# akashsengupta1997/STRAPS-3DHumanShapePose

Measured on AMD Instinct MI355X. Metric: bodies/sec, higher is better.
Workload: dtype fp32 (encoder convolutions as exact bf16x3 operand splits (six bf16 products per term); in-step SMPL blend contraction and skinning as 3-product fp16 splits (fp16x3_lbs: 22-bit operands); fp32 accumulate throughout)

## Files before the change

### include/straps_hip.h

```cpp
#ifndef STRAPS_HIP_H
#define STRAPS_HIP_H

#include <stddef.h>
#include <stdint.h>

#ifdef __cplusplus
extern "C" {
#endif

#define STRAPS_ABI_VERSION 12

#define STRAPS_OK 0
#define STRAPS_EINVAL 1
#define STRAPS_EHIP 2
#define STRAPS_EUNSUPPORTED 3

int straps_abi_version(void);
int straps_selftest_mfma_peak(const float* seed512, float* out, int blocks, int iters, void* stream);
int straps_selftest_mfma_bf16(float* out, unsigned long long* clk2, int blocks, int iters, void* stream);
int straps_selftest_mfma_bf16_dense(float* out, unsigned long long* clk2, int blocks, int iters, int data, void* stream);
const char* straps_last_error(void);
int straps_device_count(void);
int straps_wall_clock_khz(void);
int straps_set_clock_accumulator(unsigned long long* acc2);
// ... 129 lines not shown
#define STRAPS_SMPL_SPLIT_F16_LBS_P16 4

size_t straps_smpl_workspace_bytes(const straps_smpl_model_t* model, long long batch);
int straps_smpl_fwd(const straps_smpl_model_t* model, const float* betas, const float* rotmats,
                    float* verts, float* joints, void* workspace, long long batch, int chunks, int mode,
                    void* stream);

size_t straps_smpl_bwd_workspace_bytes(long long batch, int chunks);
int straps_smpl_bwd(const straps_smpl_model_t* model, const float* betas, const float* rotmats,
                    const float* dverts, const float* djoints, float* dbetas, float* drotmats,
                    void* workspace, long long batch, int chunks, void* stream);
int straps_smpl_bwd_aa(const straps_smpl_model_t* model, const float* betas, const float* rotmats,
                       const float* full_pose_aa, const float* dverts, const float* djoints, float* dbetas,
                       float* dfull_pose_aa, float* drotmats, void* workspace, long long batch, int chunks,
                       void* stream);

int straps_conv_dgrad(const float* dy_nhwc, const float* w_crsk, const float* addend,
                      float* dx_nhwc, int batch, int h, int w, int cin, int cout, int kh, int kw,
                      int stride, int pad, int tile_cfg, void* stream);

int straps_split3_bf16(const float* x, unsigned short* planes, long long n, long long plane_stride,
                       void* stream);
int straps_split3_bf16_cm(const float* x, unsigned short* planes, long long rows, int c,
                          long long plane_stride, void* stream);
int straps_conv_x3_stat_blocks(int batch, int h, int w, int cin, int cout, int kh, int kw, int stride,
                               int pad, int tile_cfg);

int straps_conv_x3f_supported(int cin, int cout, int kh, int kw, int stride, int pad);
int straps_conv_fwd_x3f(const float* x, const float* a_scale, const float* a_shift, int a_relu, const unsigned short* w3,
                        long long w_plane_stride, const float* scale, const float* shift, const float* residual, int relu,
                        float* y, float* stats_partial, int batch, int h, int w, int cin, int cout, int kh, int kw, int stride,
                        int pad, int tile_cfg, void* stream);
int straps_conv_x3f_stat_blocks(int batch, int h, int w, int cin, int cout, int kh, int kw, int stride, int pad, int tile_cfg);
int straps_conv_dgrad_x3f(const float* dy, const unsigned short* w3_crsk, long long w_plane_stride, const float* addend,
                          const unsigned* addend_bits, float* dx, int batch, int h, int w, int cin, int cout, int kh, int kw,
                          int stride, int pad, int tile_cfg, const float* bn_raw, const unsigned* bn_out_bits,
                          const float* bn_mask_scale, const float* bn_mask_shift, const float* bn_mean, const float* bn_invstd,
                          double* bn_partials, void* stream);
int straps_conv_dgrad_x3f_bn_blocks(int batch, int h, int w, int cin, int cout, int kh, int kw, int stride, int pad, int tile_cfg);
size_t straps_conv_wgrad_x3f_workspace_bytes(int batch, int h, int w, int cin, int cout, int kh, int kw, int stride, int pad);
int straps_conv_wgrad_x3f(const float* x, const float* a_scale, const float* a_shift, int a_relu, const float* dy, float* dw_oihw,
                          void* workspace, int batch, int h, int w, int cin, int cout, int kh, int kw, int stride, int pad,
                          int accumulate, void* stream);
int straps_conv_fwd_x3(const unsigned short* x3, long long x_plane_stride,
                       const unsigned short* w3_krsc, long long w_plane_stride, const float* scale,
                       const float* shift, const float* residual, int relu, float* y_nhwc,
                       float* stats_partial, int batch, int h, int w, int cin, int cout, int kh,
                       int kw, int stride, int pad, int tile_cfg, void* stream);
int straps_conv_fwd_x3p(const unsigned short* x3, long long x_plane_stride,
                        const unsigned short* w3_krsc, long long w_plane_stride, const float* scale,
                        const float* shift, const float* residual, int relu, float* y_nhwc,
                        unsigned short* y_planes, long long y_plane_stride, int batch, int h, int w,
                        int cin, int cout, int kh, int kw, int stride, int pad, int tile_cfg, void* stream);
int straps_split_bf16_cm(const float* x, unsigned short* plane, long long rows, int c, void* stream);
int straps_pack_conv_weight_bf16(const float* w_oihw, unsigned short* w_plane, int cout, int cin, int kh, int kw, void* stream);
int straps_conv_bf16_tile_choice(int batch, int h, int w, int cin, int cout, int kh, int kw, int stride, int pad);
int straps_conv_fwd_bf16(const unsigned short* x1, const unsigned short* w1_krsc, const float* scale, const float* shift,
                         const float* residual, int relu, float* y_nhwc, unsigned short* y_plane, int batch, int h, int w,
                         int cin, int cout, int kh, int kw, int stride, int pad, int tile_cfg, void* stream);
int straps_conv_dgrad_x3(const unsigned short* dy3, long long dy_plane_stride,
                         const unsigned short* w3_crsk, long long w_plane_stride,
                         const float* addend, float* dx_nhwc, int batch, int h, int w, int cin,
                         int cout, int kh, int kw, int stride, int pad, int tile_cfg, void* stream);
int straps_bn_apply_x3(const float* raw, const float* scale, const float* shift, const float* residual,
                       int relu, float* y, unsigned short* y_planes, long long plane_stride,
                       long long rows, int c, void* stream);
int straps_bn_relu_maxpool_fwd_x3(const float* raw, const float* scale, const float* shift,
                                  float* y_pool, uint8_t* idx, unsigned short* y_planes,
                                  long long plane_stride, int batch, int h, int w, int c, void* stream);
int straps_bn_bwd_x3(const float* dy, const float* yact, const float* raw, const float* save_mean,
                     const float* save_invstd, const float* gamma, const float* mask_scale,
                     const float* mask_shift, float* dgamma, float* dbeta, float* draw, float* dz_out,
                     unsigned short* draw_planes, long long plane_stride, void* workspace,
                     long long rows, int c, int accumulate, void* stream);
int straps_conv_dgrad_x3_bn_blocks(int batch, int h, int w, int cin, int cout, int kh, int kw, int stride,
                                   int pad, int tile_cfg);
int straps_conv_dgrad_x3_bn(const unsigned short* dy3, long long dy_plane_stride,
                            const unsigned short* w3_crsk, long long w_plane_stride, const float* addend,
                            float* dx_nhwc, int batch, int h, int w, int cin, int cout, int kh, int kw,
                            int stride, int pad, int tile_cfg, const float* bn_raw, const float* bn_out,
                            const float* bn_mask_scale, const float* bn_mask_shift, const float* bn_mean,
                            const float* bn_invstd, double* bn_partials, void* stream);
int straps_bn_bwd_finish_x3(const float* dy, const float* yact, const float* raw, const float* save_mean,
                            const float* save_invstd, const float* gamma, const float* mask_scale,
                            const float* mask_shift, float* dgamma, float* dbeta, float* draw, float* dz_out,
                            unsigned short* draw_planes, long long plane_stride, const double* partials,
                            int nblk, void* workspace, long long rows, int c, int accumulate, void* stream);
int straps_bn_apply_bits_x3(const float* raw, const float* scale, const float* shift, const float* residual, float* y,
                            unsigned short* y_planes, long long plane_stride, unsigned* relu_bits, long long rows,
                            int c, void* stream);
int straps_bn_bwd_bits_x3(const float* dy, const unsigned* relu_bits, const float* raw, const float* save_mean,
                          const float* save_invstd, const float* gamma, float* dgamma, float* dbeta, float* draw,
                          unsigned short* draw_planes, long long plane_stride, void* workspace, long long rows, int c,
                          int accumulate, void* stream);
int straps_bn_bwd_finish_bits_x3(const float* dy, const unsigned* relu_bits, const float* raw, const float* save_mean,
                                 const float* save_invstd, const float* gamma, float* dgamma, float* dbeta, float* draw,
                                 unsigned short* draw_planes, long long plane_stride, const double* partials, int nblk,
                                 void* workspace, long long rows, int c, int accumulate, void* stream);
int straps_conv_dgrad_x3_bits(const unsigned short* dy3, long long dy_plane_stride, const unsigned short* w3_crsk,
                              long long w_plane_stride, const float* addend, float* dx_nhwc, int batch, int h, int w,
                              int cin, int cout, int kh, int kw, int stride, int pad, int tile_cfg,
                              const unsigned* addend_bits, void* stream);
int straps_conv_dgrad_x3_bn_bits(const unsigned short* dy3, long long dy_plane_stride,
                                 const unsigned short* w3_crsk, long long w_plane_stride, const float* addend,
                                 float* dx_nhwc, int batch, int h, int w, int cin, int cout, int kh, int kw,
                                 int stride, int pad, int tile_cfg, const float* bn_raw, const float* bn_out,
                                 const float* bn_mask_scale, const float* bn_mask_shift, const float* bn_mean,
                                 const float* bn_invstd, double* bn_partials, const unsigned* addend_bits,
                                 const unsigned* bn_out_bits, void* stream);
int straps_conv_wgrad_x3_on_planes(int batch, int h, int w, int cin, int cout, int kh, int kw,
                                   int stride, int pad);
int straps_conv_wgrad_x3(const float* x_nhwc, const float* dy_nhwc, const unsigned short* x3,
                         long long x_plane_stride, const unsigned short* dy3, long long dy_plane_stride,
                         float* dw_oihw, void* workspace, int batch, int h, int w, int cin, int cout,
                         int kh, int kw, int stride, int pad, int accumulate, void* stream);


size_t straps_conv_wgrad_workspace_bytes(int batch, int h, int w, int cin, int cout, int kh,
                                         int kw, int stride, int pad);
int straps_conv_wgrad(const float* x_nhwc, const float* dy_nhwc, float* dw_oihw, void* workspace,
                      int batch, int h, int w, int cin, int cout, int kh, int kw, int stride,
                      int pad, int accumulate, void* stream);
size_t straps_stem_wgrad_workspace_bytes(int batch, int cin, int h, int w);
int straps_stem_wgrad(const float* x_nchw, const float* dy_nhwc, float* dw_oihw, void* workspace,
                      const uint32_t* nzmask , int batch, int cin,
                      int h, int w, int accumulate, void* stream);
#define STRAPS_STEM_DGRAD_MAX_CIN 64
size_t straps_stem_dgrad_weight_floats(int cin);
int straps_pack_stem_dgrad_weight(const float* w_oihw, float* w_pk, int cin, void* stream);
int straps_stem_dgrad(const float* dy_nhwc, const float* w_pk, float* dx_nchw, int batch, int cin, int h, int w,
                      int accumulate, void* stream);
int straps_bn_bwd_blocks(long long rows, int c);
size_t straps_bn_bwd_workspace_bytes(long long rows, int c);
int straps_bn_bwd(const float* dy, const float* yact, const float* raw, const float* save_mean,
                  const float* save_invstd, const float* gamma, const float* mask_scale,
                  const float* mask_shift, float* dgamma, float* dbeta, float* draw, float* dz_out,
                  void* workspace, long long rows, int c, int accumulate, void* stream);
int straps_bn_relu_maxpool_fwd(const float* raw_nhwc, const float* scale, const float* shift,
                               float* y_pool_nhwc, uint8_t* idx, int batch, int h, int w, int c,
                               void* stream);
int straps_bn_bwd_pooled(const float* dy_pool_nhwc, const uint8_t* idx, const float* raw,
                         const float* save_mean, const float* save_invstd, const float* gamma,
                         const float* mask_scale, const float* mask_shift, float* dgamma, float* dbeta,
                         float* draw, void* workspace, int batch, int h, int w, int c, int accumulate,
                         void* stream);
size_t straps_stem_tiles(int batch, int in_h, int in_w);
int straps_stem_tile_activity(const uint32_t* nzmask, uint8_t* tile_active, int batch, int cin, int in_h,
                              int in_w, void* stream);
int straps_bn_bwd_pooled_sparse(const float* dy_pool_nhwc, const uint8_t* idx, const float* raw,
                                const float* save_mean, const float* save_invstd, const float* gamma,
                                const float* mask_scale, const float* mask_shift, float* dgamma,
                                float* dbeta, float* draw, void* workspace, int batch, int h, int w, int c,
                                int accumulate, const uint8_t* tile_active, void* stream);
int straps_maxpool_fwd_idx(const float* x_nhwc, float* y_nhwc, uint8_t* idx, int batch, int h,
                           int w, int c, void* stream);
int straps_maxpool_bwd(const float* dy_nhwc, const uint8_t* idx, float* dx_nhwc, int batch, int h,
                       int w, int c, void* stream);
int straps_gap_bwd(const float* dfeat, float* dx_nhwc, int batch, int hw, int c, void* stream);
int straps_masked_copy(const float* x, int ldx, const float* mask, int ldmask, float* y, int ldy,
                       int m, int n, int accumulate, void* stream);
int straps_rot6d_bwd(const float* x6, long long ld, int per_row, const float* drot, float* dx6,
                     long long ldd, long long rows, void* stream);

int straps_build_proxy_input(const float* seg, const float* joints2d, float* out_nchw, int batch,
                             int nj, int wh, void* stream);
int straps_build_proxy_input_std(const float* seg, const float* joints2d, float* out_nchw, int batch,
                                 int nj, int wh, int std, void* stream);
int straps_build_proxy_input_nz(const float* seg, const float* joints2d, float* out_nchw, uint32_t* nzmask,
                                int batch, int nj, int wh, int std, void* stream);
size_t straps_loss_workspace_bytes(long long batch);
int straps_loss_fwd_bwd(const float* pred_verts, const float* pred_joints, const float* est,
                        int ld_est, const float* pred_rot, const float* tgt_verts,
                        const float* tgt_joints2d, const float* tgt_joints3d,
                        const float* tgt_shape, const float* tgt_rot, const float* log_vars,
                        float* loss_out, float* dverts, float* djoints, float* dest, float* drot,
                        float* dlogvar, void* workspace, long long batch, int img_wh, void* stream);
int straps_loss_fwd_bwd_gm(const float* pred_verts, const float* pred_joints, const float* est, int ld_est,
                           const float* pred_rot, const float* tgt_verts, const float* tgt_joints2d,
                           const float* tgt_joints3d, const float* tgt_shape, const float* tgt_rot,
                           const float* log_vars, float* loss_out, float* dverts, float* djoints, float* dest,
                           float* drot, float* dlogvar, void* workspace, long long batch, int img_wh,
                           const float* j2d_count_global, float count_scale, void* stream);
int straps_count_visible(const float* tgt_joints2d, float* out_count, long long batch, int nj, int img_wh,
                         void* stream);
int straps_mse_fwd(const float* pred, const float* tgt, const uint8_t* row_mask, long long rows,
                   int cols, float tgt_scale, float tgt_shift, float* out3, void* workspace,
                   void* stream);
int straps_mse_bwd(const float* pred, const float* tgt, const uint8_t* row_mask, long long rows,
                   int cols, float tgt_scale, float tgt_shift, const float* coef, float* grad,
                   void* stream);
int straps_augment_seg(const float* seg, const float* uniforms, const float* remove_prob,
                       float occlude_prob, int box_dim, float* out, int batch, int wh, void* stream);
int straps_philox_fill(unsigned long long seed, const long long* step_dev, long long step_host,
                       unsigned substream, float* out, long long n, int kind, void* stream);
int straps_counter_add(long long* counters, int n, long long delta, void* stream);
int straps_gather_f32(const float* src, const int* index, float* dst, int n, void* stream);
int straps_memset_zero(void* ptr, size_t bytes, void* stream);
int straps_augment_smpl(const float* pose_rows, long long n_rows, const float* u_index,
                        const float* orig_shape, const float* mean_shape, const float* shape_draws,
                        int shape_mode, const float* std_vector, double range_lo, double range_hi,
                        float* out_shape, float* out_rotmats, float* out_pose, long long batch,
                        void* stream);
int straps_augment_cam_t(const float* mean_cam_t, const float* normals_xy, const float* uniform_z,
                         double xy_std, double z_lo, double z_hi, float* out_cam_t, long long batch,
                         void* stream);
int straps_deviate_joints2d(const float* joints2d, const float* uniforms, double lo, double hi,
                            double hip_lo, double hip_hi, float* out, long long batch, void* stream);
int straps_deviate_verts2d(const float* verts, const float* uniforms, double lo, double hi, float* out,
                           long long nverts_total, void* stream);
int straps_project_targets(const float* joints, const float* cam_t, float fx, float fy, float cx,
                           float cy, float* joints2d, float* joints3d, long long batch, void* stream);
size_t straps_rasterize_workspace_bytes(long long batch, int nverts, int wh);
int straps_rasterize_parts(const float* verts, const int32_t* faces, const uint8_t* face_parts,
                           const float* cam_K, const float* cam_R, const float* cam_t, float* parts,
                           float* depth, void* workspace, long long batch, int nverts, int nfaces, int wh,
                           int cam_per_body, float near, float far, const float* vert_noise_u, double noise_lo,
                           double noise_hi, void* stream);
int straps_crop_resize(const float* seg, const float* joints2d, const float* uniforms,
                       double orig_scale_factor, double delta_scale_lo, double delta_scale_hi,
                       double delta_centre_lo, double delta_centre_hi, float* out_seg,
                       float* out_joints2d, int* boxes, int batch, int wh, int out_wh, int nj,
                       void* stream);
int straps_point_metrics(const float* pred, const float* target, float* out3, long long batch,
                         int npoints, void* stream);
int straps_adam_step(float* params, const float* grads, float* exp_avg, float* exp_avg_sq,
                     long long n, int step, float lr, float beta1, float beta2, float eps,
                     float grad_scale, const long long* step_dev, void* stream);

typedef struct {
    int layers;
    int in_channels;
    int ief_iters;
    int precision;
} straps_regressor_desc_t;
size_t straps_regressor_param_floats(const straps_regressor_desc_t* desc);
size_t straps_regressor_prepared_bytes(const straps_regressor_desc_t* desc);
int straps_regressor_prepare(const straps_regressor_desc_t* desc, const float* params, void* prepared, void* stream);
size_t straps_regressor_workspace_bytes(const straps_regressor_desc_t* desc, int batch, int h, int w);
int straps_regressor_fwd_infer(const straps_regressor_desc_t* desc, const void* prepared, const float* x, int batch, int h, int w,
                               float* est, int ld_est, float* rotmats, void* workspace, size_t workspace_bytes, void* stream);

size_t straps_regressor_train_param_floats(const straps_regressor_desc_t* desc);
size_t straps_regressor_bn_state_floats(const straps_regressor_desc_t* desc);
size_t straps_regressor_train_workspace_bytes(const straps_regressor_desc_t* desc, int batch, int h, int w);
int straps_regressor_fwd_train(const straps_regressor_desc_t* desc, const float* params, float* bn_state, const float* init_est,
                               const float* x, int batch, int h, int w, float* est, int ld_est,
                               void* workspace, size_t workspace_bytes, void* stream);
int straps_regressor_bwd(const straps_regressor_desc_t* desc, const float* params, const float* x, int batch, int h, int w,
                         const float* dest, int ld_dest, float* grads, float* dx,
                         void* workspace, size_t workspace_bytes, void* stream);
int straps_regressor_export_infer_params(const straps_regressor_desc_t* desc, const float* params, const float* bn_state,
                                         const float* init_est, float* infer_params, void* stream);

#define STRAPS_COMM_ID_BYTES 128
int straps_comm_unique_id(void* id128);
int straps_comm_init_rank(const void* id128, int nranks, int rank, void** comm);
int straps_comm_destroy(void* comm);
int straps_comm_size(void* comm);
const char* straps_comm_library(void);
int straps_allreduce_grads(float* flat_g, long long n, void* comm, void* stream);

#ifdef __cplusplus
}
#endif
#endif
```

### straps-3dhumanshapepose_amd/autograd_ops.py

```python
import ctypes as C

import torch

from . import hipabi
from .encoder_exec import encoder_forward
from .ief_module import EST_LD


def _empty_like(t):
    return torch.empty_like(t, memory_format=torch.contiguous_format)


class GradSink(dict):

    def __init__(self, views=None):
        super().__init__()
        self.views = views

    def buf(self, p, zero=False):
        if self.views is not None and p in self.views:
            return self.views[p]
        return torch.zeros_like(p) if zero else torch.empty_like(p)


class _SideStream:

    def __init__(self, stream):
        self.s, self.keep = stream, []

    def run(self, fn, *tensors):
        if self.s is None:
            return fn()
        self.keep.extend(tensors)
        self.s.wait_stream(torch.cuda.current_stream())
        with torch.cuda.stream(self.s):
            return fn()

    def join(self):
        if self.s is not None:
            torch.cuda.current_stream().wait_stream(self.s)
            self.keep.clear()


_FUSE_BN_SUMS = True
_SPARSE_STEM_TAIL = True


def _packed_dgrad_weight(net, conv):
    w = conv.weight

    def make():
        wd = w.detach().contiguous()
        out = torch.empty(wd.numel(), device=wd.device, dtype=torch.float32)
        hipabi.check(hipabi.lib().straps_pack_conv_weight_dgrad(hipabi.ptr(wd), hipabi.ptr(out), wd.shape[0], wd.shape[1], wd.shape[2],
                                                                wd.shape[3], hipabi.stream_ptr()), 'straps_pack_conv_weight_dgrad')
        return out
    return net._cached(('wd', id(conv)), [w], make)


def _bn_bwd(L, rec, dy, masked, want_dz, grads, planes_sink=None, keep_fp32=True, mask_bits=None):
    bn = rec['bn']
    raw, ss = rec['raw'], rec['stats']
    rows, Cc = raw.numel() // raw.shape[-1], raw.shape[-1]
    ws = torch.empty(L.straps_bn_bwd_workspace_bytes(rows, Cc) // 4, device=raw.device, dtype=torch.float32)
    dgamma, dbeta = grads.buf(bn.weight), grads.buf(bn.bias)
    keep_fp32 = keep_fp32 or planes_sink is None
    draw = _empty_like(raw) if keep_fp32 else raw.new_empty(0)
    dz = _empty_like(raw) if want_dz else None
    from_raw = masked and rec.get('residual') is None
    bits = mask_bits if mask_bits is not None else (rec.get('bits') if masked and not from_raw else None)
    if bits is not None and want_dz:
        raise RuntimeError('BatchNorm backward on ReLU bits writes no masked gradient (dz)')
    planes, ps = None, 0
    if planes_sink is not None:
        ps = (raw.numel() + 7) // 8 * 8
        planes = torch.empty(3, ps, device=raw.device, dtype=torch.int16)
        planes_sink[id(draw)] = (draw, planes, ps)
    flags = 2 if rec.get('frozen') else 0
    fused = rec.pop('bwd_partials', None)
    if bits is not None:
        args = (hipabi.ptr(dy), hipabi.ptr(bits), hipabi.ptr(raw), hipabi.ptr(ss[2]), hipabi.ptr(ss[3]), hipabi.ptr(bn.weight), hipabi.ptr(dgamma),
                hipabi.ptr(dbeta), hipabi.ptr(draw if keep_fp32 else None), hipabi.ptr(planes), ps)
        if fused is not None and fused[2] is dy and masked:
            hipabi.check(L.straps_bn_bwd_finish_bits_x3(*args, hipabi.ptr(fused[0]), fused[1], hipabi.ptr(ws), rows, Cc, flags, hipabi.stream_ptr()),
                         'straps_bn_bwd_finish_bits_x3')
        else:
            hipabi.check(L.straps_bn_bwd_bits_x3(*args, hipabi.ptr(ws), rows, Cc, flags, hipabi.stream_ptr()), 'straps_bn_bwd_bits_x3')
    elif fused is not None and fused[2] is dy and masked:
        hipabi.check(L.straps_bn_bwd_finish_x3(hipabi.ptr(dy), hipabi.ptr(rec['out'] if not from_raw else None), hipabi.ptr(raw), hipabi.ptr(ss[2]),
                                               hipabi.ptr(ss[3]), hipabi.ptr(bn.weight), hipabi.ptr(ss[0] if from_raw else None),
                                               hipabi.ptr(ss[1] if from_raw else None), hipabi.ptr(dgamma), hipabi.ptr(dbeta),
                                               hipabi.ptr(draw if keep_fp32 else None), hipabi.ptr(dz), hipabi.ptr(planes), ps, hipabi.ptr(fused[0]),
                                               fused[1], hipabi.ptr(ws), rows, Cc, flags, hipabi.stream_ptr()), 'straps_bn_bwd_finish_x3')
    else:
        hipabi.check(L.straps_bn_bwd_x3(hipabi.ptr(dy), hipabi.ptr(rec['out'] if masked and not from_raw else None), hipabi.ptr(raw), hipabi.ptr(ss[2]),
                                        hipabi.ptr(ss[3]), hipabi.ptr(bn.weight), hipabi.ptr(ss[0] if from_raw else None),
                                        hipabi.ptr(ss[1] if from_raw else None), hipabi.ptr(dgamma), hipabi.ptr(dbeta), hipabi.ptr(draw if keep_fp32 else None),
                                        hipabi.ptr(dz), hipabi.ptr(planes), ps, hipabi.ptr(ws), rows, Cc, flags, hipabi.stream_ptr()), 'straps_bn_bwd')
    grads[bn.weight] = dgamma
    grads[bn.bias] = dbeta
    return draw, dz


def _conv_wgrad(L, rec, draw, grads, planes_sink=None):
    conv = rec['conv']
    B, H, W, Cin, Cout, k, stride, pad, Ho, Wo = rec['geom']
    dw = grads.buf(conv.weight)
    if rec.get('fmode'):
        a_bn = rec.get('a_bn')
        wsf = torch.empty(max(L.straps_conv_wgrad_x3f_workspace_bytes(B, H, W, Cin, Cout, k, k, stride, pad) // 4, 1), device=draw.device, dtype=torch.float32)
        hipabi.check(L.straps_conv_wgrad_x3f(hipabi.ptr(rec['x']), hipabi.ptr(a_bn[0] if a_bn is not None else None), hipabi.ptr(a_bn[1] if a_bn is not None else None),
                                             int(a_bn is not None), hipabi.ptr(draw), hipabi.ptr(dw), hipabi.ptr(wsf), B, H, W, Cin, Cout, k, k, stride, pad, 0,
                                             hipabi.stream_ptr()), 'straps_conv_wgrad_x3f')
        grads[conv.weight] = dw
        return
    ws = torch.empty(L.straps_conv_wgrad_workspace_bytes(B, H, W, Cin, Cout, k, k, stride, pad) // 4, device=draw.device, dtype=torch.float32)
    fp = lambda t: hipabi.ptr(t if t is not None and t.numel() else None)
    xh = rec.get('x3')
    gh = planes_sink.get(id(draw)) if planes_sink is not None else None
    if xh is not None and gh is not None and xh[0] is rec['x'] and gh[0] is draw:
        hipabi.check(L.straps_conv_wgrad_x3(fp(rec['x']), fp(draw), hipabi.ptr(xh[1]), xh[2], hipabi.ptr(gh[1]), gh[2], hipabi.ptr(dw),
                                            hipabi.ptr(ws), B, H, W, Cin, Cout, k, k, stride, pad, 0, hipabi.stream_ptr()), 'straps_conv_wgrad_x3')
    else:
        hipabi.check(L.straps_conv_wgrad(hipabi.ptr(rec['x']), hipabi.ptr(draw), hipabi.ptr(dw), hipabi.ptr(ws), B, H, W, Cin, Cout, k, k, stride,
                                         pad, 0, hipabi.stream_ptr()), 'straps_conv_wgrad')
    grads[conv.weight] = dw


def _conv_dgrad(L, net, rec, draw, addend, planes_sink=None, bn_next=None, addend_bits=None):
    conv = rec['conv']
    B, H, W, Cin, Cout, k, stride, pad, Ho, Wo = rec['geom']
    dx = torch.empty(B, H, W, Cin, device=draw.device, dtype=torch.float32)
    if rec.get('fmode'):
        if not draw.numel():
            raise RuntimeError('fp32-operand data gradient: the fp32 gradient was not materialised')
        w3, wps = net._packed_weight_x3(conv, dgrad=True)
        raw = nbits = msc = msh = mean = invstd = part = None
        if bn_next is not None and _FUSE_BN_SUMS:
            ssn = bn_next['stats']
            from_raw = bn_next.get('residual') is None
            nbits = None if from_raw else bn_next.get('bits')
            if from_raw or nbits is not None:
                nblk = L.straps_conv_dgrad_x3f_bn_blocks(B, H, W, Cin, Cout, k, k, stride, pad, 0)
                part = torch.empty(nblk, Cin, 2, device=dx.device, dtype=torch.float64)
                raw, mean, invstd = bn_next['raw'], ssn[2], ssn[3]
                if from_raw:
                    msc, msh = ssn[0], ssn[1]
        if bn_next is None or not _FUSE_BN_SUMS or part is not None:
            hipabi.check(L.straps_conv_dgrad_x3f(hipabi.ptr(draw), hipabi.ptr(w3), wps, hipabi.ptr(addend), hipabi.ptr(addend_bits), hipabi.ptr(dx), B, H, W, Cin, Cout,
                                                 k, k, stride, pad, 0, hipabi.ptr(raw), hipabi.ptr(nbits), hipabi.ptr(msc), hipabi.ptr(msh), hipabi.ptr(mean),
                                                 hipabi.ptr(invstd), hipabi.ptr(part), hipabi.stream_ptr()), 'straps_conv_dgrad_x3f')
            if part is not None:
                bn_next['bwd_partials'] = (part, nblk, dx)
            return dx
    if getattr(net, 'conv_precision', 'fp32') == 'bf16x3':
        if not draw.numel() and (planes_sink is None or planes_sink.get(id(draw)) is None):
            raise RuntimeError('data gradient: neither the fp32 gradient nor its planes exist')
        hit = planes_sink.get(id(draw)) if planes_sink is not None else None
        if hit is not None and hit[0] is draw:
            g3, gps = hit[1], hit[2]
        else:
            from .encoder_exec import split3
            g3, gps = split3(L, draw)
        w3, wps = net._packed_weight_x3(conv, dgrad=True)
        if bn_next is not None and _FUSE_BN_SUMS:
            ssn = bn_next['stats']
            from_raw = bn_next.get('residual') is None
            nblk = L.straps_conv_dgrad_x3_bn_blocks(B, H, W, Cin, Cout, k, k, stride, pad, 0)
            part = torch.empty(nblk, Cin, 2, device=dx.device, dtype=torch.float64)
            nbits = None if from_raw else bn_next.get('bits')
            if addend_bits is not None or nbits is not None:
                hipabi.check(L.straps_conv_dgrad_x3_bn_bits(hipabi.ptr(g3), gps, hipabi.ptr(w3), wps, hipabi.ptr(addend), hipabi.ptr(dx), B, H, W, Cin,
                                                            Cout, k, k, stride, pad, 0, hipabi.ptr(bn_next['raw']),
                                                            hipabi.ptr(None if from_raw or nbits is not None else bn_next['out']),
                                                            hipabi.ptr(ssn[0] if from_raw else None), hipabi.ptr(ssn[1] if from_raw else None),
                                                            hipabi.ptr(ssn[2]), hipabi.ptr(ssn[3]), hipabi.ptr(part), hipabi.ptr(addend_bits),
                                                            hipabi.ptr(nbits), hipabi.stream_ptr()), 'straps_conv_dgrad_x3_bn_bits')
                bn_next['bwd_partials'] = (part, nblk, dx)
                return dx
            hipabi.check(L.straps_conv_dgrad_x3_bn(hipabi.ptr(g3), gps, hipabi.ptr(w3), wps, hipabi.ptr(addend), hipabi.ptr(dx), B, H, W, Cin, Cout,
                                                   k, k, stride, pad, 0, hipabi.ptr(bn_next['raw']), hipabi.ptr(None if from_raw else bn_next['out']),
                                                   hipabi.ptr(ssn[0] if from_raw else None), hipabi.ptr(ssn[1] if from_raw else None),
                                                   hipabi.ptr(ssn[2]), hipabi.ptr(ssn[3]), hipabi.ptr(part), hipabi.stream_ptr()),
                         'straps_conv_dgrad_x3_bn')
            bn_next['bwd_partials'] = (part, nblk, dx)
            return dx
        if addend_bits is not None:
            hipabi.check(L.straps_conv_dgrad_x3_bits(hipabi.ptr(g3), gps, hipabi.ptr(w3), wps, hipabi.ptr(addend), hipabi.ptr(dx), B, H, W, Cin, Cout,
                                                     k, k, stride, pad, 0, hipabi.ptr(addend_bits), hipabi.stream_ptr()), 'straps_conv_dgrad_x3_bits')
            return dx
        hipabi.check(L.straps_conv_dgrad_x3(hipabi.ptr(g3), gps, hipabi.ptr(w3), wps, hipabi.ptr(addend), hipabi.ptr(dx), B, H, W, Cin, Cout,
                                            k, k, stride, pad, 0, hipabi.stream_ptr()), 'straps_conv_dgrad_x3')
        return dx
    if addend_bits is not None:
        raise RuntimeError('ReLU bits exist only on the bf16x3 route')
    hipabi.check(L.straps_conv_dgrad(hipabi.ptr(draw), hipabi.ptr(_packed_dgrad_weight(net, conv)), hipabi.ptr(addend), hipabi.ptr(dx), B, H, W,
                                     Cin, Cout, k, k, stride, pad, 0, hipabi.stream_ptr()), 'straps_conv_dgrad')
    return dx


def encoder_backward(net, tape, dfeat, views=None, side_stream=None, after_layer3=None, want_dx=False, param_grads=True):
    L = hipabi.lib()
    grads = GradSink(views)
    side = _SideStream(side_stream)
    sink = {} if getattr(net, 'conv_precision', 'fp32') == 'bf16x3' else None

    def sink_of(rec):
        return None if rec.get('fmode') else sink

    def keep(rec):
        if sink is None or rec.get('x3') is None:
            return True
        B, H, W, Cin, Cout, k, stride, pad, Ho, Wo = rec['geom']
        return not L.straps_conv_wgrad_x3_on_planes(B, H, W, Cin, Cout, k, k, stride, pad)
    rec = tape['gap']
    B, HW, Cf = rec['geom']
    dy = _empty_like(rec['x'])
    hipabi.check(L.straps_gap_bwd(hipabi.ptr(dfeat.contiguous()), hipabi.ptr(dy), B, HW, Cf, hipabi.stream_ptr()), 'straps_gap_bwd')
    units = [u for li in range(1, 5) for u in getattr(net, 'layer%d' % li)]
    for li in range(4, 0, -1):
        for unit in reversed(list(getattr(net, 'layer%d' % li))):
            pairs = unit.conv_bn_pairs()
            ui = units.index(unit)
            prev_last = tape[id(units[ui - 1].conv_bn_pairs()[-1][0])] if ui > 0 else None
            rec = tape[id(pairs[-1][0])]
            ubits = rec.get('bits') if sink is not None else None
            dskip_bits = None
            if ubits is not None:
                draw, _ = _bn_bwd(L, rec, dy, True, False, grads, sink_of(rec), keep(rec))
                dz = dy
            else:
                draw, dz = _bn_bwd(L, rec, dy, True, True, grads, sink_of(rec), keep(rec))
            if param_grads:
                side.run(lambda rec=rec, draw=draw: _conv_wgrad(L, rec, draw, grads, sink), draw)
            if unit.downsample is not None:
                recd = tape[id(unit.downsample[0])]
                drawd, _ = _bn_bwd(L, recd, dz, False, False, grads, sink_of(recd), keep(recd), mask_bits=ubits)
                if param_grads:
                    side.run(lambda recd=recd, drawd=drawd: _conv_wgrad(L, recd, drawd, grads, sink), drawd)
                dskip = _conv_dgrad(L, net, recd, drawd, None, sink)
            else:
                dskip, dskip_bits = dz, ubits
            for ci in range(len(pairs) - 1, 0, -1):
                rec_prev = tape[id(pairs[ci - 1][0])]
                dt = _conv_dgrad(L, net, tape[id(pairs[ci][0])], draw, None, sink, bn_next=rec_prev if sink is not None else None)
                rec = rec_prev
                draw, _ = _bn_bwd(L, rec, dt, True, False, grads, sink_of(rec), keep(rec))
                if param_grads:
                    side.run(lambda rec=rec, draw=draw: _conv_wgrad(L, rec, draw, grads, sink), draw)
            dy = _conv_dgrad(L, net, tape[id(pairs[0][0])], draw, dskip, sink, bn_next=prev_last if sink is not None else None,
                             addend_bits=dskip_bits)
        if li == 3 and after_layer3 is not None:
            side.join()
            after_layer3()
    rec = tape['maxpool']
    B, H, W, Cc, Hp, Wp = rec['geom']
    if rec['kind'] == 'maxpool_fused':
        idx = rec['idx']
        rec = tape['stem']
        bn, raw, ss = rec['bn'], rec['raw'], rec['stats']
        ws = torch.empty(L.straps_bn_bwd_workspace_bytes(B * H * W, Cc) // 4, device=raw.device, dtype=torch.float32)
        dgamma, dbeta = grads.buf(bn.weight), grads.buf(bn.bias)
        draw = _empty_like(raw)
        tact = None
        if rec.get('nzmask') is not None and _SPARSE_STEM_TAIL and not want_dx:
            _, Cin0, Hin, Win = rec['geom'][:4]
            tact = torch.empty(L.straps_stem_tiles(B, Hin, Win), device=raw.device, dtype=torch.uint8)
            hipabi.check(L.straps_stem_tile_activity(hipabi.ptr(rec['nzmask']), hipabi.ptr(tact), B, Cin0, Hin, Win, hipabi.stream_ptr()),
                         'straps_stem_tile_activity')
        hipabi.check(L.straps_bn_bwd_pooled_sparse(hipabi.ptr(dy), hipabi.ptr(idx), hipabi.ptr(raw), hipabi.ptr(ss[2]), hipabi.ptr(ss[3]),
                                                   hipabi.ptr(bn.weight), hipabi.ptr(ss[0]), hipabi.ptr(ss[1]), hipabi.ptr(dgamma), hipabi.ptr(dbeta),
                                                   hipabi.ptr(draw), hipabi.ptr(ws), B, H, W, Cc, 2 if rec.get('frozen') else 0, hipabi.ptr(tact),
                                                   hipabi.stream_ptr()), 'straps_bn_bwd_pooled_sparse')
        grads[bn.weight] = dgamma
        grads[bn.bias] = dbeta
    else:
        dstem = _empty_like(rec['x'])
        hipabi.check(L.straps_maxpool_bwd(hipabi.ptr(dy), hipabi.ptr(rec['idx']), hipabi.ptr(dstem), B, H, W, Cc, hipabi.stream_ptr()),
                     'straps_maxpool_bwd')
        rec = tape['stem']
        draw, _ = _bn_bwd(L, rec, dstem, True, False, grads)
    B, Cin, H, W, Ho, Wo = rec['geom']
    dx = None
    if want_dx:
        dx = torch.empty(B, Cin, H, W, device=draw.device, dtype=torch.float32)
        hipabi.check(L.straps_stem_dgrad(hipabi.ptr(draw), hipabi.ptr(net._packed_stem_dgrad_weight()), hipabi.ptr(dx), B, Cin, H, W, 0,
                                         hipabi.stream_ptr()), 'straps_stem_dgrad')
    if param_grads:
        ws = torch.empty(L.straps_stem_wgrad_workspace_bytes(B, Cin, H, W) // 4, device=draw.device, dtype=torch.float32)
        dw = grads.buf(net.conv1.weight)
        hipabi.check(L.straps_stem_wgrad(hipabi.ptr(rec['x']), hipabi.ptr(draw), hipabi.ptr(dw), hipabi.ptr(ws), hipabi.ptr(rec.get('nzmask')),
                                         B, Cin, H, W, 0, hipabi.stream_ptr()), 'straps_stem_wgrad')
        grads[net.conv1.weight] = dw
    side.join()
    return (grads, dx) if want_dx else grads


def ief_backward(ief, feat, tape, dest, views=None, param_grads=True):
    sink = GradSink(views)
    L, st = hipabi.lib(), hipabi.stream_ptr()
    pk = ief._packed(feat.device)
    B, F = feat.shape
    H1, H2, P = ief.fc1.out_features, ief.fc2.out_features, ief.num_output_params
    dev = feat.device
    T = len(tape)
    e = lambda *s: torch.empty(*s, device=dev, dtype=torch.float32)
    D = hipabi.gemm_desc
    ests, h1s, h2s = tape[0]['stacks']
    assert ests.shape == (T + 1, B, EST_LD) and h1s.shape == (T, B, H1) and h2s.shape == (T, B, H2)
    dW3, db3 = sink.buf(ief.fc3.weight), sink.buf(ief.fc3.bias)
    dW2, db2 = sink.buf(ief.fc2.weight), sink.buf(ief.fc2.bias)
    dW1, db1 = sink.buf(ief.fc1.weight), sink.buf(ief.fc1.bias)
    dests = e(T + 1, B, EST_LD)
    dsrc = dest if dest.stride(-1) == 1 and dest.dim() == 2 else dest.contiguous()
    hipabi.check(L.straps_masked_copy(hipabi.ptr(dsrc), dsrc.stride(0), None, 0, hipabi.ptr(dests[T]), EST_LD, B, EST_LD, 0, st), 'ief dest slot')
    dh2s, dh1s, dc1 = e(T, B, H2), e(T, B, H1), e(B, H1)
    w3, w2 = ief.fc3.weight, ief.fc2.weight
    for it in reversed(range(T)):
        hipabi.gemm_multi([D(dests[it + 1], EST_LD, 1, w3, H2, 1, dh2s[it], H2, B, H2, P, mask=h2s[it], ldmask=H2)])
        hipabi.gemm_multi([D(dh2s[it], H2, 1, w2, H1, 1, dh1s[it], H1, B, H1, H2, mask=h1s[it], ldmask=H1,
                             c2=dc1, ldc2=H1, accumulate2=int(it != T - 1))])
        hipabi.gemm_multi([D(dh1s[it], H1, 1, pk['w1e'], EST_LD, 1, dests[it], EST_LD, B, P, H1, addend=dests[it + 1], ldadd=EST_LD)])
    one = pk['one']
    dfeat = e(B, F)
    if not param_grads:
        hipabi.gemm_multi([D(dc1, H1, 1, pk['w1f'], F, 1, dfeat, F, B, F, H1)])
        return dfeat, {}
    KB = T * B
    hipabi.gemm_multi([
        D(dh2s, 1, H2, h1s, H1, 1, dW2, H1, H2, H1, KB),
        D(dc1, 1, H1, feat, F, 1, dW1, F + P, H1, F, B),
        D(dh1s, 1, H1, ests, EST_LD, 1, dW1.data_ptr() + 4 * F, F + P, H1, P, KB),
        D(dests[1], 1, EST_LD, h2s, H2, 1, dW3, H2, P, H2, KB),
        D(dc1, H1, 1, pk['w1f'], F, 1, dfeat, F, B, F, H1),
        D(one, 0, 0, dh2s, H2, 1, db2, H2, 1, H2, KB),
        D(one, 0, 0, dests[1], EST_LD, 1, db3, P, 1, P, KB),
        D(one, 0, 0, dc1, H1, 1, db1, H1, 1, H1, B)])
    grads = {ief.fc1.weight: dW1, ief.fc1.bias: db1, ief.fc2.weight: dW2, ief.fc2.bias: db2, ief.fc3.weight: dW3, ief.fc3.bias: db3}
    return dfeat, grads


class _RegressorFn(torch.autograd.Function):

    @staticmethod
    def forward(ctx, reg, x, *params):
        enc_tape, ief_tape = {}, []
        with torch.no_grad():
            feat = encoder_forward(reg.image_encoder, x, enc_tape)
            est = reg.ief_module.forward_estimate(feat, ief_tape)
        ctx.reg, ctx.feat, ctx.enc_tape, ctx.ief_tape, ctx.params = reg, feat, enc_tape, ief_tape, params
        return est

    @staticmethod
    def backward(ctx, dest):
        reg = ctx.reg
        want_dx, pg = ctx.needs_input_grad[1], any(ctx.needs_input_grad[2:])
        dfeat, g_ief = ief_backward(reg.ief_module, ctx.feat, ctx.ief_tape, dest, param_grads=pg)
        g_enc = encoder_backward(reg.image_encoder, ctx.enc_tape, dfeat, want_dx=want_dx, param_grads=pg)
        g_enc, dx = g_enc if want_dx else (g_enc, None)
        g_enc.update(g_ief)
        out = [g_enc.get(p) if need else None for p, need in zip(ctx.params, ctx.needs_input_grad[2:])]
        ctx.enc_tape = ctx.ief_tape = None
        return (None, dx) + tuple(out)


def regressor_autograd(reg, x):
    hipabi.require_gpu_tensor(x, 'regressor input', torch.float32)
    params = list(reg.parameters())
    est = _RegressorFn.apply(reg, x, *params)
    P = reg.ief_module.num_output_params
    return est[:, :3], est[:, 3:3 + 24 * 6], est[:, 3 + 24 * 6:P]


class _EncoderFn(torch.autograd.Function):

    @staticmethod
    def forward(ctx, net, x, *params):
        tape = {}
        with torch.no_grad():
            feat = encoder_forward(net, x, tape)
        ctx.net, ctx.tape, ctx.params = net, tape, params
        return feat

    @staticmethod
    def backward(ctx, dfeat):
        want_dx = ctx.needs_input_grad[1]
        g = encoder_backward(ctx.net, ctx.tape, dfeat, want_dx=want_dx, param_grads=any(ctx.needs_input_grad[2:]))
        g, dx = g if want_dx else (g, None)
        ctx.tape = None
        return (None, dx) + tuple(g.get(p) if need else None for p, need in zip(ctx.params, ctx.needs_input_grad[2:]))


def encoder_autograd(net, x):
    hipabi.require_gpu_tensor(x, 'encoder input', torch.float32)
    return _EncoderFn.apply(net, x, *list(net.parameters()))


class _IefFn(torch.autograd.Function):
    @staticmethod
    def forward(ctx, ief, feat, *params):
        tape = []
        with torch.no_grad():
            est = ief.forward_estimate(feat, tape)
        ctx.ief, ctx.feat, ctx.tape, ctx.params = ief, feat.detach().contiguous(), tape, params
        return est

    @staticmethod
    def backward(ctx, dest):
        dfeat, g = ief_backward(ctx.ief, ctx.feat, ctx.tape, dest, param_grads=any(ctx.needs_input_grad[2:]))
        return (None, dfeat) + tuple(g.get(p) if need else None for p, need in zip(ctx.params, ctx.needs_input_grad[2:]))


def ief_autograd(ief, feat):
    return _IefFn.apply(ief, feat, *list(ief.parameters()))


class _Rot6dFn(torch.autograd.Function):
    @staticmethod
    def forward(ctx, x):
        from .rigid_transform_utils import _rot6d_fwd
        ctx.save_for_backward(x)
        return _rot6d_fwd(x.detach())

    @staticmethod
    def backward(ctx, dR):
        (x,) = ctx.saved_tensors
        xd = x.detach()
        if xd.dim() == 2 and xd.stride(1) == 1 and xd.shape[1] % 6 == 0 and xd.stride(0) >= xd.shape[1]:
            rows, per_row, ld = xd.shape[0], xd.shape[1] // 6, xd.stride(0)
            dx = torch.empty(rows, xd.shape[1], device=xd.device, dtype=torch.float32)
        else:
            xd = xd.contiguous().view(-1, 6)
            rows, per_row, ld = xd.shape[0], 1, 6
            dx = torch.empty(rows, 6, device=xd.device, dtype=torch.float32)
        hipabi.check(hipabi.lib().straps_rot6d_bwd(hipabi.ptr(xd), ld, per_row, hipabi.ptr(dR.contiguous()), hipabi.ptr(dx), dx.stride(0), rows,
                                                   hipabi.stream_ptr()), 'straps_rot6d_bwd')
        return dx.view(x.shape)


def rot6d_autograd(x):
    return _Rot6dFn.apply(x)


class _RodriguesFn(torch.autograd.Function):
    @staticmethod
# ... 78 lines not shown
```

### straps-3dhumanshapepose_amd/csrc/backward.hip

```cpp
#include "common.h"
#include <stdlib.h>

namespace {

struct WgradP {
    const float* x;
    const float* dy;
    float* part;
    int B, H, W, Cin, Cout, R, S, stride, pad, Ho, Wo;
    int M, rows_per_split, ct, it;
};

__device__ __attribute__((aligned(16))) float k_zero16w[4] = {0.f, 0.f, 0.f, 0.f};

template <int BCO, int BCI>
__global__ __launch_bounds__(256) void conv_wgrad_kernel(WgradP p) {
    constexpr int STG = 32 * (BCO + BCI);
    constexpr int LPD = BCO / 4, PWD = 64 / LPD, RDD = 8 / PWD;
    constexpr int LPX = BCI / 4, PWX = 64 / LPX, RDX = 8 / PWX;
    constexpr int MI = BCO / 64, NI = BCI / 64;
    extern __shared__ __attribute__((aligned(16))) float smem[];
    const int tid = threadIdx.x, lane = tid & 63, wave = tid >> 6;
    const int wave_u = __builtin_amdgcn_readfirstlane(wave);
    const int wm = wave >> 1, wn = wave & 1;
// ... 510 lines not shown
#pragma unroll
        for (int q = 0; q < DR; ++q) {
            if (NG > 1 && (q & 1) != grp) continue;
#pragma unroll
            for (int pl = 0; pl < 3; ++pl)
                __builtin_amdgcn_global_load_lds((const __attribute__((address_space(1))) void*)(dbase + d_off[q] + pl * p.dps),
                                                 (__attribute__((address_space(3))) void*)(D + (pl * DPX + 32 * q + 8 * wave_u) * 64), 16, 0, 0);
        }
#pragma unroll
        for (int q = 0; q < XR; ++q) {
            if (q * 32 + 8 * wave_u >= npatch || q * 32 + 8 * wave_u >= XPX) break;
            if (NG > 1 && ((q + DR) & 1) != grp) continue;
            const int hi = ho0 + x_pr[q], wi = wo0 + x_pc[q];
            const bool ok = (unsigned)hi < (unsigned)p.H && (unsigned)wi < (unsigned)p.W;
            const u16* src = ok ? xsrc + (x_pr[q] * p.W + x_pc[q]) * 32 + x_g[q] : zsrc;
            const long long ps = ok ? p.xps : 0;
#pragma unroll
            for (int pl = 0; pl < 3; ++pl)
                __builtin_amdgcn_global_load_lds((const __attribute__((address_space(1))) void*)(src + pl * ps),
                                                 (__attribute__((address_space(3))) void*)(X + (pl * XPX + 32 * q + 8 * wave_u) * 64), 16, 0, 0);
        }
    };

    const int t = lane & 15, ch16 = (lane >> 4) & 1, kh = lane >> 5;
    auto row_off = [&](int slot_px, int c4) {
        const int g = (c4 >> 3) ^ (((slot_px >> 1) & 1) << 2);
        return slot_px * 64 + g * 8 + (c4 & 4);
    };
    int d_fo[KSG][2], x_fo[KSG][2];
#pragma unroll
    for (int ks = 0; ks < KSG; ++ks)
#pragma unroll
        for (int r = 0; r < 2; ++r) {
            const int px = (grp + NG * ks) * 16 + kh * 8 + r * 4 + (t >> 2);
            d_fo[ks][r] = row_off(px, wm * 32 + ch16 * 16 + (t & 3) * 4);
            x_fo[ks][r] = (px >> p.cw_log2) * pw + (px & (p.cw - 1));
        }
    const int x_c4 = wn * 32 + ch16 * 16 + (t & 3) * 4;

    f32x16 acc[9];
#pragma unroll
    for (int tp = 0; tp < 9; ++tp)
#pragma unroll
        for (int q = 0; q < 16; ++q) acc[tp][q] = 0.f;
    if (cbeg < cend) dma_chunk(cbeg, 0);
    constexpr int TA[6] = {1, 0, 2, 0, 1, 0};
    constexpr int TB[6] = {1, 2, 0, 1, 0, 0};
    for (int c = cbeg; c < cend; ++c) {
        const int stage = (c - cbeg) & 1;
        asm volatile("s_waitcnt vmcnt(0)" ::: "memory");
        __builtin_amdgcn_s_barrier();
        asm volatile("" ::: "memory");
        if (c + 1 < cend && !(ABL & 1)) dma_chunk(c + 1, stage ^ 1);
        const u16* D = smem + ((ABL & 1) ? 0 : stage) * STAGE;
        const u16* X = D + 3 * DPX * 64;
        __builtin_amdgcn_s_setprio(1);
#pragma unroll
        for (int ks = 0; ks < KSG; ++ks) {
            bf16x8w a[3];
#pragma unroll
            for (int pl = 0; pl < 3; ++pl) a[pl] = tr_frag(D + pl * DPX * 64 + d_fo[ks][0], D + pl * DPX * 64 + d_fo[ks][1]);
#pragma unroll
            for (int tp0 = 0; tp0 < 9; tp0 += W3X_TG) {
                bf16x8w b[W3X_TG][3];
#pragma unroll
                for (int u = 0; u < W3X_TG; ++u) {
                    const int tp = tp0 + u;
                    if (tp >= 9) break;
                    const int sh = (ABL & 4) ? 0 : (tp / 3) * pw + (tp % 3);
                    const int o0 = row_off(x_fo[ks][0] + sh, x_c4), o1 = row_off(x_fo[ks][1] + sh, x_c4);
#pragma unroll
                    for (int pl = 0; pl < 3; ++pl) b[u][pl] = tr_frag(X + pl * XPX * 64 + o0, X + pl * XPX * 64 + o1);
                }
                if (ABL & 2) {
#pragma unroll
                    for (int u = 0; u < W3X_TG; ++u)
                        if (tp0 + u < 9)
#pragma unroll
                            for (int pl = 0; pl < 3; ++pl) acc[0][pl] += (float)b[u][pl][0] + (float)a[pl][1];
                    continue;
                }
#pragma unroll
                for (int e = 0; e < 6; ++e)
#pragma unroll
                    for (int u = 0; u < W3X_TG; ++u)
                        if (tp0 + u < 9) acc[tp0 + u] = __builtin_amdgcn_mfma_f32_32x32x16_bf16(a[TA[e]], b[u][TB[e]], acc[tp0 + u], 0, 0, 0);
            }
        }
        __builtin_amdgcn_s_setprio(0);
    }
    if constexpr (NG > 1) {
        float* R = smem_f + ((wave * 3) * 16) * 64 + lane;
#pragma unroll
        for (int rd = 0; rd < 3; ++rd) {
            __syncthreads();
            if (grp == 1) {
#pragma unroll
                for (int tp = 0; tp < 3; ++tp)
#pragma unroll
                    for (int q = 0; q < 16; ++q) R[(tp * 16 + q) * 64] = acc[rd * 3 + tp][q];
            }
            __syncthreads();
            if (grp == 0) {
#pragma unroll
                for (int tp = 0; tp < 3; ++tp)
#pragma unroll
                    for (int q = 0; q < 16; ++q) acc[rd * 3 + tp][q] += R[(tp * 16 + q) * 64];
            }
        }
        if (grp != 0) return;
    }
    const int i = lane & 31;
    float* o = p.part + (long long)blockIdx.y * p.Cout * 9 * p.Cin;
#pragma unroll
    for (int tp = 0; tp < 9; ++tp)
#pragma unroll
        for (int q = 0; q < 16; ++q) {
            const int co = co0 + wm * 32 + mfma_row(q, lane);
            o[((long long)co * 9 + tp) * p.Cin + ci0 + wn * 32 + i] = acc[tp][q];
        }
}

__global__ __launch_bounds__(256) void wgrad_reduce_kernel(const float* __restrict__ part, float* __restrict__ dw, int splits,
                                                           int Cout, int Cin, int RS, int accumulate) {
    __shared__ f32x4 red[4][64];
    const long long n = (long long)Cout * RS * Cin;
    const int lane = threadIdx.x & 63, sg = threadIdx.x >> 6;
    const long long idx = ((long long)blockIdx.x * 64 + lane) * 4;
    f32x4 s = {0.f, 0.f, 0.f, 0.f};
    int k = sg;
    for (; k + 12 < splits; k += 16) {
        const f32x4 v0 = *reinterpret_cast<const f32x4*>(part + (long long)k * n + idx);
        const f32x4 v1 = *reinterpret_cast<const f32x4*>(part + (long long)(k + 4) * n + idx);
        const f32x4 v2 = *reinterpret_cast<const f32x4*>(part + (long long)(k + 8) * n + idx);
        const f32x4 v3 = *reinterpret_cast<const f32x4*>(part + (long long)(k + 12) * n + idx);
        s += (v0 + v1) + (v2 + v3);
    }
    for (; k < splits; k += 4) s += *reinterpret_cast<const f32x4*>(part + (long long)k * n + idx);
    red[sg][lane] = s;
    __syncthreads();
    if (sg != 0) return;
    s = (red[0][lane] + red[1][lane]) + (red[2][lane] + red[3][lane]);
    const int ci = (int)(idx % Cin);
    long long t = idx / Cin;
    const int tap = (int)(t % RS);
    const int co = (int)(t / RS);
#pragma unroll
    for (int e = 0; e < 4; ++e) {
        const long long o = ((long long)co * Cin + ci + e) * RS + tap;
        dw[o] = accumulate ? dw[o] + s[e] : s[e];
    }
}

constexpr int TY = 2, TX = 32, PH = 2 * TY + 5, PW = 72, TPIX = TY * TX;
constexpr int CG = 4, GK = CG * 49, GNB = (GK + 31) / 32, GUNITS = 2 * GNB, UPW = (GUNITS + 3) / 4;

__global__ __launch_bounds__(256) void stem_tileact_kernel(const unsigned* __restrict__ nzmask, uint8_t* __restrict__ tact, int C, int H, int W,
                                                           int tiles_x, int tiles_y, int ntiles, int groups) {
    const int idx = blockIdx.x * 256 + threadIdx.x;
    if (idx >= ntiles * groups) return;
    const int grp = idx / ntiles, tile = idx - grp * ntiles;
    int bid = tile;
    const int b = bid / (tiles_x * tiles_y);
    bid -= b * tiles_x * tiles_y;
    const int ty = bid / tiles_x, tx = bid - ty * tiles_x;
    const int hi0 = 2 * (ty * TY) - 3, wi0 = 2 * (tx * TX) - 3;
    const int HC = (H + 3) >> 2, WW = (W + 255) >> 8;
    const int rc0 = max(hi0, 0) >> 2, rc1 = min(hi0 + PH - 1, H - 1) >> 2;
    const int wa = max(wi0 - 1, 0), wb = min(wi0 - 2 + PW, W - 1);
    const int c0 = grp * CG, nc = min(CG, C - c0);
    unsigned chact = 0;
    for (int cl = 0; cl < nc; ++cl) {
        unsigned any = 0;
        for (int rcell = rc0; rcell <= rc1; ++rcell)
            for (int word = wa >> 8; word <= (wb >> 8); ++word) {
                const int lo = max(wa, word << 8), hi = min(wb, (word << 8) + 255);
                const int b0 = (lo >> 3) & 31, b1 = (hi >> 3) & 31;
                const unsigned bits = (b1 == 31 ? 0xffffffffu : ((1u << (b1 + 1)) - 1u)) & ~((1u << b0) - 1u);
                any |= nzmask[(((long long)b * C + c0 + cl) * HC + rcell) * WW + word] & bits;
            }
        if (any) chact |= 1u << cl;
    }
    tact[idx] = (uint8_t)chact;
}

__global__ __launch_bounds__(256) void stem_tileany_kernel(const unsigned* __restrict__ nzmask, uint8_t* __restrict__ tany, int C, int H, int W,
                                                           int tiles_x, int tiles_y, int ntiles) {
    const int lane = threadIdx.x & 63, sub = lane & 31;
    const int tile = (blockIdx.x * 256 + threadIdx.x) >> 5;
    unsigned any = 0;
    if (tile < ntiles) {
        int bid = tile;
        const int b = bid / (tiles_x * tiles_y);
        bid -= b * tiles_x * tiles_y;
        const int ty = bid / tiles_x, tx = bid - ty * tiles_x;
        const int hi0 = 2 * (ty * TY) - 3, wi0 = 2 * (tx * TX) - 3;
        const int HC = (H + 3) >> 2, WW = (W + 255) >> 8;
        const int rc0 = max(hi0, 0) >> 2, rc1 = min(hi0 + PH - 1, H - 1) >> 2;
        const int wa = max(wi0 - 1, 0), wb = min(wi0 - 2 + PW, W - 1);
        for (int c = sub; c < C; c += 32)
            for (int rcell = rc0; rcell <= rc1; ++rcell)
                for (int word = wa >> 8; word <= (wb >> 8); ++word) {
                    const int lo = max(wa, word << 8), hi = min(wb, (word << 8) + 255);
                    const int b0 = (lo >> 3) & 31, b1 = (hi >> 3) & 31;
                    const unsigned bits = (b1 == 31 ? 0xffffffffu : ((1u << (b1 + 1)) - 1u)) & ~((1u << b0) - 1u);
                    any |= nzmask[(((long long)b * C + c) * HC + rcell) * WW + word] & bits;
                }
    }
    const unsigned long long bal = __ballot(any != 0u);
    const unsigned mine = (unsigned)(bal >> (lane & 32));
    if (sub == 0 && tile < ntiles) tany[tile] = mine ? 1 : 0;
}

__global__ __launch_bounds__(256) void stem_wgrad_kernel(const float* __restrict__ x, const float* __restrict__ dy,
                                                         float* __restrict__ part, const uint8_t* __restrict__ tact, int B, int C, int H,
                                                         int W, int Ho, int Wo,
                                                         int tiles_x, int tiles_y, int Kp, int ntiles, int rot) {
    __shared__ __attribute__((aligned(16))) float patch[2 * CG * PH * PW];
    __shared__ __attribute__((aligned(16))) float dys[2 * TPIX * 68];
    const int tid = threadIdx.x, lane = tid & 63;
    const int wave = __builtin_amdgcn_readfirstlane(tid >> 6);
    const int i = lane & 31, h = lane >> 5;
    const int c0 = blockIdx.y * CG;
    const int nc = min(CG, C - c0);
    const int gk = nc * 49;

    int u_a[UPW], u_nb[UPW], u_ko[UPW];
    unsigned u_span[UPW];
#pragma unroll
    for (int j = 0; j < UPW; ++j) {
        const int u = wave + 4 * j;
        u_a[j] = u & 1;
        u_nb[j] = u >> 1;
        const int k = u_nb[j] * 32 + i;
        int o = 0;
        if (u < GUNITS && k < gk) {
            const int cl = k / 49, rs = k - cl * 49;
            const int r = rs / 7, s_ = rs - r * 7;
            o = (cl * PH + r) * PW + s_ + 1;
        }
        u_ko[j] = o;
        const int k0 = u_nb[j] * 32;
        u_span[j] = 0;
        if (u < GUNITS && k0 < gk) {
            const int cl0 = k0 / 49, cl1 = min(k0 + 31, gk - 1) / 49;
            u_span[j] = (1u << cl0) | (1u << cl1);
        }
    }
    f32x16 acc[UPW];
#pragma unroll
    for (int j = 0; j < UPW; ++j)
#pragma unroll
        for (int q = 0; q < 16; ++q) acc[j][q] = 0.f;

    constexpr int PIT = (CG * PH * (PW / 4) + 255) / 256;
    constexpr int DIT = TPIX * 16 / 256;
    const bool vec = (W & 3) == 0;
    f32x4 pv[PIT], dv[DIT];
    auto tile_origin = [&](int tile, int& b, int& y0, int& x0) {
        b = tile / (tiles_x * tiles_y);
        const int bid = tile - b * tiles_x * tiles_y;
        const int ty = bid / tiles_x;
        y0 = ty * TY;
        x0 = (bid - ty * tiles_x) * TX;
    };
    auto issue_loads = [&](int tile, unsigned chact) {
        int b, y0, x0;
        tile_origin(tile, b, y0, x0);
        const int hi0 = 2 * y0 - 3, wi0 = 2 * x0 - 3;
#pragma unroll
        for (int it = 0; it < PIT; ++it) {
            const int idx = tid + it * 256;
            const int q = idx % (PW / 4);
            const int rc = idx / (PW / 4);
            const int row = rc % PH, cl = rc / PH;
            const int hi = hi0 + row, wi = wi0 - 1 + 4 * q;
            pv[it] = f32x4{0.f, 0.f, 0.f, 0.f};
            if (vec && cl < nc && ((chact >> cl) & 1u) && (unsigned)hi < (unsigned)H && wi >= 0 && wi < W)
                pv[it] = *reinterpret_cast<const f32x4*>(x + (((long long)b * C + c0 + cl) * H + hi) * W + wi);
        }
#pragma unroll
        for (int it = 0; it < DIT; ++it) {
            const int idx = tid + it * 256;
            const int pix = idx >> 4, c4 = idx & 15;
            const int yo = y0 + (pix >> 5), xo = x0 + (pix & 31);
            dv[it] = f32x4{0.f, 0.f, 0.f, 0.f};
            if (yo < Ho && xo < Wo) dv[it] = *reinterpret_cast<const f32x4*>(dy + (((long long)b * Ho + yo) * Wo + xo) * 64 + c4 * 4);
        }
    };
    auto store_tile = [&](int tile, unsigned chact, float* pb, float* db) {
        if (vec) {
#pragma unroll
            for (int it = 0; it < PIT; ++it) {
                const int idx = tid + it * 256;
                if (idx < nc * PH * (PW / 4)) *reinterpret_cast<f32x4*>(pb + (idx / (PW / 4)) * PW + 4 * (idx % (PW / 4))) = pv[it];
            }
        } else {
            int b, y0, x0;
            tile_origin(tile, b, y0, x0);
            const int hi0 = 2 * y0 - 3, wi0 = 2 * x0 - 3;
            for (int idx = tid; idx < nc * PH * PW; idx += 256) {
                const int col = idx % PW;
                const int rc = idx / PW;
                const int row = rc % PH, cl = rc / PH;
                const int hi = hi0 + row, wi = wi0 - 1 + col;
                float v = 0.f;
                if (((chact >> cl) & 1u) && (unsigned)hi < (unsigned)H && (unsigned)wi < (unsigned)W) v = x[(((long long)b * C + c0 + cl) * H + hi) * W + wi];
                pb[idx] = v;
            }
        }
#pragma unroll
        for (int it = 0; it < DIT; ++it) {
            const int idx = tid + it * 256;
            *reinterpret_cast<f32x4*>(db + (idx >> 4) * 68 + (idx & 15) * 4) = dv[it];
        }
    };

    const uint8_t* myact = tact + (long long)blockIdx.y * ntiles;
    int buf = 0;
    const int G = gridDim.x;
    for (int m0 = 0; (long long)m0 * G < ntiles; m0 += 64) {
        const int m = m0 + lane;
        const long long mine_l = (long long)m * G + (blockIdx.x + (long long)rot * m) % G;
        const int mine = mine_l < ntiles ? (int)mine_l : -1;
        const unsigned act = mine >= 0 ? myact[mine] : 0u;
        unsigned long long todo = __ballot(act != 0u);
        if (todo) {
            const int l0 = __ffsll((long long)todo) - 1;
            issue_loads(__shfl(mine, l0, 64), (unsigned)__shfl((int)act, l0, 64));
        }
        while (todo) {
            const int l = __ffsll((long long)todo) - 1;
            todo &= todo - 1;
            const int tile = __shfl(mine, l, 64);
            const unsigned chact = (unsigned)__shfl((int)act, l, 64);
            float* pb = patch + buf * (CG * PH * PW);
            float* db = dys + buf * (TPIX * 68);
            store_tile(tile, chact, pb, db);
            __syncthreads();
            if (todo) {
                const int ln = __ffsll((long long)todo) - 1;
                issue_loads(__shfl(mine, ln, 64), (unsigned)__shfl((int)act, ln, 64));
            }
#pragma unroll
            for (int j = 0; j < UPW; ++j) {
                if (!(u_span[j] & chact)) continue;
                const float* ap = db + (h * 4) * 68 + u_a[j] * 32 + i;
                const float* bp = pb + u_ko[j] + 8 * h;
                float av[32], bv[32];
#pragma unroll
                for (int g = 0; g < TPIX / 8; ++g)
#pragma unroll
                    for (int e = 0; e < 4; ++e) {
                        av[g * 4 + e] = ap[(g * 8 + e) * 68];
                        bv[g * 4 + e] = bp[(g >> 2) * 2 * PW + (g & 3) * 16 + 2 * e];
                    }
                __builtin_amdgcn_sched_barrier(0);
                f32x16 c = acc[j];
#pragma unroll
                for (int t = 0; t < 32; ++t) c = mfma32(av[t], bv[t], c);
                acc[j] = c;
                __builtin_amdgcn_sched_barrier(0);
            }
            buf ^= 1;
        }
        __syncthreads();
    }
    float* o = part + (long long)blockIdx.x * 64 * Kp + c0 * 49;
#pragma unroll
    for (int j = 0; j < UPW; ++j) {
        const int kcol = u_nb[j] * 32 + i;
        if (wave + 4 * j < GUNITS && kcol < gk) {
#pragma unroll
            for (int q = 0; q < 16; ++q) o[(long long)(u_a[j] * 32 + mfma_row(q, lane)) * Kp + kcol] = acc[j][q];
        }
    }
}

__global__ __launch_bounds__(256) void stem_wgrad_reduce_kernel(const float* __restrict__ part, float* __restrict__ dw, int nblocks,
                                                                int K, int Kp, int accumulate) {
    __shared__ float red[4][64];
    const int o = threadIdx.x & 63, g = threadIdx.x >> 6;
    const int idx = blockIdx.x * 64 + o;
    const bool live = idx < 64 * K;
    const int co = live ? idx / K : 0, k = live ? idx - co * K : 0;
    const float* src = part + (long long)co * Kp + k;
    const long long bstride = (long long)64 * Kp;
    float s = 0.f;
    if (live) {
#pragma unroll 8
        for (int b = g; b < nblocks; b += 4) s += src[b * bstride];
    }
    red[g][o] = s;
    __syncthreads();
    if (g == 0 && live) {
        const float t = ((red[0][o] + red[1][o]) + red[2][o]) + red[3][o];
        dw[idx] = accumulate ? dw[idx] + t : t;
    }
}

struct PoolSrc {
    const float* dyp;
    const uint8_t* idx;
    int H, W, Ho, Wo;
    const uint8_t* tany;
    int tiles_x, tiles_y;
};

__device__ __forceinline__ f32x4 pool_grad(const PoolSrc& ps, long long row, int c4, int C) {
    const int wi = (int)(row % ps.W);
    const long long t = row / ps.W;
    const int hi = (int)(t % ps.H);
    const long long b = t / ps.H;
    f32x4 g = {0.f, 0.f, 0.f, 0.f};
    const int ho_lo = hi >> 1, ho_hi = (hi + 1) >> 1;
    const int wo_lo = wi >> 1, wo_hi = (wi + 1) >> 1;
    for (int ho = ho_lo; ho <= ho_hi; ++ho) {
        if (ho >= ps.Ho) continue;
        const int r = hi - (2 * ho - 1);
        for (int wo = wo_lo; wo <= wo_hi; ++wo) {
            if (wo >= ps.Wo) continue;
            const int want = r * 3 + wi - (2 * wo - 1);
            const long long o = ((b * ps.Ho + ho) * ps.Wo + wo) * C + c4 * 4;
            const uchar4 k = *reinterpret_cast<const uchar4*>(ps.idx + o);
            const f32x4 d = *reinterpret_cast<const f32x4*>(ps.dyp + o);
            if (k.x == want) g[0] += d[0];
            if (k.y == want) g[1] += d[1];
            if (k.z == want) g[2] += d[2];
            if (k.w == want) g[3] += d[3];
        }
    }
    return g;
}

template <bool POOL>
__global__ __launch_bounds__(256) void bn_bwd_reduce_kernel(const float* __restrict__ dy, const float* __restrict__ yact,
                                                            const float* __restrict__ raw, const float* __restrict__ mean,
                                                            const float* __restrict__ invstd, const float* __restrict__ msc,
                                                            const float* __restrict__ msh, double* __restrict__ part, long long rows,
                                                            int C, int rows_per_block, PoolSrc ps, const unsigned* __restrict__ bits) {
    __shared__ double red[256][8];
    constexpr int TR = 16;
    const int tc = threadIdx.x & 15, tr = threadIdx.x >> 4;
    const int c4 = blockIdx.y * 16 + tc;
    const bool active = c4 * 4 < C;
    const long long r0 = (long long)blockIdx.x * rows_per_block;
    const long long r1 = r0 + rows_per_block < rows ? r0 + rows_per_block : rows;
    double s1[4] = {0.0, 0.0, 0.0, 0.0}, s2[4] = {0.0, 0.0, 0.0, 0.0};
    f32x4 is = {0.f, 0.f, 0.f, 0.f};
    if (active) {
        const f32x4 mu = *reinterpret_cast<const f32x4*>(mean + c4 * 4);
        is = *reinterpret_cast<const f32x4*>(invstd + c4 * 4);
        f32x4 ksc = {0.f, 0.f, 0.f, 0.f}, ksh = ksc;
        if (msc) { ksc = *reinterpret_cast<const f32x4*>(msc + c4 * 4); ksh = *reinterpret_cast<const f32x4*>(msh + c4 * 4); }
        long long r = r0 + tr;
        for (; r + 3 * TR < r1; r += 4 * TR) {
            f32x4 g[4], ya[4], xr[4];
#pragma unroll
            for (int u = 0; u < 4; ++u) {
                const long long o = (r + (long long)u * TR) * C + c4 * 4;
                if constexpr (POOL) g[u] = pool_grad(ps, r + (long long)u * TR, c4, C);
                else g[u] = *reinterpret_cast<const f32x4*>(dy + o);
                xr[u] = *reinterpret_cast<const f32x4*>(raw + o);
                if (bits) ya[u][0] = __uint_as_float(bits[(r + (long long)u * TR) * (C >> 5) + (c4 >> 3)]);
                else if (yact) ya[u] = *reinterpret_cast<const f32x4*>(yact + o);
            }
#pragma unroll
            for (int u = 0; u < 4; ++u) {
                if (bits) {
                    const unsigned nib = __float_as_uint(ya[u][0]) >> ((c4 & 7) * 4);
#pragma unroll
                    for (int e = 0; e < 4; ++e) g[u][e] = ((nib >> e) & 1u) ? g[u][e] : 0.f;
                } else if (yact) {
#pragma unroll
                    for (int e = 0; e < 4; ++e) g[u][e] = ya[u][e] > 0.f ? g[u][e] : 0.f;
                } else if (msc) {
#pragma unroll
                    for (int e = 0; e < 4; ++e) g[u][e] = fmaf(xr[u][e], ksc[e], ksh[e]) > 0.f ? g[u][e] : 0.f;
                }
#pragma unroll
                for (int e = 0; e < 4; ++e) {
                    s1[e] += (double)g[u][e];
                    s2[e] += (double)g[u][e] * ((double)xr[u][e] - (double)mu[e]);
                }
            }
        }
        for (; r < r1; r += TR) {
            const long long o = r * C + c4 * 4;
            f32x4 g;
            if constexpr (POOL) g = pool_grad(ps, r, c4, C);
            else g = *reinterpret_cast<const f32x4*>(dy + o);
            const f32x4 xr = *reinterpret_cast<const f32x4*>(raw + o);
            if (bits) {
                const unsigned nib = bits[r * (C >> 5) + (c4 >> 3)] >> ((c4 & 7) * 4);
#pragma unroll
                for (int e = 0; e < 4; ++e) g[e] = ((nib >> e) & 1u) ? g[e] : 0.f;
            } else if (yact) {
                const f32x4 ya = *reinterpret_cast<const f32x4*>(yact + o);
#pragma unroll
                for (int e = 0; e < 4; ++e) g[e] = ya[e] > 0.f ? g[e] : 0.f;
            } else if (msc) {
#pragma unroll
                for (int e = 0; e < 4; ++e) g[e] = fmaf(xr[e], ksc[e], ksh[e]) > 0.f ? g[e] : 0.f;
            }
#pragma unroll
            for (int e = 0; e < 4; ++e) {
                s1[e] += (double)g[e];
                s2[e] += (double)g[e] * ((double)xr[e] - (double)mu[e]);
            }
        }
    }
#pragma unroll
    for (int e = 0; e < 4; ++e) { red[threadIdx.x][e] = s1[e]; red[threadIdx.x][4 + e] = s2[e] * (double)is[e]; }
    __syncthreads();
    if (tr == 0 && active) {
        double t[8];
#pragma unroll
        for (int e = 0; e < 8; ++e) t[e] = red[tc][e];
        for (int q = 1; q < TR; ++q)
#pragma unroll
            for (int e = 0; e < 8; ++e) t[e] += red[q * 16 + tc][e];
        double* o = part + ((long long)blockIdx.x * C + c4 * 4) * 2;
#pragma unroll
        for (int e = 0; e < 4; ++e) { o[e * 2 + 0] = t[e]; o[e * 2 + 1] = t[4 + e]; }
    }
}

__global__ __launch_bounds__(256) void bn_bwd_reduce_pooled_kernel(const float* __restrict__ raw, const float* __restrict__ mean,
                                                                   const float* __restrict__ invstd, const float* __restrict__ msc,
                                                                   const float* __restrict__ msh, double* __restrict__ part, long long prows,
                                                                   int C, int rows_per_block, PoolSrc ps) {
    __shared__ double red[256][8];
    constexpr int TR = 16;
    const int tc = threadIdx.x & 15, tr = threadIdx.x >> 4;
    const int c4 = blockIdx.y * 16 + tc;
    const bool active = c4 * 4 < C;
    const long long r0 = (long long)blockIdx.x * rows_per_block;
    const long long r1 = r0 + rows_per_block < prows ? r0 + rows_per_block : prows;
    double s1[4] = {0.0, 0.0, 0.0, 0.0}, s2[4] = {0.0, 0.0, 0.0, 0.0};
    f32x4 is = {0.f, 0.f, 0.f, 0.f};
    if (active) {
        const f32x4 mu = *reinterpret_cast<const f32x4*>(mean + c4 * 4);
        is = *reinterpret_cast<const f32x4*>(invstd + c4 * 4);
        const f32x4 ksc = *reinterpret_cast<const f32x4*>(msc + c4 * 4), ksh = *reinterpret_cast<const f32x4*>(msh + c4 * 4);
        for (long long r = r0 + tr; r < r1; r += TR) {
            const int wo = (int)(r % ps.Wo);
            const long long t = r / ps.Wo;
            const int ho = (int)(t % ps.Ho);
            const long long b = t / ps.Ho;
            const long long o = r * C + c4 * 4;
            const f32x4 d = *reinterpret_cast<const f32x4*>(ps.dyp + o);
            const uchar4 k4 = *reinterpret_cast<const uchar4*>(ps.idx + o);
            const int k[4] = {k4.x, k4.y, k4.z, k4.w};
            float xr[4];
#pragma unroll
            for (int e = 0; e < 4; ++e) {
                const int hi = 2 * ho - 1 + k[e] / 3, wi = 2 * wo - 1 + k[e] % 3;
                xr[e] = raw[((b * ps.H + hi) * ps.W + wi) * C + c4 * 4 + e];
            }
#pragma unroll
            for (int e = 0; e < 4; ++e) {
                const float g = fmaf(xr[e], ksc[e], ksh[e]) > 0.f ? d[e] : 0.f;
                s1[e] += (double)g;
                s2[e] += (double)g * ((double)xr[e] - (double)mu[e]);
            }
        }
    }
#pragma unroll
    for (int e = 0; e < 4; ++e) { red[threadIdx.x][e] = s1[e]; red[threadIdx.x][4 + e] = s2[e] * (double)is[e]; }
    __syncthreads();
    if (tr == 0 && active) {
        double t[8];
#pragma unroll
        for (int e = 0; e < 8; ++e) t[e] = red[tc][e];
        for (int q = 1; q < TR; ++q)
#pragma unroll
            for (int e = 0; e < 8; ++e) t[e] += red[q * 16 + tc][e];
        double* o = part + ((long long)blockIdx.x * C + c4 * 4) * 2;
#pragma unroll
        for (int e = 0; e < 4; ++e) { o[e * 2 + 0] = t[e]; o[e * 2 + 1] = t[4 + e]; }
    }
}

__global__ __launch_bounds__(256) void bn_bwd_finalize_kernel(const double* __restrict__ part, int nblocks, int C, double count,
                                                             const float* __restrict__ gamma, const float* __restrict__ invstd,
                                                             float* __restrict__ dgamma, float* __restrict__ dbeta,
                                                             double* __restrict__ coefd, float* __restrict__ k1, int accumulate) {
    int c;
    double s1, s2;
    if (bn_partials_sum4(part, nblocks, C, s1, s2, c)) {
        dbeta[c] = accumulate ? dbeta[c] + (float)s1 : (float)s1;
        dgamma[c] = accumulate ? dgamma[c] + (float)s2 : (float)s2;
        k1[c] = gamma[c] * invstd[c];
        coefd[c] = s1 / count;
        coefd[C + c] = s2 / count;
    }
}

constexpr int POOL_CHUNK = 1024;
template <bool POOL>
__global__ __launch_bounds__(256) void bn_bwd_apply_kernel(const float* __restrict__ dy, const float* __restrict__ yact,
                                                           const float* __restrict__ raw, const float* __restrict__ mean,
                                                           const float* __restrict__ invstd, const double* __restrict__ coefd,
                                                           const float* __restrict__ k1p, const float* __restrict__ msc,
                                                           const float* __restrict__ msh, float* __restrict__ draw, float* dz_out,
                                                           u16* __restrict__ planes, long long pstride, long long n4, int C, PoolSrc ps,
                                                           const unsigned* __restrict__ bits, int tiled) {
    const int C4 = C >> 2;
    const long long first = POOL ? (long long)blockIdx.x * POOL_CHUNK + threadIdx.x : (long long)blockIdx.x * 256 + threadIdx.x;
    const long long last = POOL ? (n4 < ((long long)blockIdx.x + 1) * POOL_CHUNK ? n4 : ((long long)blockIdx.x + 1) * POOL_CHUNK) : n4;
    const long long step = POOL ? 256 : (long long)gridDim.x * 256;
    const long long rows = n4 / C4;
    struct Consts { f32x4 ksc, ksh, mu, is, k1; double m1[4], m2[4]; };
    auto load_consts = [&](int c4) {
        Consts k;
        if (!yact && !bits && msc) { k.ksc = *reinterpret_cast<const f32x4*>(msc + c4 * 4); k.ksh = *reinterpret_cast<const f32x4*>(msh + c4 * 4); }
        k.mu = *reinterpret_cast<const f32x4*>(mean + c4 * 4);
        k.is = *reinterpret_cast<const f32x4*>(invstd + c4 * 4);
        k.k1 = *reinterpret_cast<const f32x4*>(k1p + c4 * 4);
#pragma unroll
        for (int e = 0; e < 4; ++e) { k.m1[e] = coefd[c4 * 4 + e]; k.m2[e] = coefd[C + c4 * 4 + e]; }
        return k;
    };
    auto body = [&](long long idx, long long row, int c4, const Consts& k) {
        f32x4 g;
        if constexpr (POOL) {
            if (ps.tany) {
                const int wi = (int)(row % ps.W);
                const long long t = row / ps.W;
                const int hi = (int)(t % ps.H);
                const long long b = t / ps.H;
                if (!ps.tany[(b * ps.tiles_y + (hi >> 1)) * ps.tiles_x + (wi >> 5)]) return;
            }
            g = pool_grad(ps, row, c4, C);
        } else {
            g = *reinterpret_cast<const f32x4*>(dy + idx * 4);
        }
        const f32x4 xr = *reinterpret_cast<const f32x4*>(raw + idx * 4);
        if (bits) {
            const unsigned nib = bits[row * (C >> 5) + (c4 >> 3)] >> ((c4 & 7) * 4);
#pragma unroll
            for (int e = 0; e < 4; ++e) g[e] = ((nib >> e) & 1u) ? g[e] : 0.f;
        } else if (yact) {
            const f32x4 ya = *reinterpret_cast<const f32x4*>(yact + idx * 4);
#pragma unroll
            for (int e = 0; e < 4; ++e) g[e] = ya[e] > 0.f ? g[e] : 0.f;
        } else if (msc) {
#pragma unroll
            for (int e = 0; e < 4; ++e) g[e] = fmaf(xr[e], k.ksc[e], k.ksh[e]) > 0.f ? g[e] : 0.f;
        }
        f32x4 o;
#pragma unroll
        for (int e = 0; e < 4; ++e) {
            const double xh = ((double)xr[e] - (double)k.mu[e]) * (double)k.is[e];
            o[e] = (float)((double)k.k1[e] * (((double)g[e] - k.m1[e]) - xh * k.m2[e]));
        }
        if (dz_out) *reinterpret_cast<f32x4*>(dz_out + idx * 4) = g;
        if (draw) *reinterpret_cast<f32x4*>(draw + idx * 4) = o;
        if (planes) store_planes4_cm(planes, pstride, row, c4 * 4, rows, o);
    };
    if (!POOL && tiled) {
        const int l = threadIdx.x & 63, w = threadIdx.x >> 6, wcg = tiled, ncb = (C4 >> 4) / wcg, trows = 16 / wcg;
        const int c4 = ((int)(blockIdx.x % ncb) * wcg + w % wcg) * 16 + (l >> 5) * 8 + (l & 7);
        const Consts k = load_consts(c4);
        const long long rstep = (long long)(gridDim.x / ncb) * trows;
        for (long long row = (long long)(blockIdx.x / ncb) * trows + (w / wcg) * 4 + ((l >> 3) & 3); row < rows; row += rstep) body(row * C4 + c4, row, c4, k);
    } else if (step % C4 == 0) {
        if (first >= last) return;
        const int c4 = (int)(first % C4);
        const Consts k = load_consts(c4);
        const long long rstep = step / C4;
        long long row = first / C4;
        for (long long idx = first; idx < last; idx += step, row += rstep) body(idx, row, c4, k);
    } else {
        for (long long idx = first; idx < last; idx += step) {
            const int c4 = (int)(idx % C4);
            body(idx, idx / C4, c4, load_consts(c4));
        }
    }
}

__global__ __launch_bounds__(256) void maxpool_idx_kernel(const float* __restrict__ x, float* __restrict__ y, uint8_t* __restrict__ idx,
                                                          int B, int H, int W, int C, int Ho, int Wo) {
    const int C4 = C >> 2;
    const long long n = (long long)B * Ho * Wo * C4;
    for (long long i = (long long)blockIdx.x * 256 + threadIdx.x; i < n; i += (long long)gridDim.x * 256) {
        const int c4 = (int)(i % C4);
        long long t = i / C4;
        const int wo = (int)(t % Wo); t /= Wo;
        const int ho = (int)(t % Ho);
        const int b = (int)(t / Ho);
        f32x4 m = {-INFINITY, -INFINITY, -INFINITY, -INFINITY};
        int am[4] = {0, 0, 0, 0};
        bool first = true;
#pragma unroll
        for (int r = 0; r < 3; ++r) {
            const int hi = 2 * ho - 1 + r;
            if ((unsigned)hi >= (unsigned)H) continue;
#pragma unroll
            for (int s = 0; s < 3; ++s) {
                const int wi = 2 * wo - 1 + s;
                if ((unsigned)wi >= (unsigned)W) continue;
                const f32x4 v = *reinterpret_cast<const f32x4*>(x + (((long long)b * H + hi) * W + wi) * C + c4 * 4);
#pragma unroll
                for (int e = 0; e < 4; ++e)
                    if (first || v[e] > m[e] || v[e] != v[e]) { m[e] = v[e]; am[e] = r * 3 + s; }
                first = false;
            }
        }
        *reinterpret_cast<f32x4*>(y + i * 4) = m;
        *reinterpret_cast<uchar4*>(idx + i * 4) = make_uchar4((unsigned char)am[0], (unsigned char)am[1], (unsigned char)am[2], (unsigned char)am[3]);
    }
}

__global__ __launch_bounds__(256) void bn_relu_maxpool_kernel(const float* __restrict__ raw, const float* __restrict__ scale,
                                                              const float* __restrict__ shift, float* __restrict__ y, uint8_t* __restrict__ idx,
                                                              u16* __restrict__ planes, long long pstride, int B, int H, int W, int C, int Ho, int Wo) {
    const int C4 = C >> 2;
    const long long n = (long long)B * Ho * Wo * C4;
    for (long long i = (long long)blockIdx.x * 256 + threadIdx.x; i < n; i += (long long)gridDim.x * 256) {
        const int c4 = (int)(i % C4);
        long long t = i / C4;
        const int wo = (int)(t % Wo); t /= Wo;
        const int ho = (int)(t % Ho);
        const int b = (int)(t / Ho);
        const f32x4 sc = *reinterpret_cast<const f32x4*>(scale + c4 * 4);
        const f32x4 sh = *reinterpret_cast<const f32x4*>(shift + c4 * 4);
        f32x4 m = {-INFINITY, -INFINITY, -INFINITY, -INFINITY};
        int am[4] = {0, 0, 0, 0};
        bool first = true;
#pragma unroll
        for (int r = 0; r < 3; ++r) {
            const int hi = 2 * ho - 1 + r;
            if ((unsigned)hi >= (unsigned)H) continue;
#pragma unroll
            for (int s = 0; s < 3; ++s) {
                const int wi = 2 * wo - 1 + s;
                if ((unsigned)wi >= (unsigned)W) continue;
                f32x4 v = *reinterpret_cast<const f32x4*>(raw + (((long long)b * H + hi) * W + wi) * C + c4 * 4);
#pragma unroll
                for (int e = 0; e < 4; ++e) {
                    v[e] = fmaxf(fmaf(v[e], sc[e], sh[e]), 0.f);
                    if (first || v[e] > m[e] || v[e] != v[e]) { m[e] = v[e]; am[e] = r * 3 + s; }
                }
                first = false;
            }
        }
        *reinterpret_cast<f32x4*>(y + i * 4) = m;
        *reinterpret_cast<uchar4*>(idx + i * 4) = make_uchar4((unsigned char)am[0], (unsigned char)am[1], (unsigned char)am[2], (unsigned char)am[3]);
        if (planes) store_planes4_cm(planes, pstride, i / C4, c4 * 4, (long long)B * Ho * Wo, m);
    }
}

__global__ __launch_bounds__(256) void maxpool_bwd_kernel(const float* __restrict__ dy, const uint8_t* __restrict__ idx,
                                                          float* __restrict__ dx, int B, int H, int W, int C, int Ho, int Wo) {
    const int C4 = C >> 2;
    const long long n = (long long)B * H * W * C4;
    for (long long i = (long long)blockIdx.x * 256 + threadIdx.x; i < n; i += (long long)gridDim.x * 256) {
        const int c4 = (int)(i % C4);
        long long t = i / C4;
        const int wi = (int)(t % W); t /= W;
        const int hi = (int)(t % H);
        const int b = (int)(t / H);
        f32x4 g = {0.f, 0.f, 0.f, 0.f};
        const int ho_lo = hi >> 1, ho_hi = (hi + 1) >> 1;
        const int wo_lo = wi >> 1, wo_hi = (wi + 1) >> 1;
        for (int ho = ho_lo; ho <= ho_hi; ++ho) {
            if (ho >= Ho) continue;
            const int r = hi - (2 * ho - 1);
            for (int wo = wo_lo; wo <= wo_hi; ++wo) {
                if (wo >= Wo) continue;
                const int s = wi - (2 * wo - 1);
                const long long o = (((long long)b * Ho + ho) * Wo + wo) * C + c4 * 4;
                const uchar4 k = *reinterpret_cast<const uchar4*>(idx + o);
                const f32x4 d = *reinterpret_cast<const f32x4*>(dy + o);
                const int want = r * 3 + s;
                if (k.x == want) g[0] += d[0];
                if (k.y == want) g[1] += d[1];
                if (k.z == want) g[2] += d[2];
                if (k.w == want) g[3] += d[3];
            }
        }
        *reinterpret_cast<f32x4*>(dx + i * 4) = g;
    }
}

__global__ __launch_bounds__(256) void gap_bwd_kernel(const float* __restrict__ dfeat, float* __restrict__ dx, int B, int HW, int C) {
    const long long n = (long long)B * HW * C;
    const float inv = 1.0f / (float)HW;
    for (long long i = (long long)blockIdx.x * 256 + threadIdx.x; i < n; i += (long long)gridDim.x * 256) {
        const int c = (int)(i % C);
        const long long b = i / ((long long)HW * C);
        dx[i] = dfeat[b * C + c] * inv;
    }
}

__global__ __launch_bounds__(256) void masked_copy_kernel(const float* __restrict__ x, int ldx, const float* __restrict__ mask, int ldm,
                                                          float* y, int ldy, int M, int N, int accumulate) {
    const long long i = (long long)blockIdx.x * 256 + threadIdx.x;
    if (i >= (long long)M * N) return;
    const int m = (int)(i / N), n = (int)(i - (long long)m * N);
    float v = x[(long long)m * ldx + n];
    if (mask) v = mask[(long long)m * ldm + n] > 0.f ? v : 0.f;
    float* o = y + (long long)m * ldy + n;
    *o = accumulate ? *o + v : v;
}

__global__ __launch_bounds__(256) void rot6d_bwd_kernel(const float* __restrict__ x6, long long ld, int per_row,
                                                        const float* __restrict__ dR, float* __restrict__ dx6, long long ldd,
// ... 176 lines not shown
static void wgrad_x3_block(long long M, int cin, int cout, int taps, bool big, int stride, int* bco, int* bci) {
    const int v = STRAPS_TOOL_ENV_INT("STRAPS_WGRAD_TILE", 0);
    if (v) {
        const int o = v / 1000, i = v % 1000;
        const bool known = (o == 256 && i == 64) || (o == 64 && i == 256) || (o == 256 && i == 128) || (o == 128 && i == 256) || (o == 128 && i == 64) ||
                           (o == 64 && i == 128) || (o == 128 && i == 128) || (o == 64 && i == 64);
        if (known && cout % o == 0 && cin % i == 0 && !(o == 128 && i == 128 && !big)) { *bco = o; *bci = i; }
        return;
    }
    if (taps == 1) {
        if (M >= 32768 && cout % 256 == 0 && cin % 128 == 0) { *bco = 256; *bci = 128; }
        else if (M <= 8192 && cout % 128 == 0 && cin % 128 == 0) {
            if (stride == 1 && cout > cin) { *bco = 64; *bci = 128; }
            else { *bco = 128; *bci = 64; }
        }
    } else if (cout % 256 == 0 && cin % 128 == 0) { *bco = 256; *bci = 128; }
    else if (cout % 128 == 0 && cin % 64 == 0) { *bco = 128; *bci = 64; }
}

extern "C" int straps_conv_wgrad_x3_on_planes(int batch, int h, int w, int cin, int cout, int kh, int kw, int stride, int pad) {
    return wgrad_x3_route(batch, h, w, cin, cout, kh, kw, stride, pad) != 0;
}

extern "C" int straps_conv_wgrad_x3(const float* x, const float* dy, const unsigned short* x3, long long x_plane_stride, const unsigned short* dy3,
                                    long long dy_plane_stride, float* dw_oihw, void* workspace, int batch, int h, int w, int cin, int cout, int kh,
                                    int kw, int stride, int pad, int accumulate, void* stream) {
    STRAPS_REQUIRE(dw_oihw && workspace, "straps_conv_wgrad_x3: null pointer");
    const int route = (x3 && dy3) ? wgrad_x3_route(batch, h, w, cin, cout, kh, kw, stride, pad) : 0;
    STRAPS_REQUIRE(route != 0 || (x && dy), "straps_conv_wgrad_x3: this shape runs on the fp32 tensors, which are NULL (see straps_conv_wgrad_x3_on_planes)");
    STRAPS_REQUIRE(cin % 64 == 0 && cout % 64 == 0, "straps_conv_wgrad_x3: need cin%%64==0 and cout%%64==0 (cin=%d cout=%d)", cin, cout);
    Wgrad3P p3;
    int splits3;
    if (route == 1 && wgrad3_plan(batch, h, w, cin, cout, kh, kw, stride, pad, &p3, &splits3)) {
        STRAPS_REQUIRE(x_plane_stride % 8 == 0 && dy_plane_stride % 8 == 0, "straps_conv_wgrad_x3: plane strides must be multiples of 8 elements");
        Wgrad3XP q;
        q.x3 = x3; q.dy3 = dy3; q.xps = x_plane_stride; q.dps = dy_plane_stride; q.part = (float*)workspace;
        q.H = p3.H; q.W = p3.W; q.Cin = p3.Cin; q.Cout = p3.Cout; q.cw = p3.cw; q.cw_log2 = p3.cw_log2; q.rpc = p3.rpc;
        q.chunks_per_row = p3.chunks_per_row; q.chunk_rows_per_img = p3.chunk_rows_per_img; q.nchunks = p3.nchunks;
        q.chunks_per_split = p3.chunks_per_split; q.it = p3.it;
        q.rows = (long long)batch * h * w;
        constexpr int W3X_NG = 2;
        hipStream_t st3 = (hipStream_t)stream;
        Wgrad3P p64;
        int splits64;
        const bool c64 = wgrad3_plan(batch, h, w, cin, cout, kh, kw, stride, pad, &p64, &splits64, 64) && splits64 <= splits3;
        if (c64) {
            q.rpc = p64.rpc; q.chunks_per_row = p64.chunks_per_row; q.chunk_rows_per_img = p64.chunk_rows_per_img; q.nchunks = p64.nchunks;
            q.chunks_per_split = p64.chunks_per_split;
            splits3 = splits64;
            const size_t lds = (size_t)2 * 3 * (64 + 136) * 64 * sizeof(u16);
            const dim3 grid3((cout / 64) * (cin / 64), splits3);
#ifdef STRAPS_TOOLS
            static const int abl = STRAPS_TOOL_ENV_INT("STRAPS_WGRAD3_ABL", 0);
            if (abl) {
                auto kern = abl == 1 ? conv_wgrad3x3_x3_kernel<W3X_NG, 64, 1> : abl == 2 ? conv_wgrad3x3_x3_kernel<W3X_NG, 64, 2>
                          : abl == 3 ? conv_wgrad3x3_x3_kernel<W3X_NG, 64, 3> : abl == 4 ? conv_wgrad3x3_x3_kernel<W3X_NG, 64, 4> : conv_wgrad3x3_x3_kernel<W3X_NG, 64, 5>;
                hipFuncSetAttribute((const void*)kern, hipFuncAttributeMaxDynamicSharedMemorySize, (int)lds);
                hipLaunchKernelGGL(kern, grid3, dim3(256 * W3X_NG), lds, st3, q);
                STRAPS_CHECK_LAUNCH("conv_wgrad3x3_x3_kernel (ablation)");
                return STRAPS_OK;
            }
#endif
            STRAPS_RAISE_LDS((conv_wgrad3x3_x3_kernel<W3X_NG, 64>), lds, "conv_wgrad3x3_x3_kernel");
            hipLaunchKernelGGL((conv_wgrad3x3_x3_kernel<W3X_NG, 64>), grid3, dim3(256 * W3X_NG), lds, st3, q);
        } else {
            const size_t lds = (size_t)2 * 3 * (32 + 128) * 64 * sizeof(u16);
            STRAPS_RAISE_LDS((conv_wgrad3x3_x3_kernel<W3X_NG, 32>), lds, "conv_wgrad3x3_x3_kernel");
            hipLaunchKernelGGL((conv_wgrad3x3_x3_kernel<W3X_NG, 32>), dim3((cout / 64) * (cin / 64), splits3), dim3(256 * W3X_NG), lds, st3, q);
        }
        STRAPS_CHECK_LAUNCH("conv_wgrad3x3_x3_kernel");
        const long long n3 = (long long)cout * 9 * cin;
        hipLaunchKernelGGL(wgrad_reduce_kernel, dim3((unsigned)(n3 / 256)), dim3(256), 0, st3, q.part, dw_oihw, splits3, cout, cin, 9, accumulate);
        STRAPS_CHECK_LAUNCH("wgrad_reduce_kernel");
        return STRAPS_OK;
    }
    if (route == 2) {
        STRAPS_REQUIRE(x_plane_stride % 8 == 0 && dy_plane_stride % 8 == 0, "straps_conv_wgrad_x3: plane strides must be multiples of 8 elements");
        WgradXP q;
        q.x3 = x3; q.dy3 = dy3; q.xps = x_plane_stride; q.dps = dy_plane_stride; q.part = (float*)workspace;
        q.B = batch; q.H = h; q.W = w; q.Cin = cin; q.Cout = cout; q.R = kh; q.S = kw; q.stride = stride; q.pad = pad;
        q.Ho = (h + 2 * pad - kh) / stride + 1;
        q.Wo = (w + 2 * pad - kw) / stride + 1;
        const long long M = (long long)batch * q.Ho * q.Wo;
        STRAPS_REQUIRE(M < (1LL << 31), "straps_conv_wgrad_x3: problem too large");
        q.M = (int)M;
        const bool big = wgrad_big_tile(M, cin, cout, kh * kw);
        int bco = big ? 128 : 64, bci = bco;
        wgrad_x3_block(M, cin, cout, kh * kw, big, stride, &bco, &bci);
        q.ct = cout / bco; q.it = cin / bci;
        const int tiles = kh * kw * q.ct * q.it;
        const size_t lds = (size_t)2 * 3 * 32 * (bco + bci) * sizeof(u16);
        int splits;
        if (bco == bci) splits = wgrad_splits(M, tiles, bco == 128, true);
        else {
            const int per_cu = (int)((160 * 1024) / lds) < 1 ? 1 : (int)((160 * 1024) / lds);
            splits = (256 * per_cu + tiles - 1) / tiles;
            const long long max_s = (M + 127) / 128;
            if (splits > max_s) splits = (int)max_s;
            const int cap = wgrad_splits(M, kh * kw * (cout / (big ? 128 : 64)) * (cin / (big ? 128 : 64)), big);
            if (splits > cap) splits = cap;
            if (splits < 1) splits = 1;
        }
        q.rows_per_split = (int)(((M + splits - 1) / splits + 31) / 32 * 32);
        hipStream_t st = (hipStream_t)stream;
        static const int nst_env = STRAPS_TOOL_ENV_INT("STRAPS_WGRAD_TAP_NST", 2);
        constexpr int SB = 3 * 32 * 256 * 2, SS = 3 * 32 * 128 * 2;
#define STRAPS_WGRAD_X3_LAUNCH(BCO_, BCI_)                                                                              \
        do {                                                                                                            \
            STRAPS_RAISE_LDS((conv_wgrad_x3_kernel<BCO_, BCI_, 2>), lds, "conv_wgrad_x3_kernel");                       \
            hipLaunchKernelGGL((conv_wgrad_x3_kernel<BCO_, BCI_, 2>), dim3(tiles, splits), dim3(256), lds, st, q);      \
        } while (0)
        if (bco == 256 && bci == 64) STRAPS_WGRAD_X3_LAUNCH(256, 64);
        else if (bco == 64 && bci == 256) STRAPS_WGRAD_X3_LAUNCH(64, 256);
        else if (bco == 256 && bci == 128) STRAPS_WGRAD_X3_LAUNCH(256, 128);
        else if (bco == 128 && bci == 256) STRAPS_WGRAD_X3_LAUNCH(128, 256);
        else if (bco == 128 && bci == 64) STRAPS_WGRAD_X3_LAUNCH(128, 64);
        else if (bco == 64 && bci == 128) STRAPS_WGRAD_X3_LAUNCH(64, 128);
        else if (bco == 128) {
            if (nst_env == 3) {
                STRAPS_RAISE_LDS((conv_wgrad_x3_kernel<128, 128, 3>), 3 * SB, "conv_wgrad_x3_kernel");
                hipLaunchKernelGGL((conv_wgrad_x3_kernel<128, 128, 3>), dim3(tiles, splits), dim3(256), 3 * SB, st, q);
            } else {
                STRAPS_RAISE_LDS((conv_wgrad_x3_kernel<128, 128, 2>), 2 * SB, "conv_wgrad_x3_kernel");
                hipLaunchKernelGGL((conv_wgrad_x3_kernel<128, 128, 2>), dim3(tiles, splits), dim3(256), 2 * SB, st, q);
            }
        } else if (nst_env == 3) {
            STRAPS_RAISE_LDS((conv_wgrad_x3_kernel<64, 64, 3>), 3 * SS, "conv_wgrad_x3_kernel");
            hipLaunchKernelGGL((conv_wgrad_x3_kernel<64, 64, 3>), dim3(tiles, splits), dim3(256), 3 * SS, st, q);
        } else if (nst_env == 4) {
            STRAPS_RAISE_LDS((conv_wgrad_x3_kernel<64, 64, 4>), 4 * SS, "conv_wgrad_x3_kernel");
            hipLaunchKernelGGL((conv_wgrad_x3_kernel<64, 64, 4>), dim3(tiles, splits), dim3(256), 4 * SS, st, q);
        } else {
            hipLaunchKernelGGL((conv_wgrad_x3_kernel<64, 64, 2>), dim3(tiles, splits), dim3(256), 2 * SS, st, q);
        }
#undef STRAPS_WGRAD_X3_LAUNCH
        STRAPS_CHECK_LAUNCH("conv_wgrad_x3_kernel");
        const long long n = (long long)cout * kh * kw * cin;
        hipLaunchKernelGGL(wgrad_reduce_kernel, dim3((unsigned)(n / 256)), dim3(256), 0, st, q.part, dw_oihw, splits, cout, cin, kh * kw, accumulate);
        STRAPS_CHECK_LAUNCH("wgrad_reduce_kernel");
        return STRAPS_OK;
    }
    return straps_conv_wgrad(x, dy, dw_oihw, workspace, batch, h, w, cin, cout, kh, kw, stride, pad, accumulate, stream);
}

extern "C" size_t straps_stem_wgrad_workspace_bytes(int batch, int cin, int h, int w) {
    const int Ho = (h - 1) / 2 + 1, Wo = (w - 1) / 2 + 1;
    const int ntiles = batch * ((Ho + TY - 1) / TY) * ((Wo + TX - 1) / TX);
    const int Kp = (cin * 49 + 31) / 32 * 32;
    const size_t groups = (cin + CG - 1) / CG;
    return (size_t)stem_wgrad_blocks(ntiles) * 64 * Kp * sizeof(float) + straps_stem_nzmask_words(batch, cin, h, w) * sizeof(uint32_t) +
           ((groups * ntiles + 3) & ~(size_t)3);
}

extern "C" int straps_stem_wgrad(const float* x_nchw, const float* dy_nhwc, float* dw_oihw, void* workspace, const uint32_t* nzmask,
                                 int batch, int cin, int h, int w, int accumulate, void* stream) {
    STRAPS_REQUIRE(x_nchw && dy_nhwc && dw_oihw && workspace, "straps_stem_wgrad: null pointer");
    STRAPS_REQUIRE(batch > 0 && cin > 0 && h >= 7 && w >= 7, "straps_stem_wgrad: bad shape B=%d C=%d H=%d W=%d", batch, cin, h, w);
    const int K = cin * 49, Kp = (K + 31) / 32 * 32;
    const int Ho = (h - 1) / 2 + 1, Wo = (w - 1) / 2 + 1;
    const int tiles_x = (Wo + TX - 1) / TX, tiles_y = (Ho + TY - 1) / TY;
    const int ntiles = batch * tiles_x * tiles_y;
    const int nblk = stem_wgrad_blocks(ntiles);
    const int groups = (cin + CG - 1) / CG;
    STRAPS_REQUIRE(groups <= 65535, "straps_stem_wgrad: too many input channels (%d)", cin);
    hipStream_t st = (hipStream_t)stream;
    float* part = (float*)workspace;
    uint32_t* own = (uint32_t*)(part + (size_t)nblk * 64 * Kp);
    uint8_t* tact = (uint8_t*)(own + straps_stem_nzmask_words(batch, cin, h, w));
    if (!nzmask) {
        const int rc = straps_stem_nzmask(x_nchw, own, batch, cin, h, w, stream);
        if (rc != STRAPS_OK) return rc;
        nzmask = own;
    }
    hipLaunchKernelGGL(stem_tileact_kernel, dim3((ntiles * groups + 255) / 256), dim3(256), 0, st, nzmask, tact, cin, h, w, tiles_x, tiles_y, ntiles,
                       groups);
    STRAPS_CHECK_LAUNCH("stem_tileact_kernel");
    static const int rot = STRAPS_TOOL_ENV_INT("STRAPS_STEM_WGRAD_ROT", 97);
    hipLaunchKernelGGL(stem_wgrad_kernel, dim3(nblk, groups), dim3(256), 0, st, x_nchw, dy_nhwc, part, tact, batch, cin, h, w, Ho, Wo,
                       tiles_x, tiles_y, Kp, ntiles, rot);
    STRAPS_CHECK_LAUNCH("stem_wgrad_kernel");
    hipLaunchKernelGGL(stem_wgrad_reduce_kernel, dim3((64 * K + 63) / 64), dim3(256), 0, st, (const float*)workspace, dw_oihw, nblk, K, Kp, accumulate);
    STRAPS_CHECK_LAUNCH("stem_wgrad_reduce_kernel");
    return STRAPS_OK;
}

static double bn_bwd_count(long long rows, int flags) { return (flags & 2) ? (double)INFINITY : (double)rows; }

extern "C" int straps_bn_bwd_blocks(long long rows, int c) {
    const int colblocks = (c + 63) / 64;
    long long b = 2048 / colblocks;
    const long long cap = (rows + 63) / 64;
    if (b > cap) b = cap;
    return (int)(b < 1 ? 1 : b);
}

static int bn_bwd_x3_impl(const float* dy, const float* yact, const unsigned* relu_bits, const float* raw, const float* save_mean, const float* save_invstd,
                          const float* gamma, const float* mask_scale, const float* mask_shift, float* dgamma, float* dbeta, float* draw,
                          float* dz_out, unsigned short* draw_planes, long long plane_stride, void* workspace, long long rows, int c,
                          int accumulate, void* stream) {
    STRAPS_REQUIRE(!relu_bits || (!yact && (c & 31) == 0), "straps_bn_bwd_bits_x3: the bits replace yact (and need c %% 32 == 0; c=%d)", c);
    STRAPS_REQUIRE(!draw_planes || (plane_stride >= rows * c && plane_stride % 8 == 0), "straps_bn_bwd_x3: plane_stride must be >= rows*c and a multiple of 8");
    STRAPS_REQUIRE(!draw_planes || (c & 31) == 0, "straps_bn_bwd_x3: chunk-major planes need c %% 32 == 0 (c=%d)", c);
    STRAPS_REQUIRE(dy && raw && save_mean && save_invstd && gamma && dgamma && dbeta && (draw || draw_planes) && workspace, "straps_bn_bwd: null pointer");
    STRAPS_REQUIRE(rows > 0 && c > 0 && (c & 3) == 0, "straps_bn_bwd: bad shape rows=%lld c=%d", rows, c);
    const int C4 = c >> 2;
    STRAPS_REQUIRE(C4 <= 256 ? (256 % C4 == 0) : (C4 % 256 == 0), "straps_bn_bwd: channel count %d not supported", c);
    hipStream_t st = (hipStream_t)stream;
    const int nblk = straps_bn_bwd_blocks(rows, c);
    const int rpb = (int)((rows + nblk - 1) / nblk);
    double* part = (double*)workspace;
    double* coefd = part + (size_t)nblk * c * 2;
    float* k1 = (float*)(coefd + 2 * (size_t)c);
    hipLaunchKernelGGL(bn_bwd_reduce_kernel<false>, dim3(nblk, (c + 63) / 64), dim3(256), 0, st, dy, yact, raw, save_mean, save_invstd, mask_scale, mask_shift, part, rows, c, rpb, PoolSrc{}, relu_bits);
    STRAPS_CHECK_LAUNCH("bn_bwd_reduce_kernel");
    hipLaunchKernelGGL(bn_bwd_finalize_kernel, dim3((c + 3) / 4), dim3(256), 0, st, part, nblk, c, bn_bwd_count(rows, accumulate), gamma, save_invstd, dgamma, dbeta, coefd, k1, accumulate & 1);
    STRAPS_CHECK_LAUNCH("bn_bwd_finalize_kernel");
    const long long n4 = rows * C4;
    const int tiled = straps_bn_tiled(rows, c >> 2);
    hipLaunchKernelGGL(bn_bwd_apply_kernel<false>, dim3(tiled ? straps_bn_tiled_grid(rows, c >> 2, tiled) : straps_grid256_rows(n4, c >> 2)), dim3(256), 0, st, dy, yact, raw, save_mean, save_invstd, coefd, k1, mask_scale, mask_shift, draw, dz_out, draw_planes, plane_stride, n4, c, PoolSrc{}, relu_bits, tiled);
    STRAPS_CHECK_LAUNCH("bn_bwd_apply_kernel");
    return STRAPS_OK;
}

extern "C" int straps_bn_bwd_x3(const float* dy, const float* yact, const float* raw, const float* save_mean, const float* save_invstd,
                                const float* gamma, const float* mask_scale, const float* mask_shift, float* dgamma, float* dbeta, float* draw,
                                float* dz_out, unsigned short* draw_planes, long long plane_stride, void* workspace, long long rows, int c,
                                int accumulate, void* stream) {
    return bn_bwd_x3_impl(dy, yact, nullptr, raw, save_mean, save_invstd, gamma, mask_scale, mask_shift, dgamma, dbeta, draw, dz_out, draw_planes,
                          plane_stride, workspace, rows, c, accumulate, stream);
}

extern "C" int straps_bn_bwd_bits_x3(const float* dy, const unsigned* relu_bits, const float* raw, const float* save_mean, const float* save_invstd,
                                     const float* gamma, float* dgamma, float* dbeta, float* draw, unsigned short* draw_planes, long long plane_stride,
                                     void* workspace, long long rows, int c, int accumulate, void* stream) {
    STRAPS_REQUIRE(relu_bits, "straps_bn_bwd_bits_x3: null bit mask");
    return bn_bwd_x3_impl(dy, nullptr, relu_bits, raw, save_mean, save_invstd, gamma, nullptr, nullptr, dgamma, dbeta, draw, nullptr, draw_planes,
                          plane_stride, workspace, rows, c, accumulate, stream);
}

static int bn_bwd_finish_x3_impl(const float* dy, const float* yact, const unsigned* relu_bits, const float* raw, const float* save_mean,
                                 const float* save_invstd, const float* gamma, const float* mask_scale, const float* mask_shift, float* dgamma,
                                 float* dbeta, float* draw, float* dz_out, unsigned short* draw_planes, long long plane_stride, const double* partials,
                                 int nblk, void* workspace, long long rows, int c, int accumulate, void* stream) {
    STRAPS_REQUIRE(!relu_bits || (!yact && (c & 31) == 0), "straps_bn_bwd_finish_bits_x3: the bits replace yact (and need c %% 32 == 0; c=%d)", c);
    STRAPS_REQUIRE(!draw_planes || (plane_stride >= rows * c && plane_stride % 8 == 0), "straps_bn_bwd_finish_x3: plane_stride must be >= rows*c and a multiple of 8");
    STRAPS_REQUIRE(!draw_planes || (c & 31) == 0, "straps_bn_bwd_finish_x3: chunk-major planes need c %% 32 == 0 (c=%d)", c);
    STRAPS_REQUIRE(dy && raw && save_mean && save_invstd && gamma && dgamma && dbeta && (draw || draw_planes) && workspace && partials && nblk > 0,
                   "straps_bn_bwd_finish_x3: null pointer");
    STRAPS_REQUIRE(rows > 0 && c > 0 && (c & 3) == 0, "straps_bn_bwd_finish_x3: bad shape rows=%lld c=%d", rows, c);
    const int C4 = c >> 2;
    STRAPS_REQUIRE(C4 <= 256 ? (256 % C4 == 0) : (C4 % 256 == 0), "straps_bn_bwd_finish_x3: channel count %d not supported", c);
    hipStream_t st = (hipStream_t)stream;
    double* coefd = (double*)workspace;
    float* k1 = (float*)(coefd + 2 * (size_t)c);
    hipLaunchKernelGGL(bn_bwd_finalize_kernel, dim3((c + 3) / 4), dim3(256), 0, st, partials, nblk, c, bn_bwd_count(rows, accumulate), gamma, save_invstd, dgamma, dbeta, coefd, k1, accumulate & 1);
    STRAPS_CHECK_LAUNCH("bn_bwd_finalize_kernel");
    const long long n4 = rows * C4;
    const int tiled = straps_bn_tiled(rows, c >> 2);
    hipLaunchKernelGGL(bn_bwd_apply_kernel<false>, dim3(tiled ? straps_bn_tiled_grid(rows, c >> 2, tiled) : straps_grid256_rows(n4, c >> 2)), dim3(256), 0, st, dy, yact, raw, save_mean, save_invstd, coefd, k1, mask_scale, mask_shift, draw, dz_out, draw_planes, plane_stride, n4, c, PoolSrc{}, relu_bits, tiled);
    STRAPS_CHECK_LAUNCH("bn_bwd_apply_kernel");
    return STRAPS_OK;
}

extern "C" int straps_bn_bwd_finish_x3(const float* dy, const float* yact, const float* raw, const float* save_mean, const float* save_invstd,
                                       const float* gamma, const float* mask_scale, const float* mask_shift, float* dgamma, float* dbeta,
                                       float* draw, float* dz_out, unsigned short* draw_planes, long long plane_stride, const double* partials,
                                       int nblk, void* workspace, long long rows, int c, int accumulate, void* stream) {
    return bn_bwd_finish_x3_impl(dy, yact, nullptr, raw, save_mean, save_invstd, gamma, mask_scale, mask_shift, dgamma, dbeta, draw, dz_out, draw_planes,
                                 plane_stride, partials, nblk, workspace, rows, c, accumulate, stream);
}

extern "C" int straps_bn_bwd_finish_bits_x3(const float* dy, const unsigned* relu_bits, const float* raw, const float* save_mean,
                                            const float* save_invstd, const float* gamma, float* dgamma, float* dbeta, float* draw,
                                            unsigned short* draw_planes, long long plane_stride, const double* partials, int nblk, void* workspace,
                                            long long rows, int c, int accumulate, void* stream) {
    STRAPS_REQUIRE(relu_bits, "straps_bn_bwd_finish_bits_x3: null bit mask");
    return bn_bwd_finish_x3_impl(dy, nullptr, relu_bits, raw, save_mean, save_invstd, gamma, nullptr, nullptr, dgamma, dbeta, draw, nullptr, draw_planes,
                                 plane_stride, partials, nblk, workspace, rows, c, accumulate, stream);
}

extern "C" int straps_bn_bwd(const float* dy, const float* yact, const float* raw, const float* save_mean, const float* save_invstd,
                             const float* gamma, const float* mask_scale, const float* mask_shift, float* dgamma, float* dbeta, float* draw,
                             float* dz_out, void* workspace, long long rows, int c, int accumulate, void* stream) {
    return straps_bn_bwd_x3(dy, yact, raw, save_mean, save_invstd, gamma, mask_scale, mask_shift, dgamma, dbeta, draw, dz_out, nullptr, 0, workspace,
                            rows, c, accumulate, stream);
}

extern "C" size_t straps_stem_tiles(int batch, int h, int w) {
    const int Ho = (h - 1) / 2 + 1, Wo = (w - 1) / 2 + 1;
    return (size_t)batch * ((Wo + TX - 1) / TX) * ((Ho + TY - 1) / TY);
}

extern "C" int straps_stem_tile_activity(const uint32_t* nzmask, uint8_t* tile_active, int batch, int cin, int h, int w, void* stream) {
    STRAPS_REQUIRE(nzmask && tile_active, "straps_stem_tile_activity: null pointer");
    STRAPS_REQUIRE(batch > 0 && cin > 0 && h >= 7 && w >= 7, "straps_stem_tile_activity: bad shape B=%d C=%d H=%d W=%d", batch, cin, h, w);
    const int Ho = (h - 1) / 2 + 1, Wo = (w - 1) / 2 + 1;
    const int tiles_x = (Wo + TX - 1) / TX, tiles_y = (Ho + TY - 1) / TY;
    const int ntiles = batch * tiles_x * tiles_y;
    hipLaunchKernelGGL(stem_tileany_kernel, dim3((unsigned)(((long long)ntiles * 32 + 255) / 256)), dim3(256), 0, (hipStream_t)stream, nzmask, tile_active, cin, h, w, tiles_x, tiles_y,
                       ntiles);
    STRAPS_CHECK_LAUNCH("stem_tileany_kernel");
    return STRAPS_OK;
}

extern "C" int straps_bn_bwd_pooled(const float* dy_pool, const uint8_t* idx, const float* raw, const float* save_mean, const float* save_invstd,
                                    const float* gamma, const float* mask_scale, const float* mask_shift, float* dgamma, float* dbeta,
                                    float* draw, void* workspace, int batch, int h, int w, int c, int accumulate, void* stream) {
    return straps_bn_bwd_pooled_sparse(dy_pool, idx, raw, save_mean, save_invstd, gamma, mask_scale, mask_shift, dgamma, dbeta, draw, workspace, batch, h, w,
                                       c, accumulate, nullptr, stream);
}

extern "C" int straps_bn_bwd_pooled_sparse(const float* dy_pool, const uint8_t* idx, const float* raw, const float* save_mean, const float* save_invstd,
                                           const float* gamma, const float* mask_scale, const float* mask_shift, float* dgamma, float* dbeta,
                                           float* draw, void* workspace, int batch, int h, int w, int c, int accumulate,
                                           const uint8_t* tile_active, void* stream) {
    STRAPS_REQUIRE(dy_pool && idx && raw && save_mean && save_invstd && gamma && mask_scale && mask_shift && dgamma && dbeta && draw && workspace,
                   "straps_bn_bwd_pooled: null pointer");
    STRAPS_REQUIRE(batch > 0 && h > 0 && w > 0 && c > 0 && (c & 3) == 0, "straps_bn_bwd_pooled: bad shape %dx%dx%dx%d", batch, h, w, c);
    const int C4 = c >> 2;
    STRAPS_REQUIRE(C4 <= 256 ? (256 % C4 == 0) : (C4 % 256 == 0), "straps_bn_bwd_pooled: channel count %d not supported", c);
    hipStream_t st = (hipStream_t)stream;
    const long long rows = (long long)batch * h * w;
    const int nblk = straps_bn_bwd_blocks(rows, c);
    const int rpb = (int)((rows + nblk - 1) / nblk);
    double* part = (double*)workspace;
    double* coefd = part + (size_t)nblk * c * 2;
    float* k1 = (float*)(coefd + 2 * (size_t)c);
    const PoolSrc ps{dy_pool, idx, h, w, (h - 1) / 2 + 1, (w - 1) / 2 + 1, tile_active, (w + TX - 1) / TX, (h + TY - 1) / TY};
    const long long prows = (long long)batch * ps.Ho * ps.Wo;
    const int prpb = (int)((prows + nblk - 1) / nblk);
    (void)rpb;
    hipLaunchKernelGGL(bn_bwd_reduce_pooled_kernel, dim3(nblk, (c + 63) / 64), dim3(256), 0, st, raw, save_mean, save_invstd, mask_scale, mask_shift, part, prows, c, prpb, ps);
    STRAPS_CHECK_LAUNCH("bn_bwd_reduce_pooled_kernel");
    hipLaunchKernelGGL(bn_bwd_finalize_kernel, dim3((c + 3) / 4), dim3(256), 0, st, part, nblk, c, bn_bwd_count(rows, accumulate), gamma, save_invstd, dgamma, dbeta, coefd, k1, accumulate & 1);
    STRAPS_CHECK_LAUNCH("bn_bwd_finalize_kernel");
    const long long n4 = rows * C4;
    hipLaunchKernelGGL(bn_bwd_apply_kernel<true>, dim3((unsigned)((n4 + POOL_CHUNK - 1) / POOL_CHUNK)), dim3(256), 0, st, nullptr, nullptr, raw, save_mean, save_invstd, coefd, k1, mask_scale, mask_shift, draw, nullptr, (u16*)nullptr, 0LL, n4, c, ps, (const unsigned*)nullptr, 0);
    STRAPS_CHECK_LAUNCH("bn_bwd_apply_kernel<pool>");
    return STRAPS_OK;
}

extern "C" int straps_bn_relu_maxpool_fwd_x3(const float* raw, const float* scale, const float* shift, float* y_pool, uint8_t* idx,
                                             unsigned short* y_planes, long long plane_stride, int batch, int h, int w, int c, void* stream) {
    STRAPS_REQUIRE(raw && scale && shift && y_pool && idx && batch > 0 && h > 0 && w > 0 && c > 0 && (c & 3) == 0, "straps_bn_relu_maxpool_fwd: bad arguments");
    const int Ho = (h - 1) / 2 + 1, Wo = (w - 1) / 2 + 1;
    const long long n = (long long)batch * Ho * Wo * (c >> 2);
    STRAPS_REQUIRE(!y_planes || (plane_stride >= n * 4 && plane_stride % 8 == 0), "straps_bn_relu_maxpool_fwd_x3: plane_stride must be >= the output size and a multiple of 8");
    STRAPS_REQUIRE(!y_planes || (c & 31) == 0, "straps_bn_relu_maxpool_fwd_x3: chunk-major planes need c %% 32 == 0 (c=%d)", c);
    hipLaunchKernelGGL(bn_relu_maxpool_kernel, dim3(capped_grid(n)), dim3(256), 0, (hipStream_t)stream, raw, scale, shift, y_pool, idx, y_planes, plane_stride, batch, h, w, c, Ho, Wo);
    STRAPS_CHECK_LAUNCH("bn_relu_maxpool_kernel");
    return STRAPS_OK;
}

extern "C" int straps_bn_relu_maxpool_fwd(const float* raw, const float* scale, const float* shift, float* y_pool, uint8_t* idx, int batch, int h,
                                          int w, int c, void* stream) {
    return straps_bn_relu_maxpool_fwd_x3(raw, scale, shift, y_pool, idx, nullptr, 0, batch, h, w, c, stream);
}

extern "C" size_t straps_bn_bwd_workspace_bytes(long long rows, int c) {
    return ((size_t)straps_bn_bwd_blocks(rows, c) * c * 2 + 2 * (size_t)c) * sizeof(double) + (size_t)c * sizeof(float);
}

extern "C" int straps_maxpool_fwd_idx(const float* x, float* y, uint8_t* idx, int batch, int h, int w, int c, void* stream) {
    STRAPS_REQUIRE(x && y && idx && batch > 0 && (c & 3) == 0, "straps_maxpool_fwd_idx: bad arguments");
    const int Ho = (h - 1) / 2 + 1, Wo = (w - 1) / 2 + 1;
    const long long n = (long long)batch * Ho * Wo * (c >> 2);
    hipLaunchKernelGGL(maxpool_idx_kernel, dim3(capped_grid(n)), dim3(256), 0, (hipStream_t)stream, x, y, idx, batch, h, w, c, Ho, Wo);
    STRAPS_CHECK_LAUNCH("maxpool_idx_kernel");
    return STRAPS_OK;
}

extern "C" int straps_maxpool_bwd(const float* dy, const uint8_t* idx, float* dx, int batch, int h, int w, int c, void* stream) {
    STRAPS_REQUIRE(dy && idx && dx && batch > 0 && (c & 3) == 0, "straps_maxpool_bwd: bad arguments");
    const int Ho = (h - 1) / 2 + 1, Wo = (w - 1) / 2 + 1;
    const long long n = (long long)batch * h * w * (c >> 2);
    hipLaunchKernelGGL(maxpool_bwd_kernel, dim3(capped_grid(n)), dim3(256), 0, (hipStream_t)stream, dy, idx, dx, batch, h, w, c, Ho, Wo);
    STRAPS_CHECK_LAUNCH("maxpool_bwd_kernel");
    return STRAPS_OK;
}

extern "C" int straps_gap_bwd(const float* dfeat, float* dx, int batch, int hw, int c, void* stream) {
    STRAPS_REQUIRE(dfeat && dx && batch > 0 && hw > 0 && c > 0, "straps_gap_bwd: bad arguments");
    const long long n = (long long)batch * hw * c;
    hipLaunchKernelGGL(gap_bwd_kernel, dim3(capped_grid(n)), dim3(256), 0, (hipStream_t)stream, dfeat, dx, batch, hw, c);
    STRAPS_CHECK_LAUNCH("gap_bwd_kernel");
    return STRAPS_OK;
}

extern "C" int straps_masked_copy(const float* x, int ldx, const float* mask, int ldmask, float* y, int ldy, int m, int n, int accumulate,
                                  void* stream) {
    STRAPS_REQUIRE(x && y && m > 0 && n > 0, "straps_masked_copy: bad arguments");
    const long long t = (long long)m * n;
    hipLaunchKernelGGL(masked_copy_kernel, dim3((unsigned)((t + 255) / 256)), dim3(256), 0, (hipStream_t)stream, x, ldx, mask, ldmask, y, ldy, m, n, accumulate);
    STRAPS_CHECK_LAUNCH("masked_copy_kernel");
    return STRAPS_OK;
}

extern "C" int straps_rot6d_bwd(const float* x6, long long ld, int per_row, const float* drot, float* dx6, long long ldd, long long rows,
                                void* stream) {
    STRAPS_REQUIRE(x6 && drot && dx6 && rows > 0 && per_row > 0, "straps_rot6d_bwd: bad arguments");
    const long long n = rows * per_row;
    hipLaunchKernelGGL(rot6d_bwd_kernel, dim3((unsigned)((n + 255) / 256)), dim3(256), 0, (hipStream_t)stream, x6, ld, per_row, drot, dx6, ldd, n);
    STRAPS_CHECK_LAUNCH("rot6d_bwd_kernel");
    return STRAPS_OK;
}
```

### straps-3dhumanshapepose_amd/csrc/regressor_train.hip

```cpp
#include <algorithm>
#include <cstring>

#include "regressor_net.h"

namespace {

constexpr long long kX3fMinRows = 16384;
constexpr size_t kNone = ~(size_t)0;

struct Layer : Conv, Extent {
    long long rows;
    bool fmode;
    bool keep, planes, defer, bits;
    bool keep_grad;
    int nblk;
    size_t x, x3;
    long long x_ps;
    const Layer* a_bn;
    size_t raw, ss, out, out3, bitsb;
    long long out_ps;
};

struct Plan : Net {
    bool x3;
    int B, stem_nblk;
    Geometry geo;
    Layer lay[kMaxConvs];
    bool pool_planes;
    long long amax;
    size_t wstem, wsd, table, one, krsc, crsk, w1f, w1e, w3;
    size_t nz, stem_raw, stem_ss, pool, pool3, idx;
    long long pool_ps;
    size_t feat, c1, ests, h1s, h2s, fpart;
    size_t g[2], dz, dskip, dt, draw, draw3, drawd, drawd3, part, bnws, wgws, tact, sdraw, swgws, dgb, dests, dh2s, dh1s, dc1, dfeat;
    size_t bytes;
    const Layer& unit_out(int ui) const { return lay[units[ui].c[units[ui].nconv - 1]]; }
};

bool x3f_mode(const Plan& p, const Layer& cv) {
    if (!p.x3 || !straps_conv_x3f_supported(cv.cin, cv.cout, cv.k, cv.k, cv.stride, cv.pad)) return false;
    return (long long)p.B * cv.Ho * cv.Wo >= kX3fMinRows;
}

void needs(const Plan& p, const Layer& cv, bool& f32, bool& planes) {
    if (x3f_mode(p, cv)) { f32 = true; planes = false; return; }
    f32 = !straps_conv_wgrad_x3_on_planes(p.B, cv.H, cv.W, cv.cin, cv.cout, cv.k, cv.k, cv.stride, cv.pad);
    planes = true;
}

bool make_plan(Plan& p, int B, int H, int W) {
    if (!make_geometry(p, B, H, W, p.geo)) return false;
    p.x3 = p.precision == 0;
    p.B = B;
    for (int i = 0; i < p.nconvs; ++i) {
        static_cast<Conv&>(p.lay[i]) = p.convs[i];
        static_cast<Extent&>(p.lay[i]) = p.geo.e[i];
    }
    size_t b = 0;
    auto take = [&](size_t bytes) { const size_t o = b; b = align_up(b + (bytes ? bytes : 1)); return o; };
    auto f32s = [&](long long n) { return take((size_t)n * sizeof(float)); };
    auto planes = [&](long long n) { return take(3 * (size_t)round8(n) * sizeof(unsigned short)); };
    p.wstem = f32s((long long)straps_stem_weight_floats(p.cin));
    p.wsd = p.cin <= STRAPS_STEM_DGRAD_MAX_CIN ? f32s((long long)straps_stem_dgrad_weight_floats(p.cin)) : kNone;
    p.table = take(kMaxConvs * sizeof(straps_pack_desc_t));
    p.one = f32s(1);
    if (p.x3) { p.krsc = take(3 * (size_t)p.ps * sizeof(unsigned short)); p.crsk = take(3 * (size_t)p.ps * sizeof(unsigned short)); }
    else { p.krsc = f32s(p.conv_total); p.crsk = f32s(p.conv_total); }
    p.w1f = f32s((long long)p.H1 * p.F);
    p.w1e = f32s((long long)p.H1 * kEstLd);
    p.w3 = f32s((long long)(kNumParams + 31) / 32 * 32 * p.H2);
    const long long stem_n = (long long)B * p.geo.Hs * p.geo.Ws * 64, pool_n = (long long)B * p.geo.Hp * p.geo.Wp * 64;
    p.nz = take(straps_stem_nzmask_words(B, p.cin, H, W) * sizeof(uint32_t));
    p.stem_raw = f32s(stem_n);
    p.stem_ss = f32s(4 * 64);
    p.pool = f32s(pool_n);
    p.idx = take((size_t)pool_n);
    p.stem_nblk = straps_stem_stat_blocks(B, H, W);
    long long fpart = (long long)p.stem_nblk * 64 * 2;
    p.amax = pool_n;
    {
        const Unit& u0 = p.units[0];
        bool all = x3f_mode(p, p.lay[u0.c[0]]) && (!u0.has_ds || x3f_mode(p, p.lay[u0.ds]));
        p.pool_planes = p.x3 && !all;
        p.pool3 = p.pool_planes ? planes(pool_n) : kNone;
        p.pool_ps = p.pool_planes ? round8(pool_n) : 0;
    }
    long long part_d = 1, bnws = straps_bn_bwd_workspace_bytes(stem_n, 64), wgws = 4;
    size_t in = p.pool, in3 = p.pool3;
    long long in_ps = p.pool_ps;
    auto tape = [&](Layer& cv) -> bool {
        const int ch = cv.H, cw = cv.W;
        cv.rows = (long long)B * cv.Ho * cv.Wo;
        cv.fmode = x3f_mode(p, cv);
        cv.nblk = cv.fmode ? straps_conv_x3f_stat_blocks(B, ch, cw, cv.cin, cv.cout, cv.k, cv.k, cv.stride, cv.pad, 0)
                 : p.x3    ? straps_conv_x3_stat_blocks(B, ch, cw, cv.cin, cv.cout, cv.k, cv.k, cv.stride, cv.pad, 0)
                           : straps_conv_stat_blocks(B, cv.Ho, cv.Wo, cv.cout, cv.k * cv.k * cv.cin, 0);
        if (cv.nblk <= 0) return false;
        fpart = std::max(fpart, (long long)cv.nblk * cv.cout * 2);
        const long long n = cv.rows * cv.cout;
        p.amax = std::max(p.amax, n);
        bnws = std::max(bnws, (long long)straps_bn_bwd_workspace_bytes(cv.rows, cv.cout));
        wgws = std::max(wgws, (long long)(cv.fmode ? straps_conv_wgrad_x3f_workspace_bytes(B, ch, cw, cv.cin, cv.cout, cv.k, cv.k, cv.stride, cv.pad)
                                                   : straps_conv_wgrad_workspace_bytes(B, ch, cw, cv.cin, cv.cout, cv.k, cv.k, cv.stride, cv.pad)));
        if (p.x3) {
            const int nb = cv.fmode ? straps_conv_dgrad_x3f_bn_blocks(B, ch, cw, cv.cin, cv.cout, cv.k, cv.k, cv.stride, cv.pad, 0)
                                    : straps_conv_dgrad_x3_bn_blocks(B, ch, cw, cv.cin, cv.cout, cv.k, cv.k, cv.stride, cv.pad, 0);
            part_d = std::max(part_d, (long long)nb * cv.cin * 2);
        }
        cv.raw = f32s(n);
        cv.ss = f32s(4LL * cv.cout);
        return true;
    };
    for (int ui = 0; ui < p.nunits; ++ui) {
        const Unit& u = p.units[ui];
        if (u.has_ds) {
            Layer& cv = p.lay[u.ds];
            if (!tape(cv)) return false;
            cv.x = in; cv.x3 = in3; cv.x_ps = in_ps; cv.a_bn = nullptr;
            cv.keep = true; cv.planes = false; cv.defer = false; cv.bits = false;
            cv.out = f32s(cv.rows * cv.cout); cv.out3 = kNone; cv.out_ps = 0; cv.bitsb = kNone;
        }
        size_t t = in, t3 = in3;
        long long t_ps = in_ps;
        const Layer* a_bn = nullptr;
        for (int ci = 0; ci < u.nconv; ++ci) {
            Layer& cv = p.lay[u.c[ci]];
            if (!tape(cv)) return false;
            cv.x = t; cv.x3 = t3; cv.x_ps = t_ps; cv.a_bn = a_bn;
            bool keep = true, pl = true, defer = false;
            if (p.x3 && !cv.last) {
                needs(p, p.lay[u.c[ci + 1]], keep, pl);
                defer = keep && !pl;
            } else if (p.x3) {
                pl = false;
                if (ui + 1 < p.nunits) {
                    const Unit& nx = p.units[ui + 1];
                    bool f, q;
                    needs(p, p.lay[nx.c[0]], f, q);
                    pl = q;
                    if (nx.has_ds) { needs(p, p.lay[nx.ds], f, q); pl = pl || q; }
                }
            }
            cv.defer = defer;
            cv.bits = p.x3 && cv.last;
            if (defer) {
                cv.keep = false; cv.planes = false;
                cv.out = kNone; cv.out3 = kNone; cv.out_ps = 0; cv.bitsb = kNone;
                t = cv.raw; t3 = kNone; t_ps = 0; a_bn = &cv;
            } else {
                if (!p.x3) { keep = true; pl = false; }
                else keep = keep || !pl;
                cv.keep = keep; cv.planes = pl;
                cv.out = keep ? f32s(cv.rows * cv.cout) : kNone;
                cv.out3 = pl ? planes(cv.rows * cv.cout) : kNone;
                cv.out_ps = pl ? round8(cv.rows * cv.cout) : 0;
                cv.bitsb = cv.bits ? take((size_t)cv.rows * (cv.cout / 32) * sizeof(uint32_t)) : kNone;
                t = cv.out; t3 = cv.out3; t_ps = cv.out_ps; a_bn = nullptr;
            }
        }
        in = t; in3 = t3; in_ps = t_ps;
    }
    for (int i = 0; i < p.nconvs; ++i) {
        Layer& cv = p.lay[i];
        cv.keep_grad = !p.x3 || cv.fmode || !straps_conv_wgrad_x3_on_planes(B, cv.H, cv.W, cv.cin, cv.cout, cv.k, cv.k, cv.stride, cv.pad);
    }
    p.feat = f32s((long long)B * p.F);
    p.c1 = f32s((long long)B * p.H1);
    p.ests = f32s((long long)(p.iters + 1) * B * kEstLd);
    p.h1s = f32s((long long)p.iters * B * p.H1);
    p.h2s = f32s((long long)p.iters * B * p.H2);
    p.fpart = f32s(fpart);
    for (int i = 0; i < 2; ++i) p.g[i] = f32s(p.amax);
    p.dz = f32s(p.amax);
    p.dskip = f32s(p.amax);
    p.dt = f32s(p.amax);
    p.draw = f32s(p.amax);
    p.drawd = f32s(p.amax);
    p.draw3 = p.x3 ? planes(p.amax) : kNone;
    p.drawd3 = p.x3 ? planes(p.amax) : kNone;
    p.part = take((size_t)part_d * sizeof(double));
    p.bnws = take((size_t)bnws);
    p.wgws = take((size_t)wgws);
    p.tact = take(straps_stem_tiles(B, H, W));
    p.sdraw = f32s(stem_n);
    p.swgws = take(straps_stem_wgrad_workspace_bytes(B, p.cin, H, W));
    p.dgb = f32s(2 * 2048);
    p.dests = f32s((long long)(p.iters + 1) * B * kEstLd);
    p.dh2s = f32s((long long)p.iters * B * p.H2);
    p.dh1s = f32s((long long)p.iters * B * p.H1);
    p.dc1 = f32s((long long)B * p.H1);
    p.dfeat = f32s((long long)B * p.F);
    p.bytes = b;
    return true;
}

struct PackTable {
    straps_pack_desc_t d[kMaxConvs];
};

__global__ __launch_bounds__(64) void write_table_kernel(PackTable t, int n, straps_pack_desc_t* dst, float* one) {
    const int i = threadIdx.x;
    if (i < n) dst[i] = t.d[i];
    if (i == 0) *one = 1.0f;
}

struct Ws {
    char* base;
    float* f(size_t off) const { return off == kNone ? nullptr : (float*)(base + off); }
    unsigned short* h(size_t off) const { return off == kNone ? nullptr : (unsigned short*)(base + off); }
    unsigned* u(size_t off) const { return off == kNone ? nullptr : (unsigned*)(base + off); }
};

int check_common(const char* fn, const straps_regressor_desc_t* d, const float* params, const float* x, int batch, int h, int w,
                 const void* workspace, Plan& p) {
    RG_CALL(check_args(fn, d, true, x, batch, h, w, workspace));
    STRAPS_REQUIRE(params, "%s: null pointer `params`", fn);
    STRAPS_REQUIRE(((uintptr_t)params & 15) == 0, "%s: `params` must be 16-byte aligned", fn);
    make_net(d, p);
    STRAPS_REQUIRE(make_plan(p, batch, h, w), "%s: input %d x %d is too small for resnet%d", fn, h, w, p.layers);
    return STRAPS_OK;
}

int finalize(const float* params, float* bn_state, const float* part, int nblk, int c, long long rows, long long gb, long long rs, float* ss,
             hipStream_t st) {
    return straps_bn_stats_finalize(part, nblk, c, rows, params + gb, params + gb + c, kBnEps, kBnMomentum, bn_state + rs, bn_state + rs + c,
                                    ss, ss + c, ss + 2 * c, ss + 3 * c, st);
}

}

extern "C" size_t straps_regressor_train_param_floats(const straps_regressor_desc_t* d) {
    if (check_desc(d, true)) return 0;
    Net n;
    make_net(d, n);
    return (size_t)n.train_floats;
}

extern "C" size_t straps_regressor_bn_state_floats(const straps_regressor_desc_t* d) {
    if (check_desc(d, true)) return 0;
    Net n;
    make_net(d, n);
    return (size_t)n.bn_floats;
}

extern "C" size_t straps_regressor_train_workspace_bytes(const straps_regressor_desc_t* d, int batch, int h, int w) {
    if (check_desc(d, true)) return 0;
    Plan p;
    make_net(d, p);
    if (!make_plan(p, batch, h, w)) return 0;
    return p.bytes;
}

extern "C" int straps_regressor_fwd_train(const straps_regressor_desc_t* d, const float* params, float* bn_state, const float* init_est,
                                          const float* x, int batch, int h, int w, float* est, int ld_est, void* workspace,
                                          size_t workspace_bytes, void* stream) {
    static const char* fn = "straps_regressor_fwd_train";
    Plan p;
    RG_CALL(check_common(fn, d, params, x, batch, h, w, workspace, p));
    STRAPS_REQUIRE(bn_state, "%s: null pointer `bn_state`", fn);
    STRAPS_REQUIRE(init_est, "%s: null pointer `init_est`", fn);
    STRAPS_REQUIRE(est, "%s: null pointer `est`", fn);
    STRAPS_REQUIRE(ld_est >= kNumParams, "%s: `ld_est` must be >= %d (got %d)", fn, kNumParams, ld_est);
    STRAPS_REQUIRE(((uintptr_t)bn_state & 3) == 0 && ((uintptr_t)init_est & 3) == 0 && ((uintptr_t)est & 3) == 0,
                   "%s: `bn_state`, `init_est` and `est` must be float-aligned", fn);
    STRAPS_REQUIRE(workspace_bytes >= p.bytes, "%s: `workspace_bytes` is %zu, this batch needs %zu (straps_regressor_train_workspace_bytes)", fn,
                   workspace_bytes, p.bytes);
    hipStream_t st = (hipStream_t)stream;
    const Ws ws{(char*)workspace};
    const int B = batch, C = p.cin, F = p.F, H1 = p.H1, H2 = p.H2;
    const bool x3 = p.x3;
    unsigned short* krsc3 = ws.h(p.krsc);
    float* krsc = ws.f(p.krsc);

    RG_CALL(straps_pack_stem_weight(params + p.stem.w_off, ws.f(p.wstem), C, stream));
    PackTable tbl;
    memset(&tbl, 0, sizeof(tbl));
    for (int i = 0; i < p.nconvs; ++i) {
        const Conv& cv = p.convs[i];
        straps_pack_desc_t& e = tbl.d[i];
        e.src = params + cv.w_off;
        e.dst_krsc = x3 ? nullptr : ws.f(p.krsc) + cv.first;
        e.dst_crsk = x3 ? nullptr : ws.f(p.crsk) + cv.first;
        e.o = cv.cout; e.c = cv.cin; e.r = cv.k; e.s = cv.k;
        e.first = cv.first;
    }
    straps_pack_desc_t* table = (straps_pack_desc_t*)(ws.base + p.table);
    hipLaunchKernelGGL(write_table_kernel, dim3(1), dim3(64), 0, st, tbl, p.nconvs, table, ws.f(p.one));
    STRAPS_CHECK_LAUNCH("write_table_kernel");
    if (x3) RG_CALL(straps_pack_conv_weights_batched_x3(table, p.nconvs, p.conv_total, krsc3, ws.h(p.crsk), p.ps, stream));
    else RG_CALL(straps_pack_conv_weights_batched(table, p.nconvs, p.conv_total, stream));
    RG_CALL(straps_ief_pack(params + p.ief.fc1w, params + p.ief.fc3w, ws.f(p.w1f), ws.f(p.w1e), ws.f(p.w3), F, kNumParams, H1, H2, kEstLd, stream));

    uint32_t* nz = (uint32_t*)(ws.base + p.nz);
    float* part = ws.f(p.fpart);
    float* sss = ws.f(p.stem_ss);
    RG_CALL(straps_stem_nzmask(x, nz, B, C, h, w, stream));
    RG_CALL(straps_stem_fwd(x, ws.f(p.wstem), nullptr, nullptr, 0, ws.f(p.stem_raw), part, nz, B, C, h, w, stream));
    RG_CALL(finalize(params, bn_state, part, p.stem_nblk, 64, (long long)B * p.geo.Hs * p.geo.Ws, p.stem.gb_off, p.stem.rs_off, sss, st));
    if (p.pool_planes)
        RG_CALL(straps_bn_relu_maxpool_fwd_x3(ws.f(p.stem_raw), sss, sss + 64, ws.f(p.pool), (uint8_t*)(ws.base + p.idx), ws.h(p.pool3), p.pool_ps,
                                              B, p.geo.Hs, p.geo.Ws, 64, stream));
    else
        RG_CALL(straps_bn_relu_maxpool_fwd(ws.f(p.stem_raw), sss, sss + 64, ws.f(p.pool), (uint8_t*)(ws.base + p.idx), B, p.geo.Hs, p.geo.Ws, 64, stream));

    auto conv_fwd = [&](const Layer& cv) -> int {
        const float* sa = cv.a_bn ? ws.f(cv.a_bn->ss) : nullptr;
        if (cv.fmode)
            return straps_conv_fwd_x3f(ws.f(cv.x), sa, sa ? sa + cv.a_bn->cout : nullptr, cv.a_bn ? 1 : 0, krsc3 + cv.first, p.ps, nullptr, nullptr,
                                       nullptr, 0, ws.f(cv.raw), part, B, cv.H, cv.W, cv.cin, cv.cout, cv.k, cv.k, cv.stride, cv.pad, 0, stream);
        if (x3)
            return straps_conv_fwd_x3(ws.h(cv.x3), cv.x_ps, krsc3 + cv.first, p.ps, nullptr, nullptr, nullptr, 0, ws.f(cv.raw), part,
                                      B, cv.H, cv.W, cv.cin, cv.cout, cv.k, cv.k, cv.stride, cv.pad, 0, stream);
        return straps_conv_fwd(ws.f(cv.x), krsc + cv.first, nullptr, nullptr, nullptr, 0, ws.f(cv.raw), part, B, cv.H, cv.W, cv.cin, cv.cout,
                               cv.k, cv.k, cv.stride, cv.pad, 0, stream);
    };
    auto conv_bn = [&](const Layer& cv, const float* residual) -> int {
        RG_CALL(conv_fwd(cv));
        float* ss = ws.f(cv.ss);
        RG_CALL(finalize(params, bn_state, part, cv.nblk, cv.cout, cv.rows, cv.gb_off, cv.rs_off, ss, st));
        if (cv.defer) return STRAPS_OK;
        if (x3 && cv.relu) {
            if (cv.bits)
                return straps_bn_apply_bits_x3(ws.f(cv.raw), ss, ss + cv.cout, residual, ws.f(cv.out), ws.h(cv.out3), cv.out_ps, ws.u(cv.bitsb),
                                               cv.rows, cv.cout, stream);
            return straps_bn_apply_x3(ws.f(cv.raw), ss, ss + cv.cout, residual, 1, ws.f(cv.out), ws.h(cv.out3), cv.out_ps, cv.rows, cv.cout, stream);
        }
        return straps_bn_apply(ws.f(cv.raw), ss, ss + cv.cout, residual, cv.relu ? 1 : 0, ws.f(cv.out), cv.rows, cv.cout, stream);
    };
    for (int ui = 0; ui < p.nunits; ++ui) {
        const Unit& u = p.units[ui];
        const float* idt = ws.f(p.lay[u.c[0]].x);
        if (u.has_ds) {
            RG_CALL(conv_bn(p.lay[u.ds], nullptr));
            idt = ws.f(p.lay[u.ds].out);
        }
        for (int ci = 0; ci < u.nconv; ++ci) RG_CALL(conv_bn(p.lay[u.c[ci]], p.lay[u.c[ci]].last ? idt : nullptr));
    }
// ... 63 lines not shown
        const int KB = T * B;
        const float* one = ws.f(p.one);
        const straps_gemm_desc_t g[8] = {
            gd(dh2s, 1, H2, h1s, H1, 1, grads + p.ief.fc2w, H1, H2, H1, KB),
            gd(dc1, 1, H1, ws.f(p.feat), F, 1, grads + p.ief.fc1w, F + P, H1, F, B),
            gd(dh1s, 1, H1, ests, kEstLd, 1, grads + p.ief.fc1w + F, F + P, H1, P, KB),
            gd(dests + (size_t)B * kEstLd, 1, kEstLd, h2s, H2, 1, grads + p.ief.fc3w, H2, P, H2, KB),
            gd(dc1, H1, 1, ws.f(p.w1f), F, 1, dfeat, F, B, F, H1),
            gd(one, 0, 0, dh2s, H2, 1, grads + p.ief.fc2b, H2, 1, H2, KB),
            gd(one, 0, 0, dests + (size_t)B * kEstLd, kEstLd, 1, grads + p.ief.fc3b, P, 1, P, KB),
            gd(one, 0, 0, dc1, H1, 1, grads + p.ief.fc1b, H1, 1, H1, B)};
        RG_CALL(straps_gemm_multi(g, 8, stream));
    }

    double* part = (double*)(ws.base + p.part);
    void* bnws = ws.base + p.bnws;
    void* wgws = ws.base + p.wgws;
    const Layer* pending = nullptr;
    int pending_nblk = 0;
    int cur = 0;
    RG_CALL(straps_gap_bwd(dfeat, ws.f(p.g[cur]), B, p.geo.Hf * p.geo.Wf, F, stream));

    auto bn_bwd = [&](const Layer& cv, const float* dy, bool masked, float* dz, const unsigned* mask_bits, size_t out_off, size_t out3_off) -> int {
        const float* ss = ws.f(cv.ss);
        const int c = cv.cout;
        const bool sink = x3 && !cv.fmode;
        float* draw = (cv.keep_grad || !sink) ? ws.f(out_off) : nullptr;
        unsigned short* planes = sink ? ws.h(out3_off) : nullptr;
        const long long ps = sink ? round8(cv.rows * c) : 0;
        const bool from_raw = masked && !cv.last;
        const unsigned* bits = mask_bits ? mask_bits : (masked && !from_raw ? ws.u(cv.bitsb) : nullptr);
        const bool fused = pending == &cv && masked;
        if (pending == &cv) pending = nullptr;
        float* dg = dgamma(cv.gb_off);
        float* db = dbeta(cv.gb_off, c);
        if (bits) {
            if (fused)
                return straps_bn_bwd_finish_bits_x3(dy, bits, ws.f(cv.raw), ss + 2 * c, ss + 3 * c, params + cv.gb_off, dg, db, draw, planes, ps, part,
                                                    pending_nblk, bnws, cv.rows, c, 0, stream);
            return straps_bn_bwd_bits_x3(dy, bits, ws.f(cv.raw), ss + 2 * c, ss + 3 * c, params + cv.gb_off, dg, db, draw, planes, ps, bnws,
                                         cv.rows, c, 0, stream);
        }
        if (fused)
            return straps_bn_bwd_finish_x3(dy, from_raw ? nullptr : ws.f(cv.out), ws.f(cv.raw), ss + 2 * c, ss + 3 * c, params + cv.gb_off,
                                           from_raw ? ss : nullptr, from_raw ? ss + c : nullptr, dg, db, draw, dz, planes, ps, part, pending_nblk, bnws,
                                           cv.rows, c, 0, stream);
        return straps_bn_bwd_x3(dy, masked && !from_raw ? ws.f(cv.out) : nullptr, ws.f(cv.raw), ss + 2 * c, ss + 3 * c, params + cv.gb_off,
                                from_raw ? ss : nullptr, from_raw ? ss + c : nullptr, dg, db, draw, dz, planes, ps, bnws, cv.rows, c, 0, stream);
    };
    auto wgrad = [&](const Layer& cv, size_t draw_off, size_t draw3_off) -> int {
        if (!pg) return STRAPS_OK;
        float* dw = grads + cv.w_off;
        if (cv.fmode) {
            const float* sa = cv.a_bn ? ws.f(cv.a_bn->ss) : nullptr;
            return straps_conv_wgrad_x3f(ws.f(cv.x), sa, sa ? sa + cv.a_bn->cout : nullptr, cv.a_bn ? 1 : 0, ws.f(draw_off), dw, wgws, B, cv.H, cv.W,
                                         cv.cin, cv.cout, cv.k, cv.k, cv.stride, cv.pad, 0, stream);
        }
        if (x3)
            return straps_conv_wgrad_x3(ws.f(cv.x), cv.keep_grad ? ws.f(draw_off) : nullptr, ws.h(cv.x3), cv.x_ps, ws.h(draw3_off), round8(cv.rows * cv.cout),
                                        dw, wgws, B, cv.H, cv.W, cv.cin, cv.cout, cv.k, cv.k, cv.stride, cv.pad, 0, stream);
        return straps_conv_wgrad(ws.f(cv.x), ws.f(draw_off), dw, wgws, B, cv.H, cv.W, cv.cin, cv.cout, cv.k, cv.k, cv.stride, cv.pad, 0, stream);
    };
    auto dgrad = [&](const Layer& cv, size_t draw_off, size_t draw3_off, const float* addend, const unsigned* addend_bits, const Layer* bn_next,
                     float* out) -> int {
        const long long gps = round8(cv.rows * cv.cout);
        if (cv.fmode) {
            const float *raw = nullptr, *msc = nullptr, *msh = nullptr, *mean = nullptr, *invstd = nullptr;
            const unsigned* nbits = nullptr;
            double* prt = nullptr;
            int nblk = 0;
            if (bn_next) {
                const float* ssn = ws.f(bn_next->ss);
                const int cn = bn_next->cout;
                const bool from_raw = !bn_next->last;
                nbits = from_raw ? nullptr : ws.u(bn_next->bitsb);
                if (from_raw || nbits) {
                    nblk = straps_conv_dgrad_x3f_bn_blocks(B, cv.H, cv.W, cv.cin, cv.cout, cv.k, cv.k, cv.stride, cv.pad, 0);
                    prt = part;
                    raw = ws.f(bn_next->raw); mean = ssn + 2 * cn; invstd = ssn + 3 * cn;
                    if (from_raw) { msc = ssn; msh = ssn + cn; }
                }
            }
            RG_CALL(straps_conv_dgrad_x3f(ws.f(draw_off), crsk3 + cv.first, p.ps, addend, addend_bits, out, B, cv.H, cv.W, cv.cin, cv.cout, cv.k, cv.k,
                                          cv.stride, cv.pad, 0, raw, nbits, msc, msh, mean, invstd, prt, stream));
            if (prt) { pending = bn_next; pending_nblk = nblk; }
            return STRAPS_OK;
        }
        if (x3) {
            const unsigned short* g3 = ws.h(draw3_off);
            const unsigned short* w3 = crsk3 + cv.first;
            if (bn_next) {
                const float* ssn = ws.f(bn_next->ss);
                const int cn = bn_next->cout;
                const bool from_raw = !bn_next->last;
                const int nblk = straps_conv_dgrad_x3_bn_blocks(B, cv.H, cv.W, cv.cin, cv.cout, cv.k, cv.k, cv.stride, cv.pad, 0);
                const unsigned* nbits = from_raw ? nullptr : ws.u(bn_next->bitsb);
                if (addend_bits || nbits)
                    RG_CALL(straps_conv_dgrad_x3_bn_bits(g3, gps, w3, p.ps, addend, out, B, cv.H, cv.W, cv.cin, cv.cout, cv.k, cv.k, cv.stride, cv.pad, 0,
                                                         ws.f(bn_next->raw), (from_raw || nbits) ? nullptr : ws.f(bn_next->out),
                                                         from_raw ? ssn : nullptr, from_raw ? ssn + cn : nullptr, ssn + 2 * cn, ssn + 3 * cn, part,
                                                         addend_bits, nbits, stream));
                else
                    RG_CALL(straps_conv_dgrad_x3_bn(g3, gps, w3, p.ps, addend, out, B, cv.H, cv.W, cv.cin, cv.cout, cv.k, cv.k, cv.stride, cv.pad, 0,
                                                    ws.f(bn_next->raw), from_raw ? nullptr : ws.f(bn_next->out), from_raw ? ssn : nullptr,
                                                    from_raw ? ssn + cn : nullptr, ssn + 2 * cn, ssn + 3 * cn, part, stream));
                pending = bn_next;
                pending_nblk = nblk;
                return STRAPS_OK;
            }
            if (addend_bits)
                return straps_conv_dgrad_x3_bits(g3, gps, w3, p.ps, addend, out, B, cv.H, cv.W, cv.cin, cv.cout, cv.k, cv.k, cv.stride, cv.pad, 0,
                                                 addend_bits, stream);
            return straps_conv_dgrad_x3(g3, gps, w3, p.ps, addend, out, B, cv.H, cv.W, cv.cin, cv.cout, cv.k, cv.k, cv.stride, cv.pad, 0, stream);
        }
        return straps_conv_dgrad(ws.f(draw_off), crsk + cv.first, addend, out, B, cv.H, cv.W, cv.cin, cv.cout, cv.k, cv.k, cv.stride, cv.pad, 0, stream);
    };
    for (int ui = p.nunits - 1; ui >= 0; --ui) {
        const Unit& u = p.units[ui];
        const Layer* prev_last = ui > 0 ? &p.unit_out(ui - 1) : nullptr;
        const Layer& lc = p.unit_out(ui);
        const float* dy = ws.f(p.g[cur]);
        const unsigned* ubits = x3 ? ws.u(lc.bitsb) : nullptr;
        const float* dz = dy;
        if (ubits) {
            RG_CALL(bn_bwd(lc, dy, true, nullptr, nullptr, p.draw, p.draw3));
        } else {
            RG_CALL(bn_bwd(lc, dy, true, ws.f(p.dz), nullptr, p.draw, p.draw3));
            dz = ws.f(p.dz);
        }
        RG_CALL(wgrad(lc, p.draw, p.draw3));
        const float* dskip = dz;
        const unsigned* dskip_bits = nullptr;
        if (u.has_ds) {
            const Layer& ds = p.lay[u.ds];
            RG_CALL(bn_bwd(ds, dz, false, nullptr, ubits, p.drawd, p.drawd3));
            RG_CALL(wgrad(ds, p.drawd, p.drawd3));
            RG_CALL(dgrad(ds, p.drawd, p.drawd3, nullptr, nullptr, nullptr, ws.f(p.dskip)));
            dskip = ws.f(p.dskip);
        } else {
            dskip_bits = ubits;
        }
        for (int ci = u.nconv - 1; ci > 0; --ci) {
            const Layer& prev = p.lay[u.c[ci - 1]];
            RG_CALL(dgrad(p.lay[u.c[ci]], p.draw, p.draw3, nullptr, nullptr, x3 ? &prev : nullptr, ws.f(p.dt)));
            RG_CALL(bn_bwd(prev, ws.f(p.dt), true, nullptr, nullptr, p.draw, p.draw3));
            RG_CALL(wgrad(prev, p.draw, p.draw3));
        }
        RG_CALL(dgrad(p.lay[u.c[0]], p.draw, p.draw3, dskip, dskip_bits, x3 ? prev_last : nullptr, ws.f(p.g[cur ^ 1])));
        cur ^= 1;
    }

    const float* sss = ws.f(p.stem_ss);
    const uint32_t* nz = (const uint32_t*)(ws.base + p.nz);
    uint8_t* tact = nullptr;
    if (!dx) {
        tact = (uint8_t*)(ws.base + p.tact);
        RG_CALL(straps_stem_tile_activity(nz, tact, B, C, h, w, stream));
    }
    float* sdraw = ws.f(p.sdraw);
    RG_CALL(straps_bn_bwd_pooled_sparse(ws.f(p.g[cur]), (const uint8_t*)(ws.base + p.idx), ws.f(p.stem_raw), sss + 128, sss + 192, params + p.stem.gb_off,
                                        sss, sss + 64, dgamma(p.stem.gb_off), dbeta(p.stem.gb_off, 64), sdraw, bnws, B, p.geo.Hs, p.geo.Ws, 64, 0, tact, stream));
    if (dx) {
        RG_CALL(straps_pack_stem_dgrad_weight(params + p.stem.w_off, ws.f(p.wsd), C, stream));
        RG_CALL(straps_stem_dgrad(sdraw, ws.f(p.wsd), dx, B, C, h, w, 0, stream));
    }
    if (pg) RG_CALL(straps_stem_wgrad(x, sdraw, grads + p.stem.w_off, ws.base + p.swgws, nz, B, C, h, w, 0, stream));
    return STRAPS_OK;
}

extern "C" int straps_regressor_export_infer_params(const straps_regressor_desc_t* d, const float* params, const float* bn_state,
                                                    const float* init_est, float* infer_params, void* stream) {
    static const char* fn = "straps_regressor_export_infer_params";
    const char* bad = check_desc(d, true);
    STRAPS_REQUIRE(!bad, "%s: %s", fn, bad);
    STRAPS_REQUIRE(params, "%s: null pointer `params`", fn);
    STRAPS_REQUIRE(bn_state, "%s: null pointer `bn_state`", fn);
    STRAPS_REQUIRE(init_est, "%s: null pointer `init_est`", fn);
    STRAPS_REQUIRE(infer_params, "%s: null pointer `infer_params`", fn);
    Net n;
    make_net(d, n);
    hipStream_t st = (hipStream_t)stream;
    auto copy = [&](long long dst, const float* src, long long count) -> int {
        const hipError_t e = hipMemcpyAsync(infer_params + dst, src, (size_t)count * sizeof(float), hipMemcpyDeviceToDevice, st);
        if (e != hipSuccess) {
            straps_set_error("%s: hipMemcpyAsync failed: %s", fn, hipGetErrorString(e));
            return STRAPS_EHIP;
        }
        return STRAPS_OK;
    };
    auto layer = [&](const Conv& cv) -> int {
        RG_CALL(copy(cv.inf_w, params + cv.w_off, cv.weights()));
        RG_CALL(copy(cv.inf_bn, params + cv.gb_off, 2LL * cv.cout));
        return copy(cv.inf_bn + 2LL * cv.cout, bn_state + cv.rs_off, 2LL * cv.cout);
    };
    RG_CALL(layer(n.stem));
    for (int i = 0; i < n.nconvs; ++i) RG_CALL(layer(n.convs[i]));
    RG_CALL(copy(n.ief_inf.fc1w, params + n.ief.fc1w, n.train_floats - n.ief.fc1w));
    RG_CALL(copy(n.inf_init, init_est, kNumParams));
    return STRAPS_OK;
}
```

### straps-3dhumanshapepose_amd/hipabi.py

```python
import ctypes as C
import os
import subprocess

_HERE = os.path.dirname(os.path.abspath(__file__))
CSRC = os.path.join(_HERE, 'csrc')
LIB_PATH = os.path.join(CSRC, 'libstraps_hip.so')
HEADER = os.path.join(os.path.dirname(_HERE), 'include', 'straps_hip.h')
SOURCES = ['abi.hip', 'augment.hip', 'pose.hip', 'ief.hip', 'elementwise.hip', 'conv.hip', 'conv_x3.hip', 'conv_x3_lean.hip', 'conv_bf16.hip', 'conv_x3f.hip', 'conv_wgrad_x3f.hip', 'stem.hip', 'stem_dgrad.hip', 'smpl.hip',
           'smpl_bwd.hip', 'backward.hip', 'train.hip', 'metrics.hip', 'image.hip', 'raster.hip', 'exchange.hip',
           'regressor.hip', 'regressor_train.hip']

_lib = None
LINK_LIBS = ['-ldl']
EXTRA_FLAGS = {'smpl.hip': ['-fno-slp-vectorize']}


def _existing_sources():
    return [os.path.join(CSRC, s) for s in SOURCES if os.path.isfile(os.path.join(CSRC, s))]


TOOLS_LIB_PATH = os.path.join(os.path.dirname(_HERE), 'tools', 'bin', 'libstraps_hip_tools.so')


def build(force=False, verbose=False, tools=False):
# ... 31 lines not shown
            if verbose:
                print(' '.join(cmd))
            jobs.append((cmd, subprocess.Popen(cmd, cwd=CSRC)))
    for cmd, p in jobs:
        if p.wait() != 0:
            raise subprocess.CalledProcessError(p.returncode, cmd)
    objs = [os.path.join(objdir, os.path.basename(s)[:-4] + '.o') for s in srcs]
    cmd = [hipcc, '--offload-arch=gfx950', '-fPIC', '-shared', '-o', lib_path] + objs + LINK_LIBS
    if verbose:
        print(' '.join(cmd))
    subprocess.run(cmd, check=True, cwd=CSRC)
    if not tools:
        _audit(lib_path, 'hipabi.build', fresh=True)
    return lib_path


def _audit(lib_path, what, fresh=False):
    from . import isa_audit
    if not fresh and isa_audit.stamp_ok(lib_path):
        return
    if not isa_audit.enforce(lib_path, what):
        import warnings
        warnings.warn('%s: llvm-objdump not found under %s -- the packed-operand-select audit of %s (DESIGN section 1: wrong results in lanes 48..63 on '
                      'MI355X) did NOT run; set STRAPS_LLVM_BIN or audit the library where it was built (tools/audit_packed_fp32.py)'
                      % (what, isa_audit.LLVM_BIN, lib_path), RuntimeWarning, stacklevel=3)


class SmplModelStruct(C.Structure):
    _fields_ = [('blend_frag', C.c_void_p), ('j_template', C.c_void_p), ('j_shapedirs', C.c_void_p),
                ('parents', C.c_void_p), ('depth', C.c_void_p), ('max_depth', C.c_int32), ('skin_k', C.c_int32),
                ('skin_w', C.c_void_p), ('skin_j', C.c_void_p), ('vj_ptr', C.c_void_p), ('n_tiles', C.c_int32),
                ('reserved0', C.c_int32), ('pick_ids', C.c_void_p), ('blend_frag_t', C.c_void_p), ('children', C.c_void_p),
                ('jrt_ptr', C.c_void_p), ('jrt_code', C.c_void_p), ('jrt_w', C.c_void_p), ('dj_ptr', C.c_void_p), ('dj_code', C.c_void_p),
                ('dj_w', C.c_void_p), ('blend_frag_h', C.c_void_p), ('blend_h_unscale', C.c_float), ('reserved1', C.c_int32), ('skin_frag_p', C.c_void_p)]


class PackDesc(C.Structure):
    _fields_ = [('src', C.c_void_p), ('dst_krsc', C.c_void_p), ('dst_crsk', C.c_void_p), ('o', C.c_int32), ('c', C.c_int32),
                ('r', C.c_int32), ('s', C.c_int32), ('first', C.c_longlong)]


class GemmDesc(C.Structure):
    _fields_ = [('a', C.c_void_p), ('sam', C.c_longlong), ('sak', C.c_longlong), ('b', C.c_void_p), ('sbk', C.c_longlong), ('sbn', C.c_longlong),
                ('c', C.c_void_p), ('ldc', C.c_int32), ('accumulate', C.c_int32), ('addend', C.c_void_p), ('ldadd', C.c_int32), ('reserved0', C.c_int32),
                ('mask', C.c_void_p), ('ldmask', C.c_int32), ('reserved1', C.c_int32), ('c2', C.c_void_p), ('ldc2', C.c_int32), ('accumulate2', C.c_int32),
                ('m', C.c_int32), ('n', C.c_int32), ('k', C.c_int32), ('reserved2', C.c_int32)]


def gemm_desc(a, sam, sak, b, sbk, sbn, c, ldc, m, n, k, accumulate=0, addend=None, ldadd=0, mask=None, ldmask=0, c2=None, ldc2=0, accumulate2=0):
    adr = lambda t: None if t is None else (t if isinstance(t, int) else t.data_ptr())
    return GemmDesc(adr(a), sam, sak, adr(b), sbk, sbn, adr(c), ldc, accumulate, adr(addend), ldadd, 0, adr(mask), ldmask, 0, adr(c2), ldc2, accumulate2,
                    m, n, k, 0)


def gemm_multi(descs):
    arr = (GemmDesc * len(descs))(*descs)
    check(lib().straps_gemm_multi(arr, len(descs), stream_ptr()), 'straps_gemm_multi')


class RegressorDesc(C.Structure):
    _fields_ = [('layers', C.c_int32), ('in_channels', C.c_int32), ('ief_iters', C.c_int32), ('precision', C.c_int32)]


_P, _I, _L, _F, _Z, _D = C.c_void_p, C.c_int, C.c_longlong, C.c_float, C.c_size_t, C.c_double

ABI_VERSION = 12
SIGNATURES = {
    'straps_abi_version': (_I, []),
    'straps_last_error': (C.c_char_p, []),
    'straps_device_count': (_I, []),
    'straps_wall_clock_khz': (_I, []),
    'straps_set_clock_accumulator': (_I, [_P]),
    'straps_selftest_mfma_peak': (_I, [_P, _P, _I, _I, _P]),
    'straps_selftest_mfma_bf16': (_I, [_P, _P, _I, _I, _P]),
    'straps_selftest_mfma_bf16_dense': (_I, [_P, _P, _I, _I, _I, _P]),
    'straps_pack_conv_weight': (_I, [_P, _P, _I, _I, _I, _I, _P]),
    'straps_pack_conv_weight_dgrad': (_I, [_P, _P, _I, _I, _I, _I, _P]),
    'straps_pack_conv_weights_batched': (_I, [_P, _I, _L, _P]),
    'straps_pack_conv_weights_batched_x3': (_I, [_P, _I, _L, _P, _P, _L, _P]),
    'straps_stem_weight_floats': (_Z, [_I]),
    'straps_pack_stem_weight': (_I, [_P, _P, _I, _P]),
    'straps_bn_fold': (_I, [_P, _P, _P, _P, _F, _P, _P, _I, _P]),
    'straps_bn_fold_stats': (_I, [_P, _P, _P, _P, _F, _P, _P, _P, _P, _I, _P]),
    'straps_stem_stat_blocks': (_I, [_I, _I, _I]),
    'straps_stem_nzmask_words': (_Z, [_I, _I, _I, _I]),
    'straps_stem_nzmask': (_I, [_P, _P, _I, _I, _I, _I, _P]),
    'straps_stem_fwd': (_I, [_P, _P, _P, _P, _I, _P, _P, _P, _I, _I, _I, _I, _P]),
    'straps_conv_trace_buffer': (_I, [_P]),
    'straps_split3_bf16': (_I, [_P, _P, _L, _L, _P]),
    'straps_split3_bf16_cm': (_I, [_P, _P, _L, _I, _L, _P]),
    'straps_conv_fwd_x3': (_I, [_P, _L, _P, _L, _P, _P, _P, _I, _P, _P, _I, _I, _I, _I, _I, _I, _I, _I, _I, _I, _P]),
    'straps_conv_fwd_x3p': (_I, [_P, _L, _P, _L, _P, _P, _P, _I, _P, _P, _L, _I, _I, _I, _I, _I, _I, _I, _I, _I, _I, _P]),
    'straps_conv_dgrad_x3': (_I, [_P, _L, _P, _L, _P, _P, _I, _I, _I, _I, _I, _I, _I, _I, _I, _I, _P]),
    'straps_split_bf16_cm': (_I, [_P, _P, _L, _I, _P]),
    'straps_pack_conv_weight_bf16': (_I, [_P, _P, _I, _I, _I, _I, _P]),
    'straps_conv_bf16_tile_choice': (_I, [_I] * 9),
    'straps_conv_fwd_bf16': (_I, [_P, _P, _P, _P, _P, _I, _P, _P] + [_I] * 10 + [_P]),
    'straps_conv_x3_stat_blocks': (_I, [_I] * 10),
    'straps_conv_x3f_supported': (_I, [_I] * 6),
    'straps_conv_fwd_x3f': (_I, [_P, _P, _P, _I, _P, _L, _P, _P, _P, _I, _P, _P] + [_I] * 10 + [_P]),
    'straps_conv_x3f_stat_blocks': (_I, [_I] * 10),
    'straps_conv_dgrad_x3f': (_I, [_P, _P, _L, _P, _P, _P] + [_I] * 10 + [_P] * 8),
    'straps_conv_dgrad_x3f_bn_blocks': (_I, [_I] * 10),
    'straps_conv_wgrad_x3f_workspace_bytes': (_Z, [_I] * 9),
    'straps_conv_wgrad_x3f': (_I, [_P, _P, _P, _I, _P, _P, _P] + [_I] * 10 + [_P]),
    'straps_bn_apply_x3': (_I, [_P, _P, _P, _P, _I, _P, _P, _L, _L, _I, _P]),
    'straps_bn_relu_maxpool_fwd_x3': (_I, [_P, _P, _P, _P, _P, _P, _L, _I, _I, _I, _I, _P]),
    'straps_conv_wgrad_x3_on_planes': (_I, [_I] * 9),
    'straps_conv_dgrad_x3_bn_blocks': (_I, [_I] * 10),
    'straps_conv_dgrad_x3_bn': (_I, [_P, _L, _P, _L, _P, _P, _I, _I, _I, _I, _I, _I, _I, _I, _I, _I, _P, _P, _P, _P, _P, _P, _P, _P]),
    'straps_bn_bwd_finish_x3': (_I, [_P] * 13 + [_L, _P, _I, _P, _L, _I, _I, _P]),
    'straps_conv_wgrad_x3': (_I, [_P, _P, _P, _L, _P, _L, _P, _P, _I, _I, _I, _I, _I, _I, _I, _I, _I, _I, _P]),
    'straps_bn_bwd_x3': (_I, [_P] * 13 + [_L, _P, _L, _I, _I, _P]),
    'straps_bn_apply_bits_x3': (_I, [_P, _P, _P, _P, _P, _P, _L, _P, _L, _I, _P]),
    'straps_bn_bwd_bits_x3': (_I, [_P] * 10 + [_L, _P, _L, _I, _I, _P]),
    'straps_bn_bwd_finish_bits_x3': (_I, [_P] * 10 + [_L, _P, _I, _P, _L, _I, _I, _P]),
    'straps_conv_dgrad_x3_bits': (_I, [_P, _L, _P, _L, _P, _P, _I, _I, _I, _I, _I, _I, _I, _I, _I, _I, _P, _P]),
    'straps_conv_dgrad_x3_bn_bits': (_I, [_P, _L, _P, _L, _P, _P, _I, _I, _I, _I, _I, _I, _I, _I, _I, _I, _P, _P, _P, _P, _P, _P, _P, _P, _P, _P]),
    'straps_conv_stat_blocks': (_I, [_I, _I, _I, _I, _I, _I]),
    'straps_conv_fwd': (_I, [_P, _P, _P, _P, _P, _I, _P, _P, _I, _I, _I, _I, _I, _I, _I, _I, _I, _I, _P]),
    'straps_maxpool_fwd': (_I, [_P, _P, _I, _I, _I, _I, _P]),
    'straps_gap_fwd': (_I, [_P, _P, _I, _I, _I, _P]),
    'straps_bn_stats_finalize': (_I, [_P, _I, _I, _L, _P, _P, _F, _F, _P, _P, _P, _P, _P, _P, _P]),
    'straps_bn_apply': (_I, [_P, _P, _P, _P, _I, _P, _L, _I, _P]),
    'straps_linear_fwd': (_I, [_P, _I, _P, _I, _P, _P, _P, _I, _I, _I, _I, _I, _P]),
    'straps_broadcast_rows': (_I, [_P, _I, _P, _I, _I, _P]),
    'straps_ief_pack': (_I, [_P, _P, _P, _P, _P, _I, _I, _I, _I, _I, _P]),
    'straps_gemm_multi': (_I, [C.POINTER(GemmDesc), _I, _P]),
    'straps_rot6d_fwd': (_I, [_P, _L, _I, _P, _L, _P]),
    'straps_rodrigues_fwd': (_I, [_P, _P, _L, _P]),
    'straps_rodrigues_bwd': (_I, [_P, _P, _P, _L, _P]),
    'straps_orthographic_project': (_I, [_P, _P, _I, _P, _L, _I, _P]),
    'straps_orthographic_project_bwd': (_I, [_P, _P, _I, _P, _P, _P, _L, _I, _P]),
    'straps_perspective_project': (_I, [_P, _P, _P, _P, _I, _P, _L, _I, _P]),
    'straps_smpl_workspace_bytes': (_Z, [C.POINTER(SmplModelStruct), _L]),
    'straps_smpl_fwd': (_I, [C.POINTER(SmplModelStruct), _P, _P, _P, _P, _P, _L, _I, _I, _P]),
    'straps_smpl_bwd_workspace_bytes': (_Z, [_L, _I]),
    'straps_smpl_bwd': (_I, [C.POINTER(SmplModelStruct), _P, _P, _P, _P, _P, _P, _P, _L, _I, _P]),
    'straps_smpl_bwd_aa': (_I, [C.POINTER(SmplModelStruct), _P, _P, _P, _P, _P, _P, _P, _P, _P, _L, _I, _P]),
    'straps_conv_dgrad': (_I, [_P, _P, _P, _P, _I, _I, _I, _I, _I, _I, _I, _I, _I, _I, _P]),
    'straps_conv_wgrad_workspace_bytes': (_Z, [_I, _I, _I, _I, _I, _I, _I, _I, _I]),
    'straps_conv_wgrad': (_I, [_P, _P, _P, _P, _I, _I, _I, _I, _I, _I, _I, _I, _I, _I, _P]),
    'straps_stem_wgrad_workspace_bytes': (_Z, [_I, _I, _I, _I]),
    'straps_stem_wgrad': (_I, [_P, _P, _P, _P, _P, _I, _I, _I, _I, _I, _P]),
    'straps_stem_dgrad_weight_floats': (_Z, [_I]),
    'straps_pack_stem_dgrad_weight': (_I, [_P, _P, _I, _P]),
    'straps_stem_dgrad': (_I, [_P, _P, _P, _I, _I, _I, _I, _I, _P]),
    'straps_bn_bwd_blocks': (_I, [_L, _I]),
    'straps_bn_bwd_workspace_bytes': (_Z, [_L, _I]),
    'straps_bn_bwd': (_I, [_P, _P, _P, _P, _P, _P, _P, _P, _P, _P, _P, _P, _P, _L, _I, _I, _P]),
    'straps_bn_relu_maxpool_fwd': (_I, [_P, _P, _P, _P, _P, _I, _I, _I, _I, _P]),
    'straps_bn_bwd_pooled': (_I, [_P, _P, _P, _P, _P, _P, _P, _P, _P, _P, _P, _P, _I, _I, _I, _I, _I, _P]),
    'straps_bn_bwd_pooled_sparse': (_I, [_P, _P, _P, _P, _P, _P, _P, _P, _P, _P, _P, _P, _I, _I, _I, _I, _I, _P, _P]),
    'straps_stem_tiles': (_Z, [_I, _I, _I]),
    'straps_stem_tile_activity': (_I, [_P, _P, _I, _I, _I, _I, _P]),
    'straps_maxpool_fwd_idx': (_I, [_P, _P, _P, _I, _I, _I, _I, _P]),
    'straps_maxpool_bwd': (_I, [_P, _P, _P, _I, _I, _I, _I, _P]),
    'straps_gap_bwd': (_I, [_P, _P, _I, _I, _I, _P]),
    'straps_masked_copy': (_I, [_P, _I, _P, _I, _P, _I, _I, _I, _I, _P]),
    'straps_rot6d_bwd': (_I, [_P, _L, _I, _P, _P, _L, _L, _P]),
    'straps_build_proxy_input': (_I, [_P, _P, _P, _I, _I, _I, _P]),
    'straps_build_proxy_input_std': (_I, [_P, _P, _P, _I, _I, _I, _I, _P]),
    'straps_build_proxy_input_nz': (_I, [_P, _P, _P, _P, _I, _I, _I, _I, _P]),
    'straps_loss_workspace_bytes': (_Z, [_L]),
    'straps_loss_fwd_bwd': (_I, [_P, _P, _P, _I, _P, _P, _P, _P, _P, _P, _P, _P, _P, _P, _P, _P, _P, _P, _L, _I, _P]),
    'straps_loss_fwd_bwd_gm': (_I, [_P, _P, _P, _I, _P, _P, _P, _P, _P, _P, _P, _P, _P, _P, _P, _P, _P, _P, _L, _I, _P, _F, _P]),
    'straps_count_visible': (_I, [_P, _P, _L, _I, _I, _P]),
    'straps_adam_step': (_I, [_P, _P, _P, _P, _L, _I, _F, _F, _F, _F, _F, _P, _P]),
    'straps_mse_fwd': (_I, [_P, _P, _P, _L, _I, _F, _F, _P, _P, _P]),
    'straps_mse_bwd': (_I, [_P, _P, _P, _L, _I, _F, _F, _P, _P, _P]),
    'straps_augment_seg': (_I, [_P, _P, _P, _F, _I, _P, _I, _I, _P]),
    'straps_rasterize_workspace_bytes': (_Z, [_L, _I, _I]),
    'straps_rasterize_parts': (_I, [_P, _P, _P, _P, _P, _P, _P, _P, _P, _L, _I, _I, _I, _I, _F, _F, _P, _D, _D, _P]),
    'straps_philox_fill': (_I, [C.c_ulonglong, _P, _L, C.c_uint, _P, _L, _I, _P]),
    'straps_counter_add': (_I, [_P, _I, _L, _P]),
    'straps_gather_f32': (_I, [_P, _P, _P, _I, _P]),
    'straps_memset_zero': (_I, [_P, _Z, _P]),
    'straps_augment_smpl': (_I, [_P, _L, _P, _P, _P, _P, _I, _P, _D, _D, _P, _P, _P, _L, _P]),
    'straps_augment_cam_t': (_I, [_P, _P, _P, _D, _D, _D, _P, _L, _P]),
    'straps_deviate_verts2d': (_I, [_P, _P, _D, _D, _P, _L, _P]),
    'straps_deviate_joints2d': (_I, [_P, _P, _D, _D, _D, _D, _P, _L, _P]),
    'straps_project_targets': (_I, [_P, _P, _F, _F, _F, _F, _P, _P, _L, _P]),
    'straps_point_metrics': (_I, [_P, _P, _P, _L, _I, _P]),
    'straps_crop_resize': (_I, [_P, _P, _P, _D, _D, _D, _D, _D, _P, _P, _P, _I, _I, _I, _I, _P]),
    'straps_comm_unique_id': (_I, [_P]),
    'straps_comm_init_rank': (_I, [_P, _I, _I, C.POINTER(C.c_void_p)]),
    'straps_comm_destroy': (_I, [_P]),
    'straps_comm_size': (_I, [_P]),
    'straps_comm_library': (C.c_char_p, []),
    'straps_allreduce_grads': (_I, [_P, _L, _P, _P]),
    'straps_regressor_param_floats': (_Z, [C.POINTER(RegressorDesc)]),
    'straps_regressor_prepared_bytes': (_Z, [C.POINTER(RegressorDesc)]),
    'straps_regressor_prepare': (_I, [C.POINTER(RegressorDesc), _P, _P, _P]),
    'straps_regressor_workspace_bytes': (_Z, [C.POINTER(RegressorDesc), _I, _I, _I]),
    'straps_regressor_fwd_infer': (_I, [C.POINTER(RegressorDesc), _P, _P, _I, _I, _I, _P, _I, _P, _P, _Z, _P]),
    'straps_regressor_train_param_floats': (_Z, [C.POINTER(RegressorDesc)]),
    'straps_regressor_bn_state_floats': (_Z, [C.POINTER(RegressorDesc)]),
    'straps_regressor_train_workspace_bytes': (_Z, [C.POINTER(RegressorDesc), _I, _I, _I]),
    'straps_regressor_fwd_train': (_I, [C.POINTER(RegressorDesc), _P, _P, _P, _P, _I, _I, _I, _P, _I, _P, _Z, _P]),
    'straps_regressor_bwd': (_I, [C.POINTER(RegressorDesc), _P, _P, _I, _I, _I, _P, _I, _P, _P, _P, _Z, _P]),
    'straps_regressor_export_infer_params': (_I, [C.POINTER(RegressorDesc), _P, _P, _P, _P, _P]),
}


def load(path=None):
    global _lib
    if _lib is not None and path is None:
        return _lib
    p = path or LIB_PATH
    if not os.path.isfile(p):
        raise RuntimeError('libstraps_hip.so is not built (%s missing): run `python -c "import __graft_entry__ as g; '
                           'g.build()"` -- this package has no CPU fallback' % p)
    if os.path.abspath(p) != os.path.abspath(TOOLS_LIB_PATH):
        _audit(p, 'hipabi.load')
    lib = C.CDLL(p)
    if hasattr(lib, 'straps_abi_version'):
        lib.straps_abi_version.restype = C.c_int
        got = lib.straps_abi_version()
        if got != ABI_VERSION:
            raise RuntimeError('%s is ABI version %d, this package binds version %d: rebuild it (`python -c "import __graft_entry__ as g; g.build()"`)'
                               % (p, got, ABI_VERSION))
    for name, (res, args) in SIGNATURES.items():
        if not hasattr(lib, name):
            continue
        fn = getattr(lib, name)
        fn.restype = res
        fn.argtypes = args
    if path is None:
        _lib = lib
    return lib


def lib():
    return load()


def use_library(path):
    global _lib
    _lib = load(path)
    return _lib


_TRACE = os.environ.get('STRAPS_TRACE_CALLS')
_trace_fh = None


def check(rc, what):
    if rc != 0:
        raise RuntimeError('%s failed (code %d): %s' % (what, rc, lib().straps_last_error().decode()))
    if _TRACE:
        import torch
        global _trace_fh
        if _trace_fh is None:
            _trace_fh = open(_TRACE, 'a', buffering=1)
        if not torch.cuda.is_current_stream_capturing():
            _trace_fh.write(what + '\n')
            _trace_fh.flush()
            os.fsync(_trace_fh.fileno())
            torch.cuda.synchronize()


def stream_ptr():
    import torch
    return C.c_void_p(torch.cuda.current_stream().cuda_stream)


def _first_cuda_tensor(values):
    import torch
    for v in values:
        if isinstance(v, torch.Tensor):
            if v.is_cuda:
                return v
        elif isinstance(v, dict):
            t = _first_cuda_tensor(v.values())
            if t is not None:
                return t
    return None


def on_tensor_device(fn):
    import functools

    @functools.wraps(fn)
    def wrapper(*a, **k):
        import torch
        t = _first_cuda_tensor(list(a) + list(k.values()))
        if t is None or t.device.index == torch.cuda.current_device():
            return fn(*a, **k)
        with torch.cuda.device(t.device):
            return fn(*a, **k)
    return wrapper


def ptr(t):
    return C.c_void_p(0 if t is None else t.data_ptr())


def require_gpu_tensor(t, name, dtype=None):
    import torch
    if not isinstance(t, torch.Tensor) or not t.is_cuda:
        raise RuntimeError('%s must be a GPU tensor: the STRAPS hot path runs only through the HIP library '
                           '(no CPU fallback)' % name)
    if dtype is not None and t.dtype != dtype:
        raise RuntimeError('%s must have dtype %s (got %s)' % (name, dtype, t.dtype))
    if t.device.index != torch.cuda.current_device():
        raise RuntimeError('%s lives on %s but the current device is cuda:%d: kernels are launched on the current device\'s '
# ... 4 lines not shown
```

Before: 7899.

## Fuse stem BN-backward apply into stem weight-gradient kernel via pooled recompute

When no input gradient is needed, the stem BN backward now only computes reduction coefficients, and the stem wgrad kernel reconstructs the BN/ReLU/maxpool gradient (draw) on the fly from pooled dy, pool indices and raw activations while loading tiles. This removes the full-resolution draw write and re-read plus the separate apply kernel and tile-activity launch. The cost is extra per-tile arithmetic and gathers inside the wgrad kernel. The sparse tile-skipping path for the BN apply is no longer used on this route.

```diff
diff --git a/include/straps_hip.h b/include/straps_hip.h
--- a/include/straps_hip.h
+++ b/include/straps_hip.h
@@ -305,6 +305,16 @@
                                 const float* mask_scale, const float* mask_shift, float* dgamma,
                                 float* dbeta, float* draw, void* workspace, int batch, int h, int w, int c,
                                 int accumulate, const uint8_t* tile_active, void* stream);
+int straps_bn_bwd_pooled_coef(const float* dy_pool_nhwc, const uint8_t* idx, const float* raw,
+                              const float* save_mean, const float* save_invstd, const float* gamma,
+                              const float* mask_scale, const float* mask_shift, float* dgamma, float* dbeta,
+                              double* coefd, float* k1, void* workspace, int batch, int h, int w, int c,
+                              int accumulate, void* stream);
+int straps_stem_wgrad_pooled(const float* x_nchw, const float* dy_pool_nhwc, const uint8_t* idx, const float* raw,
+                             const float* save_mean, const float* save_invstd, const float* mask_scale,
+                             const float* mask_shift, const double* coefd, const float* k1, float* dw_oihw,
+                             void* workspace, const uint32_t* nzmask , int batch,
+                             int cin, int h, int w, int accumulate, void* stream);
 int straps_maxpool_fwd_idx(const float* x_nhwc, float* y_nhwc, uint8_t* idx, int batch, int h,
                            int w, int c, void* stream);
 int straps_maxpool_bwd(const float* dy_nhwc, const uint8_t* idx, float* dx_nhwc, int batch, int h,
diff --git a/straps-3dhumanshapepose_amd/autograd_ops.py b/straps-3dhumanshapepose_amd/autograd_ops.py
--- a/straps-3dhumanshapepose_amd/autograd_ops.py
+++ b/straps-3dhumanshapepose_amd/autograd_ops.py
@@ -44,6 +44,7 @@
 
 _FUSE_BN_SUMS = True
 _SPARSE_STEM_TAIL = True
+_FUSED_STEM_WGRAD = True
 
 
 def _packed_dgrad_weight(net, conv):
@@ -261,20 +262,31 @@
         bn, raw, ss = rec['bn'], rec['raw'], rec['stats']
         ws = torch.empty(L.straps_bn_bwd_workspace_bytes(B * H * W, Cc) // 4, device=raw.device, dtype=torch.float32)
         dgamma, dbeta = grads.buf(bn.weight), grads.buf(bn.bias)
-        draw = _empty_like(raw)
-        tact = None
-        if rec.get('nzmask') is not None and _SPARSE_STEM_TAIL and not want_dx:
-            _, Cin0, Hin, Win = rec['geom'][:4]
-            tact = torch.empty(L.straps_stem_tiles(B, Hin, Win), device=raw.device, dtype=torch.uint8)
-            hipabi.check(L.straps_stem_tile_activity(hipabi.ptr(rec['nzmask']), hipabi.ptr(tact), B, Cin0, Hin, Win, hipabi.stream_ptr()),
-                         'straps_stem_tile_activity')
-        hipabi.check(L.straps_bn_bwd_pooled_sparse(hipabi.ptr(dy), hipabi.ptr(idx), hipabi.ptr(raw), hipabi.ptr(ss[2]), hipabi.ptr(ss[3]),
-                                                   hipabi.ptr(bn.weight), hipabi.ptr(ss[0]), hipabi.ptr(ss[1]), hipabi.ptr(dgamma), hipabi.ptr(dbeta),
-                                                   hipabi.ptr(draw), hipabi.ptr(ws), B, H, W, Cc, 2 if rec.get('frozen') else 0, hipabi.ptr(tact),
-                                                   hipabi.stream_ptr()), 'straps_bn_bwd_pooled_sparse')
+        if not want_dx and _FUSED_STEM_WGRAD:
+            draw = None
+            coef = torch.empty(5 * Cc, device=raw.device, dtype=torch.float32)
+            pooled = (dy, idx, raw, ss, coef)
+            hipabi.check(L.straps_bn_bwd_pooled_coef(hipabi.ptr(dy), hipabi.ptr(idx), hipabi.ptr(raw), hipabi.ptr(ss[2]), hipabi.ptr(ss[3]),
+                                                     hipabi.ptr(bn.weight), hipabi.ptr(ss[0]), hipabi.ptr(ss[1]), hipabi.ptr(dgamma), hipabi.ptr(dbeta),
+                                                     hipabi.ptr(coef), hipabi.ptr(coef[4 * Cc:]), hipabi.ptr(ws), B, H, W, Cc,
+                                                     2 if rec.get('frozen') else 0, hipabi.stream_ptr()), 'straps_bn_bwd_pooled_coef')
+        else:
+            pooled = None
+            draw = _empty_like(raw)
+            tact = None
+            if rec.get('nzmask') is not None and _SPARSE_STEM_TAIL and not want_dx:
+                _, Cin0, Hin, Win = rec['geom'][:4]
+                tact = torch.empty(L.straps_stem_tiles(B, Hin, Win), device=raw.device, dtype=torch.uint8)
+                hipabi.check(L.straps_stem_tile_activity(hipabi.ptr(rec['nzmask']), hipabi.ptr(tact), B, Cin0, Hin, Win, hipabi.stream_ptr()),
+                             'straps_stem_tile_activity')
+            hipabi.check(L.straps_bn_bwd_pooled_sparse(hipabi.ptr(dy), hipabi.ptr(idx), hipabi.ptr(raw), hipabi.ptr(ss[2]), hipabi.ptr(ss[3]),
+                                                       hipabi.ptr(bn.weight), hipabi.ptr(ss[0]), hipabi.ptr(ss[1]), hipabi.ptr(dgamma), hipabi.ptr(dbeta),
+                                                       hipabi.ptr(draw), hipabi.ptr(ws), B, H, W, Cc, 2 if rec.get('frozen') else 0, hipabi.ptr(tact),
+                                                       hipabi.stream_ptr()), 'straps_bn_bwd_pooled_sparse')
         grads[bn.weight] = dgamma
         grads[bn.bias] = dbeta
     else:
+        pooled = None
         dstem = _empty_like(rec['x'])
         hipabi.check(L.straps_maxpool_bwd(hipabi.ptr(dy), hipabi.ptr(rec['idx']), hipabi.ptr(dstem), B, H, W, Cc, hipabi.stream_ptr()),
                      'straps_maxpool_bwd')
@@ -287,10 +299,17 @@
         hipabi.check(L.straps_stem_dgrad(hipabi.ptr(draw), hipabi.ptr(net._packed_stem_dgrad_weight()), hipabi.ptr(dx), B, Cin, H, W, 0,
                                          hipabi.stream_ptr()), 'straps_stem_dgrad')
     if param_grads:
-        ws = torch.empty(L.straps_stem_wgrad_workspace_bytes(B, Cin, H, W) // 4, device=draw.device, dtype=torch.float32)
+        ws = torch.empty(L.straps_stem_wgrad_workspace_bytes(B, Cin, H, W) // 4, device=rec['x'].device, dtype=torch.float32)
         dw = grads.buf(net.conv1.weight)
-        hipabi.check(L.straps_stem_wgrad(hipabi.ptr(rec['x']), hipabi.ptr(draw), hipabi.ptr(dw), hipabi.ptr(ws), hipabi.ptr(rec.get('nzmask')),
-                                         B, Cin, H, W, 0, hipabi.stream_ptr()), 'straps_stem_wgrad')
+        if pooled is not None:
+            dyp, idx, raw, ss, coef = pooled
+            hipabi.check(L.straps_stem_wgrad_pooled(hipabi.ptr(rec['x']), hipabi.ptr(dyp), hipabi.ptr(idx), hipabi.ptr(raw), hipabi.ptr(ss[2]),
+                                                    hipabi.ptr(ss[3]), hipabi.ptr(ss[0]), hipabi.ptr(ss[1]), hipabi.ptr(coef), hipabi.ptr(coef[4 * Cc:]),
+                                                    hipabi.ptr(dw), hipabi.ptr(ws), hipabi.ptr(rec.get('nzmask')), B, Cin, H, W, 0, hipabi.stream_ptr()),
+                         'straps_stem_wgrad_pooled')
+        else:
+            hipabi.check(L.straps_stem_wgrad(hipabi.ptr(rec['x']), hipabi.ptr(draw), hipabi.ptr(dw), hipabi.ptr(ws), hipabi.ptr(rec.get('nzmask')),
+                                             B, Cin, H, W, 0, hipabi.stream_ptr()), 'straps_stem_wgrad')
         grads[net.conv1.weight] = dw
     side.join()
     return (grads, dx) if want_dx else grads
diff --git a/straps-3dhumanshapepose_amd/csrc/backward.hip b/straps-3dhumanshapepose_amd/csrc/backward.hip
--- a/straps-3dhumanshapepose_amd/csrc/backward.hip
+++ b/straps-3dhumanshapepose_amd/csrc/backward.hip
@@ -686,6 +686,40 @@
     }
 }
 
+__device__ __forceinline__ void pool_grad_add(f32x4& g, uchar4 k, const f32x4& d, int want) {
+    if (k.x == want) g[0] += d[0];
+    if (k.y == want) g[1] += d[1];
+    if (k.z == want) g[2] += d[2];
+    if (k.w == want) g[3] += d[3];
+}
+
+struct BnBwdConsts { f32x4 ksc, ksh, mu, is, k1; double m1[4], m2[4]; };
+
+__device__ __forceinline__ f32x4 relu_mask_raw4(f32x4 g, const f32x4& xr, const BnBwdConsts& k) {
+#pragma unroll
+    for (int e = 0; e < 4; ++e) g[e] = fmaf(xr[e], k.ksc[e], k.ksh[e]) > 0.f ? g[e] : 0.f;
+    return g;
+}
+
+__device__ __forceinline__ f32x4 bn_bwd_draw4(const f32x4& g, const f32x4& xr, const BnBwdConsts& k) {
+    f32x4 o;
+#pragma unroll
+    for (int e = 0; e < 4; ++e) {
+        const double xh = ((double)xr[e] - (double)k.mu[e]) * (double)k.is[e];
+        o[e] = (float)((double)k.k1[e] * (((double)g[e] - k.m1[e]) - xh * k.m2[e]));
+    }
+    return o;
+}
+
+struct StemPoolDraw {
+    const float* raw;
+    const float* dyp;
+    const uint8_t* idx;
+    const float *mean, *invstd, *msc, *msh, *k1;
+    const double* coefd;
+    int Hp, Wp;
+};
+
 constexpr int TY = 2, TX = 32, PH = 2 * TY + 5, PW = 72, TPIX = TY * TX;
 constexpr int CG = 4, GK = CG * 49, GNB = (GK + 31) / 32, GUNITS = 2 * GNB, UPW = (GUNITS + 3) / 4;
 
@@ -746,10 +780,11 @@
     if (sub == 0 && tile < ntiles) tany[tile] = mine ? 1 : 0;
 }
 
+template <bool POOL>
 __global__ __launch_bounds__(256) void stem_wgrad_kernel(const float* __restrict__ x, const float* __restrict__ dy,
                                                          float* __restrict__ part, const uint8_t* __restrict__ tact, int B, int C, int H,
                                                          int W, int Ho, int Wo,
-                                                         int tiles_x, int tiles_y, int Kp, int ntiles, int rot) {
+                                                         int tiles_x, int tiles_y, int Kp, int ntiles, int rot, StemPoolDraw pd) {
     __shared__ __attribute__((aligned(16))) float patch[2 * CG * PH * PW];
     __shared__ __attribute__((aligned(16))) float dys[2 * TPIX * 68];
     const int tid = threadIdx.x, lane = tid & 63;
@@ -791,6 +826,19 @@
     constexpr int DIT = TPIX * 16 / 256;
     const bool vec = (W & 3) == 0;
     f32x4 pv[PIT], dv[DIT];
+    const int pc4 = tid & 15, pm = tid >> 4;
+    uchar4 wk[4];
+    f32x4 wd[4];
+    BnBwdConsts kc;
+    if constexpr (POOL) {
+        kc.ksc = *reinterpret_cast<const f32x4*>(pd.msc + pc4 * 4);
+        kc.ksh = *reinterpret_cast<const f32x4*>(pd.msh + pc4 * 4);
+        kc.mu = *reinterpret_cast<const f32x4*>(pd.mean + pc4 * 4);
+        kc.is = *reinterpret_cast<const f32x4*>(pd.invstd + pc4 * 4);
+        kc.k1 = *reinterpret_cast<const f32x4*>(pd.k1 + pc4 * 4);
+#pragma unroll
+        for (int e = 0; e < 4; ++e) { kc.m1[e] = pd.coefd[pc4 * 4 + e]; kc.m2[e] = pd.coefd[64 + pc4 * 4 + e]; }
+    }
     auto tile_origin = [&](int tile, int& b, int& y0, int& x0) {
         b = tile / (tiles_x * tiles_y);
         const int bid = tile - b * tiles_x * tiles_y;
@@ -813,13 +861,33 @@
             if (vec && cl < nc && ((chact >> cl) & 1u) && (unsigned)hi < (unsigned)H && wi >= 0 && wi < W)
                 pv[it] = *reinterpret_cast<const f32x4*>(x + (((long long)b * C + c0 + cl) * H + hi) * W + wi);
         }
-#pragma unroll
-        for (int it = 0; it < DIT; ++it) {
-            const int idx = tid + it * 256;
-            const int pix = idx >> 4, c4 = idx & 15;
-            const int yo = y0 + (pix >> 5), xo = x0 + (pix & 31);
-            dv[it] = f32x4{0.f, 0.f, 0.f, 0.f};
-            if (yo < Ho && xo < Wo) dv[it] = *reinterpret_cast<const f32x4*>(dy + (((long long)b * Ho + yo) * Wo + xo) * 64 + c4 * 4);
+        if constexpr (POOL) {
+#pragma unroll
+            for (int it = 0; it < DIT; ++it) {
+                const int yo = y0 + (it >> 1), xo = x0 + 2 * pm + (it & 1);
+                dv[it] = f32x4{0.f, 0.f, 0.f, 0.f};
+                if (yo < Ho && xo < Wo) dv[it] = *reinterpret_cast<const f32x4*>(pd.raw + (((long long)b * Ho + yo) * Wo + xo) * 64 + pc4 * 4);
+            }
+#pragma unroll
+            for (int w = 0; w < 4; ++w) {
+                const int ho = (y0 >> 1) + (w >> 1), wo = (x0 >> 1) + pm + (w & 1);
+                wk[w] = make_uchar4(255, 255, 255, 255);
+                wd[w] = f32x4{0.f, 0.f, 0.f, 0.f};
+                if (ho < pd.Hp && wo < pd.Wp) {
+                    const long long o = (((long long)b * pd.Hp + ho) * pd.Wp + wo) * 64 + pc4 * 4;
+                    wk[w] = *reinterpret_cast<const uchar4*>(pd.idx + o);
+                    wd[w] = *reinterpret_cast<const f32x4*>(pd.dyp + o);
+                }
+            }
+        } else {
+#pragma unroll
+            for (int it = 0; it < DIT; ++it) {
+                const int idx = tid + it * 256;
+                const int pix = idx >> 4, c4 = idx & 15;
+                const int yo = y0 + (pix >> 5), xo = x0 + (pix & 31);
+                dv[it] = f32x4{0.f, 0.f, 0.f, 0.f};
+                if (yo < Ho && xo < Wo) dv[it] = *reinterpret_cast<const f32x4*>(dy + (((long long)b * Ho + yo) * Wo + xo) * 64 + c4 * 4);
+            }
         }
     };
     auto store_tile = [&](int tile, unsigned chact, float* pb, float* db) {
@@ -843,10 +911,29 @@
                 pb[idx] = v;
             }
         }
-#pragma unroll
-        for (int it = 0; it < DIT; ++it) {
-            const int idx = tid + it * 256;
-            *reinterpret_cast<f32x4*>(db + (idx >> 4) * 68 + (idx & 15) * 4) = dv[it];
+        if constexpr (POOL) {
+            int b, y0, x0;
+            tile_origin(tile, b, y0, x0);
+#pragma unroll
+            for (int it = 0; it < DIT; ++it) {
+                const int row = it >> 1, par = it & 1;
+                f32x4 o = {0.f, 0.f, 0.f, 0.f};
+                if (y0 + row < Ho && x0 + 2 * pm + par < Wo) {
+                    f32x4 g = {0.f, 0.f, 0.f, 0.f};
+#pragma unroll
+                    for (int a = 0; a <= row; ++a)
+#pragma unroll
+                        for (int e = 0; e <= par; ++e) pool_grad_add(g, wk[a * 2 + e], wd[a * 2 + e], (row - 2 * a + 1) * 3 + (par - 2 * e + 1));
+                    o = bn_bwd_draw4(relu_mask_raw4(g, dv[it], kc), dv[it], kc);
+                }
+                *reinterpret_cast<f32x4*>(db + (row * 32 + 2 * pm + par) * 68 + pc4 * 4) = o;
+            }
+        } else {
+#pragma unroll
+            for (int it = 0; it < DIT; ++it) {
+                const int idx = tid + it * 256;
+                *reinterpret_cast<f32x4*>(db + (idx >> 4) * 68 + (idx & 15) * 4) = dv[it];
+            }
         }
     };
 
@@ -958,10 +1045,7 @@
             const long long o = ((b * ps.Ho + ho) * ps.Wo + wo) * C + c4 * 4;
             const uchar4 k = *reinterpret_cast<const uchar4*>(ps.idx + o);
             const f32x4 d = *reinterpret_cast<const f32x4*>(ps.dyp + o);
-            if (k.x == want) g[0] += d[0];
-            if (k.y == want) g[1] += d[1];
-            if (k.z == want) g[2] += d[2];
-            if (k.w == want) g[3] += d[3];
+            pool_grad_add(g, k, d, want);
         }
     }
     return g;
@@ -1145,7 +1229,7 @@
     const long long last = POOL ? (n4 < ((long long)blockIdx.x + 1) * POOL_CHUNK ? n4 : ((long long)blockIdx.x + 1) * POOL_CHUNK) : n4;
     const long long step = POOL ? 256 : (long long)gridDim.x * 256;
     const long long rows = n4 / C4;
-    struct Consts { f32x4 ksc, ksh, mu, is, k1; double m1[4], m2[4]; };
+    using Consts = BnBwdConsts;
     auto load_consts = [&](int c4) {
         Consts k;
         if (!yact && !bits && msc) { k.ksc = *reinterpret_cast<const f32x4*>(msc + c4 * 4); k.ksh = *reinterpret_cast<const f32x4*>(msh + c4 * 4); }
@@ -1180,15 +1264,9 @@
 #pragma unroll
             for (int e = 0; e < 4; ++e) g[e] = ya[e] > 0.f ? g[e] : 0.f;
         } else if (msc) {
-#pragma unroll
-            for (int e = 0; e < 4; ++e) g[e] = fmaf(xr[e], k.ksc[e], k.ksh[e]) > 0.f ? g[e] : 0.f;
-        }
-        f32x4 o;
-#pragma unroll
-        for (int e = 0; e < 4; ++e) {
-            const double xh = ((double)xr[e] - (double)k.mu[e]) * (double)k.is[e];
-            o[e] = (float)((double)k.k1[e] * (((double)g[e] - k.m1[e]) - xh * k.m2[e]));
-        }
+            g = relu_mask_raw4(g, xr, k);
+        }
+        const f32x4 o = bn_bwd_draw4(g, xr, k);
         if (dz_out) *reinterpret_cast<f32x4*>(dz_out + idx * 4) = g;
         if (draw) *reinterpret_cast<f32x4*>(draw + idx * 4) = o;
         if (planes) store_planes4_cm(planes, pstride, row, c4 * 4, rows, o);
@@ -1671,10 +1749,9 @@
            ((groups * ntiles + 3) & ~(size_t)3);
 }
 
-extern "C" int straps_stem_wgrad(const float* x_nchw, const float* dy_nhwc, float* dw_oihw, void* workspace, const uint32_t* nzmask,
-                                 int batch, int cin, int h, int w, int accumulate, void* stream) {
-    STRAPS_REQUIRE(x_nchw && dy_nhwc && dw_oihw && workspace, "straps_stem_wgrad: null pointer");
-    STRAPS_REQUIRE(batch > 0 && cin > 0 && h >= 7 && w >= 7, "straps_stem_wgrad: bad shape B=%d C=%d H=%d W=%d", batch, cin, h, w);
+template <bool POOL>
+static int stem_wgrad_launch(const float* x_nchw, const float* dy_nhwc, const StemPoolDraw& pd, float* dw_oihw, void* workspace, const uint32_t* nzmask,
+                             int batch, int cin, int h, int w, int accumulate, void* stream) {
     const int K = cin * 49, Kp = (K + 31) / 32 * 32;
     const int Ho = (h - 1) / 2 + 1, Wo = (w - 1) / 2 + 1;
     const int tiles_x = (Wo + TX - 1) / TX, tiles_y = (Ho + TY - 1) / TY;
@@ -1695,12 +1772,31 @@
                        groups);
     STRAPS_CHECK_LAUNCH("stem_tileact_kernel");
     static const int rot = STRAPS_TOOL_ENV_INT("STRAPS_STEM_WGRAD_ROT", 97);
-    hipLaunchKernelGGL(stem_wgrad_kernel, dim3(nblk, groups), dim3(256), 0, st, x_nchw, dy_nhwc, part, tact, batch, cin, h, w, Ho, Wo,
-                       tiles_x, tiles_y, Kp, ntiles, rot);
+    hipLaunchKernelGGL(stem_wgrad_kernel<POOL>, dim3(nblk, groups), dim3(256), 0, st, x_nchw, dy_nhwc, part, tact, batch, cin, h, w, Ho, Wo,
+                       tiles_x, tiles_y, Kp, ntiles, rot, pd);
     STRAPS_CHECK_LAUNCH("stem_wgrad_kernel");
     hipLaunchKernelGGL(stem_wgrad_reduce_kernel, dim3((64 * K + 63) / 64), dim3(256), 0, st, (const float*)workspace, dw_oihw, nblk, K, Kp, accumulate);
     STRAPS_CHECK_LAUNCH("stem_wgrad_reduce_kernel");
     return STRAPS_OK;
+}
+
+extern "C" int straps_stem_wgrad(const float* x_nchw, const float* dy_nhwc, float* dw_oihw, void* workspace, const uint32_t* nzmask,
+                                 int batch, int cin, int h, int w, int accumulate, void* stream) {
+    STRAPS_REQUIRE(x_nchw && dy_nhwc && dw_oihw && workspace, "straps_stem_wgrad: null pointer");
+    STRAPS_REQUIRE(batch > 0 && cin > 0 && h >= 7 && w >= 7, "straps_stem_wgrad: bad shape B=%d C=%d H=%d W=%d", batch, cin, h, w);
+    return stem_wgrad_launch<false>(x_nchw, dy_nhwc, StemPoolDraw{}, dw_oihw, workspace, nzmask, batch, cin, h, w, accumulate, stream);
+}
+
+extern "C" int straps_stem_wgrad_pooled(const float* x_nchw, const float* dy_pool, const uint8_t* idx, const float* raw, const float* save_mean,
+                                        const float* save_invstd, const float* mask_scale, const float* mask_shift, const double* coefd,
+                                        const float* k1, float* dw_oihw, void* workspace, const uint32_t* nzmask, int batch, int cin, int h, int w,
+                                        int accumulate, void* stream) {
+    STRAPS_REQUIRE(x_nchw && dy_pool && idx && raw && save_mean && save_invstd && mask_scale && mask_shift && coefd && k1 && dw_oihw && workspace,
+                   "straps_stem_wgrad_pooled: null pointer");
+    STRAPS_REQUIRE(batch > 0 && cin > 0 && h >= 7 && w >= 7, "straps_stem_wgrad_pooled: bad shape B=%d C=%d H=%d W=%d", batch, cin, h, w);
+    const int Ho = (h - 1) / 2 + 1, Wo = (w - 1) / 2 + 1;
+    const StemPoolDraw pd{raw, dy_pool, idx, save_mean, save_invstd, mask_scale, mask_shift, k1, coefd, (Ho - 1) / 2 + 1, (Wo - 1) / 2 + 1};
+    return stem_wgrad_launch<true>(x_nchw, nullptr, pd, dw_oihw, workspace, nzmask, batch, cin, h, w, accumulate, stream);
 }
 
 static double bn_bwd_count(long long rows, int flags) { return (flags & 2) ? (double)INFINITY : (double)rows; }
@@ -1829,6 +1925,31 @@
                                        c, accumulate, nullptr, stream);
 }
 
+static int bn_bwd_pooled_sums(const PoolSrc& ps, const float* raw, const float* save_mean, const float* save_invstd, const float* gamma,
+                              const float* mask_scale, const float* mask_shift, float* dgamma, float* dbeta, double* coefd, float* k1, double* part,
+                              int batch, int h, int w, int c, int accumulate, hipStream_t st) {
+    const long long rows = (long long)batch * h * w;
+    const int nblk = straps_bn_bwd_blocks(rows, c);
+    const long long prows = (long long)batch * ps.Ho * ps.Wo;
+    const int prpb = (int)((prows + nblk - 1) / nblk);
+    hipLaunchKernelGGL(bn_bwd_reduce_pooled_kernel, dim3(nblk, (c + 63) / 64), dim3(256), 0, st, raw, save_mean, save_invstd, mask_scale, mask_shift, part, prows, c, prpb, ps);
+    STRAPS_CHECK_LAUNCH("bn_bwd_reduce_pooled_kernel");
+    hipLaunchKernelGGL(bn_bwd_finalize_kernel, dim3((c + 3) / 4), dim3(256), 0, st, part, nblk, c, bn_bwd_count(rows, accumulate), gamma, save_invstd, dgamma, dbeta, coefd, k1, accumulate & 1);
+    STRAPS_CHECK_LAUNCH("bn_bwd_finalize_kernel");
+    return STRAPS_OK;
+}
+
+extern "C" int straps_bn_bwd_pooled_coef(const float* dy_pool, const uint8_t* idx, const float* raw, const float* save_mean, const float* save_invstd,
+                                         const float* gamma, const float* mask_scale, const float* mask_shift, float* dgamma, float* dbeta,
+                                         double* coefd, float* k1, void* workspace, int batch, int h, int w, int c, int accumulate, void* stream) {
+    STRAPS_REQUIRE(dy_pool && idx && raw && save_mean && save_invstd && gamma && mask_scale && mask_shift && dgamma && dbeta && coefd && k1 && workspace,
+                   "straps_bn_bwd_pooled_coef: null pointer");
+    STRAPS_REQUIRE(batch > 0 && h > 0 && w > 0 && c > 0 && (c & 3) == 0, "straps_bn_bwd_pooled_coef: bad shape %dx%dx%dx%d", batch, h, w, c);
+    const PoolSrc ps{dy_pool, idx, h, w, (h - 1) / 2 + 1, (w - 1) / 2 + 1, nullptr, 0, 0};
+    return bn_bwd_pooled_sums(ps, raw, save_mean, save_invstd, gamma, mask_scale, mask_shift, dgamma, dbeta, coefd, k1, (double*)workspace, batch, h, w, c,
+                              accumulate, (hipStream_t)stream);
+}
+
 extern "C" int straps_bn_bwd_pooled_sparse(const float* dy_pool, const uint8_t* idx, const float* raw, const float* save_mean, const float* save_invstd,
                                            const float* gamma, const float* mask_scale, const float* mask_shift, float* dgamma, float* dbeta,
                                            float* draw, void* workspace, int batch, int h, int w, int c, int accumulate,
@@ -1841,18 +1962,13 @@
     hipStream_t st = (hipStream_t)stream;
     const long long rows = (long long)batch * h * w;
     const int nblk = straps_bn_bwd_blocks(rows, c);
-    const int rpb = (int)((rows + nblk - 1) / nblk);
     double* part = (double*)workspace;
     double* coefd = part + (size_t)nblk * c * 2;
     float* k1 = (float*)(coefd + 2 * (size_t)c);
     const PoolSrc ps{dy_pool, idx, h, w, (h - 1) / 2 + 1, (w - 1) / 2 + 1, tile_active, (w + TX - 1) / TX, (h + TY - 1) / TY};
-    const long long prows = (long long)batch * ps.Ho * ps.Wo;
-    const int prpb = (int)((prows + nblk - 1) / nblk);
-    (void)rpb;
-    hipLaunchKernelGGL(bn_bwd_reduce_pooled_kernel, dim3(nblk, (c + 63) / 64), dim3(256), 0, st, raw, save_mean, save_invstd, mask_scale, mask_shift, part, prows, c, prpb, ps);
-    STRAPS_CHECK_LAUNCH("bn_bwd_reduce_pooled_kernel");
-    hipLaunchKernelGGL(bn_bwd_finalize_kernel, dim3((c + 3) / 4), dim3(256), 0, st, part, nblk, c, bn_bwd_count(rows, accumulate), gamma, save_invstd, dgamma, dbeta, coefd, k1, accumulate & 1);
-    STRAPS_CHECK_LAUNCH("bn_bwd_finalize_kernel");
+    const int rc = bn_bwd_pooled_sums(ps, raw, save_mean, save_invstd, gamma, mask_scale, mask_shift, dgamma, dbeta, coefd, k1, part, batch, h, w, c,
+                                      accumulate, st);
+    if (rc != STRAPS_OK) return rc;
     const long long n4 = rows * C4;
     hipLaunchKernelGGL(bn_bwd_apply_kernel<true>, dim3((unsigned)((n4 + POOL_CHUNK - 1) / POOL_CHUNK)), dim3(256), 0, st, nullptr, nullptr, raw, save_mean, save_invstd, coefd, k1, mask_scale, mask_shift, draw, nullptr, (u16*)nullptr, 0LL, n4, c, ps, (const unsigned*)nullptr, 0);
     STRAPS_CHECK_LAUNCH("bn_bwd_apply_kernel<pool>");
diff --git a/straps-3dhumanshapepose_amd/csrc/regressor_train.hip b/straps-3dhumanshapepose_amd/csrc/regressor_train.hip
--- a/straps-3dhumanshapepose_amd/csrc/regressor_train.hip
+++ b/straps-3dhumanshapepose_amd/csrc/regressor_train.hip
@@ -32,7 +32,7 @@
     size_t nz, stem_raw, stem_ss, pool, pool3, idx;
     long long pool_ps;
     size_t feat, c1, ests, h1s, h2s, fpart;
-    size_t g[2], dz, dskip, dt, draw, draw3, drawd, drawd3, part, bnws, wgws, tact, sdraw, swgws, dgb, dests, dh2s, dh1s, dc1, dfeat;
+    size_t g[2], dz, dskip, dt, draw, draw3, drawd, drawd3, part, bnws, wgws, sdraw, scoef, swgws, dgb, dests, dh2s, dh1s, dc1, dfeat;
     size_t bytes;
     const Layer& unit_out(int ui) const { return lay[units[ui].c[units[ui].nconv - 1]]; }
 };
@@ -181,8 +181,8 @@
     p.part = take((size_t)part_d * sizeof(double));
     p.bnws = take((size_t)bnws);
     p.wgws = take((size_t)wgws);
-    p.tact = take(straps_stem_tiles(B, H, W));
     p.sdraw = f32s(stem_n);
+    p.scoef = take(2 * 64 * sizeof(double) + 64 * sizeof(float));
     p.swgws = take(straps_stem_wgrad_workspace_bytes(B, p.cin, H, W));
     p.dgb = f32s(2 * 2048);
     p.dests = f32s((long long)(p.iters + 1) * B * kEstLd);
@@ -552,18 +552,22 @@
 
     const float* sss = ws.f(p.stem_ss);
     const uint32_t* nz = (const uint32_t*)(ws.base + p.nz);
-    uint8_t* tact = nullptr;
+    const uint8_t* pidx = (const uint8_t*)(ws.base + p.idx);
     if (!dx) {
-        tact = (uint8_t*)(ws.base + p.tact);
-        RG_CALL(straps_stem_tile_activity(nz, tact, B, C, h, w, stream));
+        double* coefd = (double*)(ws.base + p.scoef);
+        float* k1 = (float*)(coefd + 2 * 64);
+        RG_CALL(straps_bn_bwd_pooled_coef(ws.f(p.g[cur]), pidx, ws.f(p.stem_raw), sss + 128, sss + 192, params + p.stem.gb_off, sss, sss + 64,
+                                          dgamma(p.stem.gb_off), dbeta(p.stem.gb_off, 64), coefd, k1, bnws, B, p.geo.Hs, p.geo.Ws, 64, 0, stream));
+        if (pg)
+            RG_CALL(straps_stem_wgrad_pooled(x, ws.f(p.g[cur]), pidx, ws.f(p.stem_raw), sss + 128, sss + 192, sss, sss + 64, coefd, k1,
+                                             grads + p.stem.w_off, ws.base + p.swgws, nz, B, C, h, w, 0, stream));
+        return STRAPS_OK;
     }
     float* sdraw = ws.f(p.sdraw);
-    RG_CALL(straps_bn_bwd_pooled_sparse(ws.f(p.g[cur]), (const uint8_t*)(ws.base + p.idx), ws.f(p.stem_raw), sss + 128, sss + 192, params + p.stem.gb_off,
-                                        sss, sss + 64, dgamma(p.stem.gb_off), dbeta(p.stem.gb_off, 64), sdraw, bnws, B, p.geo.Hs, p.geo.Ws, 64, 0, tact, stream));
-    if (dx) {
-        RG_CALL(straps_pack_stem_dgrad_weight(params + p.stem.w_off, ws.f(p.wsd), C, stream));
-        RG_CALL(straps_stem_dgrad(sdraw, ws.f(p.wsd), dx, B, C, h, w, 0, stream));
-    }
+    RG_CALL(straps_bn_bwd_pooled(ws.f(p.g[cur]), pidx, ws.f(p.stem_raw), sss + 128, sss + 192, params + p.stem.gb_off, sss, sss + 64,
+                                 dgamma(p.stem.gb_off), dbeta(p.stem.gb_off, 64), sdraw, bnws, B, p.geo.Hs, p.geo.Ws, 64, 0, stream));
+    RG_CALL(straps_pack_stem_dgrad_weight(params + p.stem.w_off, ws.f(p.wsd), C, stream));
+    RG_CALL(straps_stem_dgrad(sdraw, ws.f(p.wsd), dx, B, C, h, w, 0, stream));
     if (pg) RG_CALL(straps_stem_wgrad(x, sdraw, grads + p.stem.w_off, ws.base + p.swgws, nz, B, C, h, w, 0, stream));
     return STRAPS_OK;
 }
diff --git a/straps-3dhumanshapepose_amd/hipabi.py b/straps-3dhumanshapepose_amd/hipabi.py
--- a/straps-3dhumanshapepose_amd/hipabi.py
+++ b/straps-3dhumanshapepose_amd/hipabi.py
@@ -207,6 +207,8 @@
     'straps_bn_relu_maxpool_fwd': (_I, [_P, _P, _P, _P, _P, _I, _I, _I, _I, _P]),
     'straps_bn_bwd_pooled': (_I, [_P, _P, _P, _P, _P, _P, _P, _P, _P, _P, _P, _P, _I, _I, _I, _I, _I, _P]),
     'straps_bn_bwd_pooled_sparse': (_I, [_P, _P, _P, _P, _P, _P, _P, _P, _P, _P, _P, _P, _I, _I, _I, _I, _I, _P, _P]),
+    'straps_bn_bwd_pooled_coef': (_I, [_P, _P, _P, _P, _P, _P, _P, _P, _P, _P, _P, _P, _P, _I, _I, _I, _I, _I, _P]),
+    'straps_stem_wgrad_pooled': (_I, [_P, _P, _P, _P, _P, _P, _P, _P, _P, _P, _P, _P, _P, _I, _I, _I, _I, _I, _P]),
     'straps_stem_tiles': (_Z, [_I, _I, _I]),
     'straps_stem_tile_activity': (_I, [_P, _P, _I, _I, _I, _I, _P]),
     'straps_maxpool_fwd_idx': (_I, [_P, _P, _P, _I, _I, _I, _I, _P]),
```

Result: no change. 7974 (median of 6 runs) (+1.0%).
